# donahowe/TheaterGen

Hardware: AMD Instinct MI355X
Metric: 512px 50-step char images/sec (node), CMIGBench 4-turn story (higher is better)
Workload: dtype bf16; 1 GPU; SD-1.5 512x512, 4-turn story x 2 characters = 8 char images per step per GPU, 50 DDIM steps, CFG 7.5, IP-Adapter 77+4 tokens scale 0.4, bf16, random-init weights; plan=sd15, char_batch=8, cfg_batch=16, streams=1, ddim_steps=50, parallelism=dialogue-sharded x1 (RCCL broadcast + all_gather only)

## Files before the change

include/theatergen_hip.h:

```cpp
#ifndef THEATERGEN_HIP_H
#define THEATERGEN_HIP_H

#include <stdint.h>

#ifdef __cplusplus
extern "C" {
#endif

#define TG_BF16 0
#define TG_F16 1

#define TG_OK 0
#define TG_ERR_ARG (-1)
#define TG_ERR_LAUNCH (-2)
#define TG_ERR_UNSUPPORTED (-3)

#define TG_ACT_NONE 0
#define TG_ACT_SILU 1
#define TG_ACT_GELU 2
#define TG_ACT_QUICK_GELU 3

#define TG_ABI_VERSION 308
int tg_version(void);
const char* tg_last_error(void);

typedef struct {
  int32_t dtype;
  int32_t mode;
  const void* a0;
  const void* a1;
  int32_t c0, c1;
  int32_t batch, in_h, in_w, out_h, out_w;
  int32_t stride, upsample;
  const void* w;
  int64_t M, N, K;
  const void* bias;
  const void* bvec;
  int64_t ldbvec;
  int64_t rows_per_batch;
  const void* res;
  int64_t ldres;
  int32_t act;
  int32_t geglu;
  float out_scale;
  void* out;
  int64_t ldc;
  int64_t n_split;
  void* out_t;
  int64_t ldt;
  void* workspace;
  int64_t workspace_bytes;
  int32_t force_split_k;
  int32_t force_tile;
  int64_t a_rows_per_batch;
  int64_t a_batch_stride;
  int32_t pad_mode;
  int32_t a_silu;
  const void* a_coef;
  const float* ln_u;
  const float* ln_v;
  float ln_eps;
  const float* ln_rows;
  int64_t lda;
  int64_t ldw;
  float* out_gn_partials;
  int32_t out_gn_groups;
} tg_gemm_desc;

int tg_gemm(const tg_gemm_desc* d, void* stream);
int64_t tg_gemm_workspace_bytes(const tg_gemm_desc* d);
int tg_gemm_plan(const tg_gemm_desc* d, int32_t* tile_m, int32_t* tile_n, int32_t* splits, int32_t* kernel_kind);
int tg_gemm_gn_partial_blocks(const tg_gemm_desc* d);

int tg_conv_up2_eligible(const tg_gemm_desc* d);
int tg_conv_up2(const tg_gemm_desc* d, void* stream);

typedef struct {
  int32_t dtype;
  int32_t batch, heads, head_dim;
  int32_t n_q;
  const void* q; int64_t q_ld, q_bs;
  const void* k0; int64_t k0_ld, k0_bs;
  const void* vt0; int64_t vt0_ld, vt0_bs;
  int32_t len0;
  const void* k1; int64_t k1_ld, k1_bs;
  const void* vt1; int64_t vt1_ld, vt1_bs;
  int32_t len1;
  float scale;
  float w1;
  void* out; int64_t out_ld, out_bs;
  int32_t causal;
  const float* w1_dev;
  const float* mask;
  int64_t mask_bs, mask_hs, mask_qs;
} tg_attn_desc;

int tg_attention(const tg_attn_desc* d, void* stream);

typedef struct {
  int32_t dtype, batch, heads, head_dim, n;
  const void* q; const void* k; const void* v; const void* dout;
  int64_t ld, bs;
  const void* qt; const void* kt; const void* doutt;
  int64_t t_ld, t_bs;
  float* stats;
  void* dq; void* dk; void* dv;
  float scale;
} tg_attn_bwd_desc;
int tg_attention_bwd(const tg_attn_bwd_desc* d, void* stream);
typedef struct {
  int32_t dtype, batch, heads, head_dim, n_q, n_k;
  const void* q; const void* dout; int64_t q_ld, q_bs;
  const void* k; const void* v; int64_t k_ld, k_bs;
  const void* kt; int64_t t_ld, t_bs;
  const float* extra; int64_t extra_ld;
  float* stats;
  void* dq;
  float scale, ds_scale;
} tg_attn_bwd_cross_desc;
int tg_attention_bwd_cross(const tg_attn_bwd_cross_desc* d, void* stream);
int tg_attention_bwd_wide(const tg_attn_bwd_desc* d, void* stream);
int tg_attention_bwd_cross_wide(const tg_attn_bwd_cross_desc* d, void* stream);

int tg_attn_probs(int32_t dtype, int32_t batch, int32_t b0, int32_t heads, int32_t head_dim, int32_t n_q,
                  const void* q, int64_t q_ld, int64_t q_bs, const void* k, int64_t k_ld, int64_t k_bs,
                  int32_t len, float scale, const int32_t* tokens, int32_t n_tokens, float* probs, void* stream);

int64_t tg_groupnorm_scratch_bytes(int32_t batch, int64_t hw, int32_t groups);
int tg_groupnorm(int32_t dtype, const void* x0, const void* x1, int32_t c0, int32_t c1, int32_t batch, int64_t hw,
                 int32_t groups, float eps, const void* gamma, const void* beta, int32_t silu, void* out,
                 void* partials, void* stream);
int tg_layernorm(int32_t dtype, const void* x, int64_t rows, int32_t C, int64_t ldx, float eps, const void* gamma,
                 const void* beta, void* out, int64_t ldo, void* stream);
int tg_layernorm_stats(int32_t dtype, const void* x, int64_t rows, int32_t C, int64_t ldx, float eps, float* stats, void* stream);
int tg_groupnorm_coef(int32_t dtype, const void* x0, const void* x1, int32_t c0, int32_t c1, int32_t batch, int64_t hw,
                      int32_t groups, float eps, const void* gamma, const void* beta, float* coef, void* partials, void* stream);

int tg_groupnorm_from_partials(int32_t dtype, const void* x, int32_t C, int32_t batch, int64_t hw, int32_t groups, float eps, const void* gamma,
                               const void* beta, int32_t silu, void* out, float* coef, const float* partials, int32_t nblk, void* stream);

int tg_geglu(int32_t dtype, const void* x, int64_t rows, int64_t inner, void* out, void* stream);
int tg_act(int32_t dtype, const void* x, int64_t n, int32_t act, void* out, void* stream);
int tg_add(int32_t dtype, const void* a, const void* b, int64_t n, void* out, void* stream);

int tg_transpose(int32_t dtype, const void* src, int32_t batch, int32_t rows, int32_t cols, void* dst, void* stream);

int tg_conv1x1_nchw(const float* x, int32_t batch, int32_t cin, int32_t cout, int64_t hw, const float* weight,
                    const float* bias, float in_scale, float* out, void* stream);
int tg_softmax_rows(int32_t dtype, const void* x, int64_t rows, int32_t cols, int64_t ldx, float scale, void* out,
                    int64_t ldo, void* stream);

int tg_conv_in(int32_t dtype, const void* sample, int32_t src_dtype, int32_t batch, int32_t cin, int32_t h, int32_t w,
               const void* weight, const void* bias, int32_t cout, void* out, void* stream);
int tg_conv_out(int32_t dtype, const void* x, int32_t batch, int32_t cin, int32_t h, int32_t w, const void* weight,
                const void* bias, int32_t cout, void* out, int32_t out_f32, void* stream);
int tg_conv_out_gn(int32_t dtype, const void* x, const float* coef, int32_t a_silu, int32_t batch, int32_t cin, int32_t h, int32_t w,
                   const void* weight, const void* bias, int32_t cout, void* out, int32_t out_f32, void* stream);
int tg_conv_out_takes_coef(int32_t cin, int32_t h, int32_t w, int32_t cout);

int tg_timestep_embedding(int32_t dtype, const float* t, const int32_t* index, int32_t t_stride, int32_t rows, int32_t dim,
                          int32_t flip_sin_to_cos, float freq_shift, void* out, int64_t ldo, void* stream);

int tg_step_epilogue(const float* noise_pred, float* latents, int32_t n_img, int32_t chw, int32_t hw,
                     int32_t has_cfg, float guidance_scale, const float* coef, int32_t* step_idx, int32_t advance,
                     int32_t prediction_type, const float* frozen, const float* frozen_mask, int32_t mask_per_img,
                     int32_t frozen_steps, float* history, void* model_in, int32_t model_in_dtype, void* stream);

int tg_step_epilogue_sigma(const float* noise_pred, float* latents, int32_t n_img, int32_t chw, int32_t hw,
                           int32_t has_cfg, float guidance_scale, const float* coef, int32_t* step_idx, int32_t advance,
                           const void* noise, int32_t noise_dtype, const float* frozen, const float* frozen_mask,
                           int32_t mask_per_img, int32_t frozen_steps, float* history, void* model_in, int32_t model_in_dtype,
                           void* stream);

int tg_pixel_unshuffle(int32_t dtype, const void* in, int32_t batch, int32_t channels, int32_t h, int32_t w, int32_t factor,
                       void* out, void* stream);
int tg_relu(int32_t dtype, const void* x, int64_t n, void* out, void* stream);
int tg_avgpool2x2(int32_t dtype, const void* x, int32_t batch, int32_t h, int32_t w, int32_t channels, void* out, void* stream);
int tg_scale_repeat(int32_t dtype, const void* x, int64_t n, float scale, int32_t copies, void* out, void* stream);

int64_t tg_groupnorm_bwd_scratch_bytes(int32_t batch, int64_t hw, int32_t groups);
int tg_groupnorm_bwd(int32_t dtype, const void* x, const void* dy, int32_t batch, int64_t hw, int32_t channels, int32_t groups, float eps,
                     const void* gamma, const void* beta, int32_t silu, void* dx, void* partials, void* stream);
int tg_layernorm_bwd(int32_t dtype, const void* x, const void* dy, int64_t rows, int32_t channels, float eps, const void* gamma, void* dx,
                     void* stream);
int tg_geglu_bwd(int32_t dtype, const void* h, const void* dg, int64_t rows, int64_t inner, void* dh, void* stream);
int tg_softmax_bwd_rows(int32_t dtype, const void* probs, int32_t probs_fp32, int64_t ld_probs, const void* dprobs, int64_t ld_dprobs,
                        const float* extra, int64_t ld_extra, int64_t rows, int32_t length, float scale, void* dscores, void* probs_out,
                        int64_t ld_out, void* stream);
int tg_sumpool2x2(int32_t dtype, const void* du, int32_t batch, int32_t h, int32_t w, int32_t channels, void* out, void* stream);

int tg_blend_latents(const float* bg, const float* fg, const float* mask, int32_t planes, int32_t hw, float ratio,
                     float sigma, int32_t storage_dtype, float* out, void* stream);
int tg_shift(const float* src, int64_t planes, int32_t h, int32_t w, int32_t dx, int32_t dy, float* dst, void* stream);
int tg_gaussian_sample(const float* moments, const float* noise, int32_t batch, int32_t channels, int32_t hw, float scale,
                       float* out, void* stream);
int tg_add_noise(const float* x0, const float* noise, const float* ca, const float* cb, int32_t steps, int64_t n, float* out,
                 void* stream);
int tg_masked_compose(float* dst, const float* src, const float* mask, int64_t planes, int32_t hw, void* stream);

int tg_guidance_topk(const float* attn, int32_t heads, int32_t hw, int32_t n_tok, int32_t token, const float* mask,
                     int32_t k_fg, int32_t k_bg, float fg_w, float bg_w, float scale, float* out, float* grad,
                     void* stream);
int tg_guidance_ratio(const float* attn, int32_t heads, int32_t hw, int32_t n_tok, int32_t token, const float* mask,
                      float scale, float* out, float* grad, void* stream);
int tg_guidance_ref(const float* attn, int32_t heads, int32_t hw, int32_t n_tok, int32_t token, const float* ref,
                    const float* mask, float eps, float scale, float* out, float* grad, void* stream);
typedef struct {
  const float* attn;
  float* grad;
  const float* mask;
  const float* ref;
  int32_t heads, hw, n_tok, token;
  int32_t kind, k_fg, k_bg, reserved;
  float fg_w, bg_w, scale, eps;
} tg_guidance_item;
int tg_guidance_batch(const tg_guidance_item* items_device, int32_t n_items, int32_t max_hw_topk, int32_t max_heads,
                      float* partials, float* out, void* stream);

#define TG_GUIDANCE_MAX_SLOTS 64
typedef struct {
  int32_t attn_slot, grad_slot , mask_slot, ref_slot ;
  int32_t heads, hw, n_tok, token;
  int32_t kind, k_fg, k_bg, reserved;
  float fg_w, bg_w, scale, eps;
} tg_guidance_pitem;
int tg_guidance_plan_run(const tg_guidance_pitem* items_device, int32_t n_items, int32_t max_hw_topk, int32_t max_heads,
                         const void* const* slots_host, int32_t n_slots, float* head_terms, float* out, void* stream);

typedef struct {
  int32_t dtype;
  const void* x; int64_t ldx;
  const void* wpk;
  const void* res; int64_t ldres;
  void* out; int64_t ldc;
  int64_t M;
  int32_t N, K;
  int32_t ln;
  float ln_eps;
  int32_t variant;
  const float* v640;
  const float* u640;
} tg_rc_linear_desc;
int tg_rc_linear(const tg_rc_linear_desc* d, void* stream);

typedef struct {
  int32_t dtype;
  const void* h; int64_t ldh;
  const void* wq;
  const void* kv;
  const void* wo;
  void* out; int64_t ldc;
  int64_t M;
  int32_t rows_per_batch;
  int32_t text_len, ip_tokens;
  float ln_eps;
  const float* ip_scale;
} tg_rc_xattn_desc;
int tg_rc_xattn(const tg_rc_xattn_desc* d, void* stream);
int tg_rc_kv_pack(int32_t dtype, int32_t batch, const void* k, const void* vt, int64_t ldt, int32_t text_len, const void* kip,
                  const void* vtip, int64_t ldi, int32_t ip_tokens, void* out, void* stream);

typedef struct {
  int32_t dtype;
  const void* h; int64_t ldh;
  const void* w1;
  const void* w2;
  const float* b2;
  const void* wpo;
  const void* res0; int64_t ldres;
  void* out; int64_t ldc;
  int64_t M;
  int32_t inner;
  float ln_eps;
  int32_t dbg;
} tg_rc_ff_desc;
int tg_rc_ff(const tg_rc_ff_desc* d, void* stream);

typedef struct {
  int32_t dtype;
  const void* x; int64_t ldx;
  const float* coef;
  const void* win;
  const void* wqkv;
  void* y; int64_t ldy;
  void* qk; int64_t ldqk;
  void* vt; int64_t ldt;
  int64_t M;
  int32_t rows_per_batch;
  float ln_eps;
  int32_t dbg;
} tg_rc_front_desc;
int tg_rc_front(const tg_rc_front_desc* d, void* stream);

typedef struct {
  void* ptr;
  int64_t ld;
  int64_t batch_stride;
  int32_t n_end;
  int32_t transposed;
} tg_skinny_seg;
typedef struct {
  int32_t dtype;
  const void* x; int64_t ldx;
  const void* wpk;
  int64_t M;
  int32_t N, K;
  int32_t ln;
  float ln_eps;
  const float* ln_u;
  const float* ln_v;
  const void* bias;
  int32_t act;
  const void* res; int64_t ldres;
  int32_t nseg;
  int32_t rows_per_batch;
  tg_skinny_seg seg[3];
} tg_skinny_desc;
int tg_skinny_gemm(const tg_skinny_desc* d, void* stream);

typedef struct {
  int32_t dtype;
  const void* x; int64_t ldx;
  const void* wq;
  const float* ln_u;
  const float* ln_v;
  float ln_eps;
// ... 18 lines not shown
```

theatergen_amd/_lib.py:

```python
import ctypes as C
import os

HERE = os.path.dirname(os.path.abspath(__file__))
LIB_PATH = os.environ.get("THEATERGEN_HIP_LIB") or os.path.join(HERE, "lib", "libtheatergen_hip.so")

TG_BF16, TG_F16 = 0, 1
ABI_VERSION = 308
ACT_NONE, ACT_SILU, ACT_GELU, ACT_QUICK_GELU = 0, 1, 2, 3

i32, i64, f32, vp = C.c_int32, C.c_int64, C.c_float, C.c_void_p


class GemmDesc(C.Structure):
    _fields_ = [
        ("dtype", i32), ("mode", i32), ("a0", vp), ("a1", vp), ("c0", i32), ("c1", i32),
        ("batch", i32), ("in_h", i32), ("in_w", i32), ("out_h", i32), ("out_w", i32),
        ("stride", i32), ("upsample", i32), ("w", vp), ("M", i64), ("N", i64), ("K", i64),
        ("bias", vp), ("bvec", vp), ("ldbvec", i64), ("rows_per_batch", i64), ("res", vp), ("ldres", i64),
        ("act", i32), ("geglu", i32), ("out_scale", f32), ("out", vp), ("ldc", i64), ("n_split", i64),
        ("out_t", vp), ("ldt", i64), ("workspace", vp), ("workspace_bytes", i64),
        ("force_split_k", i32), ("force_tile", i32), ("a_rows_per_batch", i64), ("a_batch_stride", i64),
        ("pad_mode", i32), ("a_silu", i32), ("a_coef", vp), ("ln_u", vp), ("ln_v", vp), ("ln_eps", f32), ("ln_rows", vp),
        ("lda", i64), ("ldw", i64), ("out_gn_partials", vp), ("out_gn_groups", i32),
    ]
# ... 34 lines not shown
        ("dtype", i32), ("x", vp), ("ldx", i64), ("wpk", vp), ("res", vp), ("ldres", i64),
        ("out", vp), ("ldc", i64), ("M", i64), ("N", i32), ("K", i32), ("ln", i32), ("ln_eps", f32), ("variant", i32), ("v640", vp), ("u640", vp),
    ]


class RcXattnDesc(C.Structure):
    _fields_ = [
        ("dtype", i32), ("h", vp), ("ldh", i64), ("wq", vp), ("kv", vp), ("wo", vp), ("out", vp), ("ldc", i64), ("M", i64),
        ("rows_per_batch", i32), ("text_len", i32), ("ip_tokens", i32), ("ln_eps", f32), ("ip_scale", vp),
    ]


class XqAttnDesc(C.Structure):
    _fields_ = [
        ("dtype", i32), ("x", vp), ("ldx", i64), ("wq", vp), ("ln_u", vp), ("ln_v", vp), ("ln_eps", f32), ("kv", vp), ("ip_scale", vp),
        ("out", vp), ("ldc", i64), ("M", i64), ("C", i32), ("head_dim", i32), ("rows_per_batch", i32), ("text_len", i32), ("ip_tokens", i32),
    ]


class RcFfDesc(C.Structure):
    _fields_ = [
        ("dtype", i32), ("h", vp), ("ldh", i64), ("w1", vp), ("w2", vp), ("b2", vp), ("wpo", vp), ("res0", vp), ("ldres", i64),
        ("out", vp), ("ldc", i64), ("M", i64), ("inner", i32), ("ln_eps", f32), ("dbg", i32),
    ]


class SkinnySeg(C.Structure):
    _fields_ = [("ptr", vp), ("ld", i64), ("batch_stride", i64), ("n_end", i32), ("transposed", i32)]


class SkinnyDesc(C.Structure):
    _fields_ = [
        ("dtype", i32), ("x", vp), ("ldx", i64), ("wpk", vp), ("M", i64), ("N", i32), ("K", i32), ("ln", i32), ("ln_eps", f32), ("ln_u", vp), ("ln_v", vp),
        ("bias", vp), ("act", i32), ("res", vp), ("ldres", i64), ("nseg", i32), ("rows_per_batch", i32), ("seg", SkinnySeg * 3),
    ]


class RcFrontDesc(C.Structure):
    _fields_ = [
        ("dtype", i32), ("x", vp), ("ldx", i64), ("coef", vp), ("win", vp), ("wqkv", vp), ("y", vp), ("ldy", i64), ("qk", vp), ("ldqk", i64),
        ("vt", vp), ("ldt", i64), ("M", i64), ("rows_per_batch", i32), ("ln_eps", f32), ("dbg", i32),
    ]


class GuidanceItem(C.Structure):
    _fields_ = [
        ("attn", vp), ("grad", vp), ("mask", vp), ("ref", vp),
        ("heads", i32), ("hw", i32), ("n_tok", i32), ("token", i32),
        ("kind", i32), ("k_fg", i32), ("k_bg", i32), ("reserved", i32),
        ("fg_w", f32), ("bg_w", f32), ("scale", f32), ("eps", f32),
    ]


class GuidancePItem(C.Structure):
    _fields_ = [
        ("attn_slot", i32), ("grad_slot", i32), ("mask_slot", i32), ("ref_slot", i32),
        ("heads", i32), ("hw", i32), ("n_tok", i32), ("token", i32),
        ("kind", i32), ("k_fg", i32), ("k_bg", i32), ("reserved", i32),
        ("fg_w", f32), ("bg_w", f32), ("scale", f32), ("eps", f32),
    ]


GUIDANCE_MAX_SLOTS = 64

SIGNATURES = {
    "tg_version": (i32, []),
    "tg_last_error": (C.c_char_p, []),
    "tg_gemm": (i32, [C.POINTER(GemmDesc), vp]),
    "tg_gemm_workspace_bytes": (i64, [C.POINTER(GemmDesc)]),
    "tg_gemm_plan": (i32, [C.POINTER(GemmDesc), vp, vp, vp, vp]),
    "tg_attention": (i32, [C.POINTER(AttnDesc), vp]),
    "tg_attention_bwd": (i32, [C.POINTER(AttnBwdDesc), vp]),
    "tg_attention_bwd_cross": (i32, [C.POINTER(AttnBwdCrossDesc), vp]),
    "tg_attention_bwd_wide": (i32, [C.POINTER(AttnBwdDesc), vp]),
    "tg_attention_bwd_cross_wide": (i32, [C.POINTER(AttnBwdCrossDesc), vp]),
    "tg_attn_probs": (i32, [i32, i32, i32, i32, i32, i32, vp, i64, i64, vp, i64, i64, i32, f32, vp, i32, vp, vp]),
    "tg_groupnorm_scratch_bytes": (i64, [i32, i64, i32]),
    "tg_groupnorm": (i32, [i32, vp, vp, i32, i32, i32, i64, i32, f32, vp, vp, i32, vp, vp, vp]),
    "tg_layernorm": (i32, [i32, vp, i64, i32, i64, f32, vp, vp, vp, i64, vp]),
    "tg_layernorm_stats": (i32, [i32, vp, i64, i32, i64, f32, vp, vp]),
    "tg_groupnorm_coef": (i32, [i32, vp, vp, i32, i32, i32, i64, i32, f32, vp, vp, vp, vp, vp]),
    "tg_groupnorm_from_partials": (i32, [i32, vp, i32, i32, i64, i32, f32, vp, vp, i32, vp, vp, vp, i32, vp]),
    "tg_gemm_gn_partial_blocks": (i32, [C.POINTER(GemmDesc)]),
    "tg_conv_up2_eligible": (i32, [C.POINTER(GemmDesc)]),
    "tg_conv_up2": (i32, [C.POINTER(GemmDesc), vp]),
    "tg_geglu": (i32, [i32, vp, i64, i64, vp, vp]),
    "tg_act": (i32, [i32, vp, i64, i32, vp, vp]),
    "tg_add": (i32, [i32, vp, vp, i64, vp, vp]),
    "tg_transpose": (i32, [i32, vp, i32, i32, i32, vp, vp]),
    "tg_conv1x1_nchw": (i32, [vp, i32, i32, i32, i64, vp, vp, f32, vp, vp]),
    "tg_softmax_rows": (i32, [i32, vp, i64, i32, i64, f32, vp, i64, vp]),
    "tg_conv_in": (i32, [i32, vp, i32, i32, i32, i32, i32, vp, vp, i32, vp, vp]),
    "tg_conv_out": (i32, [i32, vp, i32, i32, i32, i32, vp, vp, i32, vp, i32, vp]),
    "tg_conv_out_gn": (i32, [i32, vp, vp, i32, i32, i32, i32, i32, vp, vp, i32, vp, i32, vp]),
    "tg_conv_out_takes_coef": (i32, [i32, i32, i32, i32]),
    "tg_timestep_embedding": (i32, [i32, vp, vp, i32, i32, i32, i32, f32, vp, i64, vp]),
    "tg_step_epilogue": (i32, [vp, vp, i32, i32, i32, i32, f32, vp, vp, i32, i32, vp, vp, i32, i32, vp, vp, i32, vp]),
    "tg_step_epilogue_sigma": (i32, [vp, vp, i32, i32, i32, i32, f32, vp, vp, i32, vp, i32, vp, vp, i32, i32, vp, vp, i32, vp]),
    "tg_pixel_unshuffle": (i32, [i32, vp, i32, i32, i32, i32, i32, vp, vp]),
    "tg_relu": (i32, [i32, vp, i64, vp, vp]),
    "tg_avgpool2x2": (i32, [i32, vp, i32, i32, i32, i32, vp, vp]),
    "tg_scale_repeat": (i32, [i32, vp, i64, f32, i32, vp, vp]),
    "tg_blend_latents": (i32, [vp, vp, vp, i32, i32, f32, f32, i32, vp, vp]),
    "tg_shift": (i32, [vp, i64, i32, i32, i32, i32, vp, vp]),
    "tg_masked_compose": (i32, [vp, vp, vp, i64, i32, vp]),
    "tg_gaussian_sample": (i32, [vp, vp, i32, i32, i32, f32, vp, vp]),
    "tg_add_noise": (i32, [vp, vp, vp, vp, i32, i64, vp, vp]),
    "tg_guidance_topk": (i32, [vp, i32, i32, i32, i32, vp, i32, i32, f32, f32, f32, vp, vp, vp]),
    "tg_guidance_ratio": (i32, [vp, i32, i32, i32, i32, vp, f32, vp, vp, vp]),
    "tg_guidance_ref": (i32, [vp, i32, i32, i32, i32, vp, vp, f32, f32, vp, vp, vp]),
    "tg_guidance_batch": (i32, [vp, i32, i32, i32, vp, vp, vp]),
    "tg_guidance_plan_run": (i32, [vp, i32, i32, i32, vp, i32, vp, vp, vp]),
    "tg_groupnorm_bwd_scratch_bytes": (i64, [i32, i64, i32]),
    "tg_groupnorm_bwd": (i32, [i32, vp, vp, i32, i64, i32, i32, f32, vp, vp, i32, vp, vp, vp]),
    "tg_layernorm_bwd": (i32, [i32, vp, vp, i64, i32, f32, vp, vp, vp]),
    "tg_geglu_bwd": (i32, [i32, vp, vp, i64, i64, vp, vp]),
    "tg_softmax_bwd_rows": (i32, [i32, vp, i32, i64, vp, i64, vp, i64, i64, i32, f32, vp, vp, i64, vp]),
    "tg_sumpool2x2": (i32, [i32, vp, i32, i32, i32, i32, vp, vp]),
    "tg_rc_linear": (i32, [C.POINTER(RcLinearDesc), vp]),
    "tg_rc_xattn": (i32, [C.POINTER(RcXattnDesc), vp]),
    "tg_rc_kv_pack": (i32, [i32, i32, vp, vp, i64, i32, vp, vp, i64, i32, vp, vp]),
    "tg_rc_ff": (i32, [C.POINTER(RcFfDesc), vp]),
    "tg_rc_front": (i32, [C.POINTER(RcFrontDesc), vp]),
    "tg_skinny_gemm": (i32, [C.POINTER(SkinnyDesc), vp]),
    "tg_xq_attn": (i32, [C.POINTER(XqAttnDesc), vp]),
    "tg_xq_kv_bytes": (i64, [i32, i32, i32]),
    "tg_xq_kv_pack": (i32, [i32, i32, i32, i32, vp, vp, i64, i32, vp, vp, i64, i32, vp, vp]),
    "tg_debug_mfma32": (i32, [i32, vp, vp, vp, vp]),
}

_lib = None


def lib():
    global _lib
    if _lib is None:
        if not os.path.exists(LIB_PATH):
            raise RuntimeError(
                f"theatergen_amd: HIP library not found at {LIB_PATH}; build it with "
                "`python -m theatergen_amd.build` (hipcc --offload-arch=gfx950). There is no CPU fallback.")
        import torch
        h = C.CDLL(LIB_PATH)
        h.tg_version.restype = i32
        got = h.tg_version()
        compat = os.environ.get("THEATERGEN_HIP_LIB") and os.environ.get("THEATERGEN_HIP_ABI_COMPAT") == str(got)
        for name, (res, args) in SIGNATURES.items():
            if compat and not hasattr(h, name):
                continue
            fn = getattr(h, name)
            fn.restype = res
            fn.argtypes = args
        if got != ABI_VERSION and not compat:
            raise RuntimeError(f"theatergen_amd: {LIB_PATH} has ABI version {got}, this binding needs {ABI_VERSION}: "
                               "rebuild with `python -m theatergen_amd.build` (a stale library would misread descriptors)")
        _lib = h
    return _lib


def check(rc):
    if rc != 0:
        msg = lib().tg_last_error()
        raise RuntimeError(f"theatergen_hip error {rc}: {msg.decode() if msg else ''}")
```

theatergen_amd/attention_processor.py:

```python
import os
import weakref

import torch
import torch.nn as nn

from . import ops, rowchain


def _round8(n):
    return (n + 7) // 8 * 8


def tensor_version(t):
    try:
        return t._version
    except RuntimeError:
        return None


_REPLAY_STREAMS = []


def register_replay_stream(stream, device=None):
    dev = torch.device(device) if device is not None else stream.device
# ... 178 lines not shown
            self.norm_cross = None
        elif cross_attention_norm == "layer_norm":
            self.norm_cross = nn.LayerNorm(cross_attention_dim)
        elif cross_attention_norm == "group_norm":
            self.norm_cross = nn.GroupNorm(num_channels=cross_attention_dim, num_groups=cross_attention_norm_num_groups, eps=1e-5, affine=True)
        else:
            raise ValueError(f"unknown cross_attention_norm: {cross_attention_norm}. Should be None, 'layer_norm' or 'group_norm'")
        self.to_q = nn.Linear(query_dim, inner_dim, bias=bias)
        self.to_k = nn.Linear(cross_attention_dim, inner_dim, bias=bias)
        self.to_v = nn.Linear(cross_attention_dim, inner_dim, bias=bias)
        self.to_out = nn.ModuleList([nn.Linear(inner_dim, query_dim, bias=out_bias), nn.Dropout(dropout)])
        self.set_processor(processor if processor is not None else AttnProcessor())

    def set_processor(self, processor):
        if hasattr(self, "processor") and isinstance(self.processor, nn.Module) and not isinstance(processor, nn.Module):
            self._modules.pop("processor")
        self.processor = processor

    def forward(self, hidden_states, encoder_hidden_states=None, attention_mask=None, **cross_attention_kwargs):
        return self.processor(self, hidden_states, encoder_hidden_states=encoder_hidden_states,
                              attention_mask=attention_mask, **cross_attention_kwargs)


def _check_common(attn, hidden_states, attn_process_fn):
    if attn_process_fn is not None:
        raise NotImplementedError("theatergen_amd: attn_process_fn would need materialised probabilities (unsupported)")
    if getattr(attn, "spatial_norm", None) is not None:
        raise NotImplementedError("theatergen_amd: attn.spatial_norm (MoVQ SpatialNorm) is not supported")
    if getattr(attn, "added_kv_proj_dim", None) is not None:
        raise NotImplementedError("theatergen_amd: added_kv_proj_dim belongs to the AttnAddedKV processors (unsupported)")
    _need_gpu(hidden_states)


def _need_gpu(t):
    if not t.is_cuda:
        raise RuntimeError("theatergen_amd: attention runs on the GPU only (no CPU fallback)")


def _group_norm_tokens(gn, x2d, B, N):
    return ops.groupnorm(x2d, B, N, gn.num_groups, gn.eps, gn.weight, gn.bias)


def _norm_encoder(attn, enc):
    nc = attn.norm_cross
    B, L, ctx = enc.shape
    e2 = enc.contiguous().reshape(B * L, ctx)
    if isinstance(nc, nn.LayerNorm):
        return ops.layernorm(e2, nc.weight, nc.bias, nc.eps).reshape(B, L, ctx)
    if isinstance(nc, nn.GroupNorm):
        return ops.groupnorm(e2, B, L, nc.num_groups, nc.eps, nc.weight, nc.bias).reshape(B, L, ctx)
    raise RuntimeError(f"theatergen_amd: unknown attn.norm_cross {type(nc).__name__}")


def _prepare_mask(attention_mask, L, B, heads, N):
    m = attention_mask
    if m.ndim != 3:
        raise RuntimeError(f"theatergen_amd: attention_mask must be 3-D [batch(*heads), 1 or queries, keys], got {tuple(m.shape)}")
    if m.shape[-1] != L:
        raise RuntimeError(f"theatergen_amd: attention_mask covers {m.shape[-1]} keys, the key sequence has {L} "
                           "(prepare_attention_mask would pad it to a length baddbmm rejects)")
    if m.shape[1] not in (1, N):
        raise RuntimeError(f"theatergen_amd: attention_mask has {m.shape[1]} query rows for {N} queries")
    m = m.to(torch.float32)
    if m.shape[0] == B * heads and heads > 1:
        m = m.reshape(B, heads, m.shape[1], L)
    elif m.shape[0] == B:
        m = m.reshape(B, 1, m.shape[1], L)
    elif m.shape[0] == 1:
        m = m.reshape(1, 1, m.shape[1], L)
    else:
        raise RuntimeError(f"theatergen_amd: attention_mask batch {m.shape[0]} matches neither batch {B} nor batch * heads {B * heads}")
    return m.contiguous()


def _to_tokens(hidden_states):
    if hidden_states.ndim == 4:
        b, c, h, w = hidden_states.shape
        x = ops.transpose(hidden_states.contiguous(), b, c, h * w)
        return x.reshape(b * h * w, c), b, h * w, c, (b, c, h, w)
    b, n, c = hidden_states.shape
    return hidden_states.contiguous().reshape(b * n, c), b, n, c, None


def _finish(attn, o2d, B, N, C, shape4, x_tokens, fused_residual):
    res = fused_residual
    if res is None and attn.residual_connection:
        res = x_tokens
    out = None
    if attn.rescale_output_factor == 1.0:
        out = rowchain.linear320(o2d, attn.to_out[0].weight, attn.to_out[0].bias, res, attn, "to_out", _cached)
    if out is None:
        out = ops.linear(o2d, attn.to_out[0].weight, attn.to_out[0].bias, res=res, out_scale=1.0 / attn.rescale_output_factor)
    if shape4 is not None:
        b, c, h, w = shape4
        return ops.transpose(out, b, h * w, c).reshape(b, c, h, w)
    return out.reshape(B, N, C)


def _enc_rows(enc):
    B, L, ctx = enc.shape
    if enc.stride(2) == 1 and enc.stride(1) == ctx and enc.stride(0) >= L * ctx and enc.stride(0) % 8 == 0:
        return enc, L, enc.stride(0)
    enc = enc.contiguous()
    return enc, L, L * ctx


def _save_probs(attn, q, q_ld, k, k_ld, B, N, L, save_attn_to_dict, save_keys, attn_key, return_cond_ca_only,
                return_token_ca_only, offload_cross_attn_to_cpu):
    b0 = 0
    if return_cond_ca_only:
        assert B % 2 == 0, f"Samples are not in pairs: {B} samples"
        b0 = B // 2
    tokens = None
    if return_token_ca_only is not None:
        if isinstance(return_token_ca_only, int):
            tokens = torch.tensor([return_token_ca_only], dtype=torch.int32, device=q.device)
        else:
            tokens = torch.as_tensor(return_token_ca_only).to(device=q.device, dtype=torch.int32).reshape(-1)
    _, heads, d = attn_dims(attn)
    probs = ops.attn_probs(q, q_ld, N * q_ld, k, k_ld, L * k_ld, B, b0, heads, d, N, L, attn.scale, tokens)
    if offload_cross_attn_to_cpu:
        probs = probs.cpu()
    if save_attn_to_dict is not None and (save_keys is None or (tuple(attn_key) in save_keys)):
        save_attn_to_dict[tuple(attn_key)] = probs
    return probs


def front_eligible(attn, kwargs):
    if type(attn.processor) is not AttnProcessor or kwargs.get("attention_mask") is not None or kwargs.get("attn_process_fn") is not None:
        return False
    if getattr(attn, "group_norm", None) is not None or getattr(attn, "spatial_norm", None) is not None:
        return False
    if attn.rescale_output_factor != 1.0 or attn.residual_connection or kwargs.get("return_attntion_probs"):
        return False
    inner, heads, d = attn_dims(attn)
    return inner == 320 and attn.to_q.weight.shape[1] == 320


def self_attention_from_qkv(attn, qk, vt, ldt, B, N, residual):
    inner, heads, d = attn_dims(attn)
    o = torch.empty((B * N, inner), dtype=qk.dtype, device=qk.device)
    ops.attention(qk, 2 * inner, N * 2 * inner, qk[:, inner:], 2 * inner, N * 2 * inner, vt, ldt, inner * ldt, N,
                  B, heads, d, N, attn.scale, o, inner, N * inner)
    return _finish(attn, o, B, N, inner, None, None, residual).reshape(B * N, -1)


def fused_cross_block(attn, norm, x2d, B, N, enc, kwargs):
    proc = attn.processor
    if type(proc) not in (AttnProcessor, IPAttnProcessor) or enc is None or enc.ndim != 3:
        rowchain.trace("xattn no: processor / enc", type(proc).__name__, None if enc is None else tuple(enc.shape))
        return None
    for k in ("save_attn_to_dict", "attention_mask", "attn_process_fn"):
        if kwargs.get(k) is not None:
            return None
    if kwargs.get("return_attntion_probs") or attn.rescale_output_factor != 1.0 or attn.residual_connection:
        return None
    if getattr(attn, "group_norm", None) is not None or getattr(attn, "norm_cross", None) or getattr(attn, "spatial_norm", None) is not None:
        return None
    is_ip = type(proc) is IPAttnProcessor
    T = int(proc.num_tokens) if is_ip else 0
    L = enc.shape[1] - T
    C = x2d.shape[1]
    if enc.shape[0] != B or not rowchain.xattn_eligible(attn, C, B, N, L, T, x2d.dtype) or x2d.stride(0) != C:
        rowchain.trace("xattn no", tuple(enc.shape), B, N, C, L, T)
        return None
    rowchain.trace("xattn yes", B, N, T)
    inner = 320
    if is_ip:
        enc_c = enc.contiguous()
        kvpk = proc.project_kv_frags(attn, enc_c)
        scale_dev = proc.scale_device(x2d.device)
    else:
        e, Lr, enc_bs = _enc_rows(enc)
        ldt = _round8(L)
        k = torch.empty((B * L, inner), dtype=x2d.dtype, device=x2d.device)
# ... 262 lines not shown
```

theatergen_amd/csrc/tg_elementwise.hip:

```cpp
#include "tg_common.h"

namespace {

template <typename T>
__global__ __launch_bounds__(256) void geglu_kernel(const T* x, long rows, long inner, T* out) {
  typedef typename Vec<T>::v8 V8;
  const long c8 = inner / 8;
  const long total = rows * c8;
  for (long i = (long)blockIdx.x * blockDim.x + threadIdx.x; i < total; i += (long)gridDim.x * blockDim.x) {
    const long r = i / c8, c = (i - r * c8) * 8;
    V8 a = *reinterpret_cast<const V8*>(x + r * 2 * inner + c);
    V8 g = *reinterpret_cast<const V8*>(x + r * 2 * inner + inner + c);
    V8 o;
#pragma unroll
    for (int j = 0; j < 8; ++j) o[j] = from_f32<T>(to_f32<T>(a[j]) * gelu_erf_f(to_f32<T>(g[j])));
    *reinterpret_cast<V8*>(out + r * inner + c) = o;
  }
}

template <typename T>
__global__ __launch_bounds__(256) void act_kernel(const T* x, long n, int act, T* out) {
  for (long i = (long)blockIdx.x * blockDim.x + threadIdx.x; i < n; i += (long)gridDim.x * blockDim.x) {
    float f = to_f32<T>(x[i]);
    f = apply_act(f, act);
// ... 275 lines not shown
    *reinterpret_cast<V8*>(d + (c0 + c) * rows + r0 + rg * 32 + q * 8) = o;
  }
}

inline int grid_for(long n, int per_thread = 1) {
  long b = (n / per_thread + 255) / 256;
  if (b < 1) b = 1;
  if (b > 2048) b = 2048;
  return (int)b;
}

template <typename T>
__global__ __launch_bounds__(256) void conv_in_fast_kernel(const void* sample, int src_dtype, int batch, int cin, int h, int w,
                                                           const T* weight, const T* bias, int cout, T* out, int groups) {
  typedef typename Vec<T>::v8 V8;
  extern __shared__ float cin_smem[];
  const int K = 9 * cin;
  float* sw = cin_smem;
  float* patch = sw + K * cout;
  const int tid = threadIdx.x, G = cout >> 3;
  for (int i = tid; i < K * cout; i += blockDim.x) {
    const int n = i / K, k = i - n * K;
    sw[k * cout + n] = to_f32<T>(weight[i]);
  }
  const long npix = (long)batch * h * w;
  const int ppb = groups * 2;
  const int g = tid / G, cg = tid - g * G;
  float bias8[8];
#pragma unroll
  for (int e = 0; e < 8; ++e) bias8[e] = (bias != nullptr && g < groups) ? to_f32<T>(bias[cg * 8 + e]) : 0.f;
  for (long base = (long)blockIdx.x * ppb; base < npix; base += (long)gridDim.x * ppb) {
    __syncthreads();
    for (int i = tid; i < ppb * K; i += blockDim.x) {
      const int lp = i / K, k = i - lp * K;
      const long pix = base + lp;
      float v = 0.f;
      if (pix < npix) {
        const int tap = k / cin, c = k - tap * cin;
        const int ky = tap / 3, kx = tap - ky * 3;
        const int b = (int)(pix / (h * w));
        const int r = (int)(pix - (long)b * h * w);
        const int y = r / w + ky - 1, x = r % w + kx - 1;
        if (y >= 0 && y < h && x >= 0 && x < w) v = load_src(sample, src_dtype, (((long)b * cin + c) * h + y) * w + x);
      }
      patch[i] = v;
    }
    __syncthreads();
    if (g >= groups) continue;
    float a0[8], a1[8];
#pragma unroll
    for (int e = 0; e < 8; ++e) { a0[e] = bias8[e]; a1[e] = bias8[e]; }
    const float* p0 = patch + (2 * g) * K;
    const float* p1 = p0 + K;
    const float* wp = sw + cg * 8;
    for (int k = 0; k < K; ++k) {
      const f32x4 wlo = *reinterpret_cast<const f32x4*>(wp + k * cout);
      const f32x4 whi = *reinterpret_cast<const f32x4*>(wp + k * cout + 4);
      const float x0 = p0[k], x1 = p1[k];
#pragma unroll
      for (int e = 0; e < 4; ++e) {
        a0[e] = __builtin_fmaf(x0, wlo[e], a0[e]);
        a0[4 + e] = __builtin_fmaf(x0, whi[e], a0[4 + e]);
        a1[e] = __builtin_fmaf(x1, wlo[e], a1[e]);
        a1[4 + e] = __builtin_fmaf(x1, whi[e], a1[4 + e]);
      }
    }
    const long pix0 = base + 2 * g;
    V8 o;
    if (pix0 < npix) {
#pragma unroll
      for (int e = 0; e < 8; ++e) o[e] = from_f32<T>(a0[e]);
      *reinterpret_cast<V8*>(out + pix0 * cout + cg * 8) = o;
    }
    if (pix0 + 1 < npix) {
#pragma unroll
      for (int e = 0; e < 8; ++e) o[e] = from_f32<T>(a1[e]);
      *reinterpret_cast<V8*>(out + (pix0 + 1) * cout + cg * 8) = o;
    }
  }
}

template <typename T>
__global__ __launch_bounds__(256) void conv_in_mfma_kernel(const void* sample, int src_dtype, int batch, int h, int w, const T* weight, const T* bias,
                                                           int cout, T* out) {
  typedef typename Vec<T>::v8 V8;
  typedef typename Vec<T>::v4 V4;
  constexpr int CIN = 4, K = 36, KP = 48, WP = 56, OP = 168;
  extern __shared__ __attribute__((aligned(16))) char cim_smem[];
  T* sw = reinterpret_cast<T*>(cim_smem);
  const int tid = threadIdx.x, lane = tid & 63, wave = tid >> 6, l31 = lane & 31, hi = lane >> 5;
  T* so = sw + (size_t)cout * WP + (size_t)wave * 32 * OP;
  for (int i = tid; i < cout * (KP / 4); i += 256) {
    const int n = i / (KP / 4), c = i - n * (KP / 4);
    V4 v;
#pragma unroll
    for (int e = 0; e < 4; ++e) v[e] = from_f32<T>(0.f);
    if (c < K / 4) v = *reinterpret_cast<const V4*>(weight + n * K + 4 * c);
    *reinterpret_cast<V4*>(sw + n * WP + 4 * c) = v;
  }
  __syncthreads();
  const long npix = (long)batch * h * w;
  for (long base = ((long)blockIdx.x * 4 + wave) * 32; base < npix; base += (long)gridDim.x * 128) {
    const long pix = base + l31;
    const bool ok = pix < npix;
    const long pp = ok ? pix : 0;
    const int b = (int)(pp / ((long)h * w));
    const int r = (int)(pp - (long)b * h * w);
    const int y = r / w, x = r - y * w;
    V8 bh[3], bl[3];
#pragma unroll
    for (int ks = 0; ks < 3; ++ks)
#pragma unroll
      for (int e = 0; e < 8; ++e) {
        const int k = 16 * ks + 8 * hi + e, tap = k >> 2, c = k & 3;
        const int ky = tap / 3, kx = tap - 3 * ky;
        const int yy = y + ky - 1, xx = x + kx - 1;
        float v = 0.f;
        if (ok && tap < 9 && yy >= 0 && yy < h && xx >= 0 && xx < w) v = load_src(sample, src_dtype, (((long)b * CIN + c) * h + yy) * w + xx);
        const T vh = from_f32<T>(v);
        bh[ks][e] = vh;
        bl[ks][e] = from_f32<T>(v - to_f32<T>(vh));
      }
    for (int half = 0; half < cout / 160; ++half) {
      f32x16 acc[5];
#pragma unroll
      for (int j = 0; j < 5; ++j) {
#pragma unroll
        for (int q = 0; q < 16; ++q) acc[j][q] = 0.f;
#pragma unroll
        for (int ks = 0; ks < 3; ++ks) {
          const V8 a = *reinterpret_cast<const V8*>(sw + (size_t)(half * 160 + 32 * j + l31) * WP + 16 * ks + 8 * hi);
          acc[j] = mfma32(a, bl[ks], acc[j]);
          acc[j] = mfma32(a, bh[ks], acc[j]);
        }
      }
#pragma unroll
      for (int j = 0; j < 5; ++j)
#pragma unroll
        for (int g = 0; g < 4; ++g) {
          const int ch = 32 * j + 8 * g + 4 * hi;
          V4 o;
#pragma unroll
          for (int e = 0; e < 4; ++e) o[e] = from_f32<T>(acc[j][4 * g + e] + (bias != nullptr ? to_f32<T>(bias[half * 160 + ch + e]) : 0.f));
          *reinterpret_cast<V4*>(so + l31 * OP + ch) = o;
        }
      __builtin_amdgcn_wave_barrier();
      asm volatile("s_waitcnt lgkmcnt(0)" ::: "memory");
#pragma unroll
      for (int it = 0; it < 10; ++it) {
        const int q = it * 64 + lane, px = q / 20, cn = q - px * 20;
        const V8 v = *reinterpret_cast<const V8*>(so + px * OP + cn * 8);
        if (base + px < npix) *reinterpret_cast<V8*>(out + (base + px) * cout + half * 160 + cn * 8) = v;
      }
      __builtin_amdgcn_wave_barrier();
      asm volatile("s_waitcnt lgkmcnt(0)" ::: "memory");
    }
  }
}

__device__ __forceinline__ float dot8_acc(bf16x8 a, bf16x8 b, float acc) {
  typedef __attribute__((ext_vector_type(2))) __bf16 bf16x2;
#pragma unroll
  for (int i = 0; i < 4; ++i) {
    bf16x2 x = {a[2 * i], a[2 * i + 1]}, y = {b[2 * i], b[2 * i + 1]};
    acc = __builtin_amdgcn_fdot2_f32_bf16(x, y, acc, false);
  }
  return acc;
}
__device__ __forceinline__ float dot8_acc(f16x8 a, f16x8 b, float acc) {
  typedef __attribute__((ext_vector_type(2))) _Float16 f16x2;
#pragma unroll
  for (int i = 0; i < 4; ++i) {
    f16x2 x = {a[2 * i], a[2 * i + 1]}, y = {b[2 * i], b[2 * i + 1]};
    acc = __builtin_amdgcn_fdot2(x, y, acc, false);
  }
  return acc;
}

template <typename T, int COUT>
__global__ __launch_bounds__(256) void conv_out_fast_kernel(const T* x, int batch, int cin, int h, int w, const T* weight,
                                                            const T* bias, int cout, void* out, int out_f32) {
  typedef typename Vec<T>::v8 V8;
  extern __shared__ __attribute__((aligned(16))) char cout_smem[];
  T* sw = reinterpret_cast<T*>(cout_smem);
  const int K = 9 * cin, c8 = cin >> 3;
  for (int i = threadIdx.x; i < cout * K / 8; i += blockDim.x)
    reinterpret_cast<V8*>(sw)[i] = reinterpret_cast<const V8*>(weight)[i];
  __syncthreads();
  const int lane = threadIdx.x & 63;
  const long npix = (long)batch * h * w, npair = (npix + 1) >> 1;
  const long nw = (long)gridDim.x * 4;
  V8 zero8;
#pragma unroll
  for (int e = 0; e < 8; ++e) zero8[e] = from_f32<T>(0.f);
  for (long pp = (long)blockIdx.x * 4 + (threadIdx.x >> 6); pp < npair; pp += nw) {
    const long pix0 = 2 * pp, pix1 = pix0 + 1;
    const bool v1 = pix1 < npix;
    const int b0 = (int)(pix0 / (h * w)), r0 = (int)(pix0 - (long)b0 * h * w);
    const int y0 = r0 / w, x0 = r0 - y0 * w;
    const long q1 = v1 ? pix1 : pix0;
    const int b1 = (int)(q1 / (h * w)), r1 = (int)(q1 - (long)b1 * h * w);
    const int y1 = r1 / w, x1 = r1 - y1 * w;
    float acc0[COUT], acc1[COUT];
#pragma unroll
    for (int n = 0; n < COUT; ++n) { acc0[n] = 0.f; acc1[n] = 0.f; }
    for (int i = lane; i < 9 * c8; i += 64) {
      const int tap = i / c8, c = (i - tap * c8) << 3;
      const int dy = tap / 3 - 1, dx = tap - (tap / 3) * 3 - 1;
      const int ya = y0 + dy, xa = x0 + dx, yb = y1 + dy, xb = x1 + dx;
      V8 va = zero8, vb = zero8;
      if (ya >= 0 && ya < h && xa >= 0 && xa < w) va = *reinterpret_cast<const V8*>(x + (((long)b0 * h + ya) * w + xa) * cin + c);
      if (v1 && yb >= 0 && yb < h && xb >= 0 && xb < w) vb = *reinterpret_cast<const V8*>(x + (((long)b1 * h + yb) * w + xb) * cin + c);
#pragma unroll
      for (int n = 0; n < COUT; ++n) {
        if (n < cout) {
          const V8 wv = *reinterpret_cast<const V8*>(sw + n * K + tap * cin + c);
          acc0[n] = dot8_acc(va, wv, acc0[n]);
          acc1[n] = dot8_acc(vb, wv, acc1[n]);
        }
      }
    }
#pragma unroll
    for (int n = 0; n < COUT; ++n) {
      if (n >= cout) continue;
      const float s0 = wave_sum(acc0[n]), s1 = wave_sum(acc1[n]);
      if (lane == 0) {
        const float bn = bias ? to_f32<T>(bias[n]) : 0.f;
        const long o0 = (((long)b0 * cout + n) * h + y0) * w + x0;
        const long o1 = (((long)b1 * cout + n) * h + y1) * w + x1;
        if (out_f32) {
          reinterpret_cast<float*>(out)[o0] = s0 + bn;
          if (v1) reinterpret_cast<float*>(out)[o1] = s1 + bn;
        } else {
          reinterpret_cast<T*>(out)[o0] = from_f32<T>(s0 + bn);
          if (v1) reinterpret_cast<T*>(out)[o1] = from_f32<T>(s1 + bn);
// ... 102 lines not shown
  if (idx >= (long)batch * hw) return;
  const long b = idx / hw, p = idx - b * hw;
  float v[8];
  for (int c = 0; c < cin; ++c) v[c] = x[(b * cin + c) * hw + p] * in_scale;
  for (int o = 0; o < cout; ++o) {
    float a = bias ? bias[o] : 0.f;
    for (int c = 0; c < cin; ++c) a += w[o * cin + c] * v[c];
    out[(b * cout + o) * hw + p] = a;
  }
}

template <typename T>
__global__ __launch_bounds__(256) void softmax_rows_kernel(const T* x, long rows, int cols, long ldx, float scale, T* out, long ldo) {
  typedef typename Vec<T>::v8 V8;
  const int lane = threadIdx.x & 63;
  const long row = (long)blockIdx.x * 4 + (threadIdx.x >> 6);
  if (row >= rows) return;
  const T* xr = x + row * ldx;
  T* orow = out + row * ldo;
  const int c8 = cols / 8;
  float mx = -INFINITY;
  for (int i = lane; i < c8; i += 64) {
    V8 v = *reinterpret_cast<const V8*>(xr + i * 8);
#pragma unroll
    for (int j = 0; j < 8; ++j) mx = fmaxf(mx, to_f32<T>(v[j]));
  }
  mx = wave_max(mx) * scale;
  const float c = scale * 1.4426950408889634f, mc = mx * 1.4426950408889634f;
  float sum = 0.f;
  for (int i = lane; i < c8; i += 64) {
    V8 v = *reinterpret_cast<const V8*>(xr + i * 8);
#pragma unroll
    for (int j = 0; j < 8; ++j) sum += __builtin_amdgcn_exp2f(__builtin_fmaf(to_f32<T>(v[j]), c, -mc));
  }
  const float inv = 1.f / wave_sum(sum);
  for (int i = lane; i < c8; i += 64) {
    V8 v = *reinterpret_cast<const V8*>(xr + i * 8);
    V8 o;
#pragma unroll
    for (int j = 0; j < 8; ++j) o[j] = from_f32<T>(__builtin_amdgcn_exp2f(__builtin_fmaf(to_f32<T>(v[j]), c, -mc)) * inv);
    *reinterpret_cast<V8*>(orow + i * 8) = o;
  }
}

}

#define DISPATCH(dtype, NAME, GRID, BLOCK, LDS, ...)                                            \
  do {                                                                                          \
    if ((dtype) == TG_BF16) hipLaunchKernelGGL(NAME<bf16_t>, GRID, BLOCK, LDS, st, __VA_ARGS__); \
    else hipLaunchKernelGGL(NAME<f16_t>, GRID, BLOCK, LDS, st, __VA_ARGS__);                     \
  } while (0)

extern "C" int tg_geglu(int32_t dtype, const void* x, int64_t rows, int64_t inner, void* out, void* stream) {
  TG_CHECK((dtype == TG_BF16 || dtype == TG_F16) && x && out && rows > 0 && inner > 0 && inner % 8 == 0, TG_ERR_ARG,
           "tg_geglu: bad args");
  hipStream_t st = reinterpret_cast<hipStream_t>(stream);
  const int grid = grid_for(rows * inner / 8);
  if (dtype == TG_BF16) hipLaunchKernelGGL(geglu_kernel<bf16_t>, dim3(grid), dim3(256), 0, st, (const bf16_t*)x, rows, inner, (bf16_t*)out);
  else hipLaunchKernelGGL(geglu_kernel<f16_t>, dim3(grid), dim3(256), 0, st, (const f16_t*)x, rows, inner, (f16_t*)out);
  TG_LAUNCH_CHECK();
  return TG_OK;
}

extern "C" int tg_act(int32_t dtype, const void* x, int64_t n, int32_t act, void* out, void* stream) {
  TG_CHECK((dtype == TG_BF16 || dtype == TG_F16) && x && out && n > 0, TG_ERR_ARG, "tg_act: bad args");
  hipStream_t st = reinterpret_cast<hipStream_t>(stream);
  const int grid = grid_for(n);
  if (dtype == TG_BF16) hipLaunchKernelGGL(act_kernel<bf16_t>, dim3(grid), dim3(256), 0, st, (const bf16_t*)x, n, act, (bf16_t*)out);
  else hipLaunchKernelGGL(act_kernel<f16_t>, dim3(grid), dim3(256), 0, st, (const f16_t*)x, n, act, (f16_t*)out);
  TG_LAUNCH_CHECK();
  return TG_OK;
}

extern "C" int tg_add(int32_t dtype, const void* a, const void* b, int64_t n, void* out, void* stream) {
  TG_CHECK((dtype == TG_BF16 || dtype == TG_F16) && a && b && out && n > 0, TG_ERR_ARG, "tg_add: bad args");
  hipStream_t st = reinterpret_cast<hipStream_t>(stream);
  const int grid = grid_for(n, 8);
  if (dtype == TG_BF16) hipLaunchKernelGGL(add_kernel<bf16_t>, dim3(grid), dim3(256), 0, st, (const bf16_t*)a, (const bf16_t*)b, n, (bf16_t*)out);
  else hipLaunchKernelGGL(add_kernel<f16_t>, dim3(grid), dim3(256), 0, st, (const f16_t*)a, (const f16_t*)b, n, (f16_t*)out);
  TG_LAUNCH_CHECK();
  return TG_OK;
}

extern "C" int tg_conv_in(int32_t dtype, const void* sample, int32_t src_dtype, int32_t batch, int32_t cin, int32_t h,
                          int32_t w, const void* weight, const void* bias, int32_t cout, void* out, void* stream) {
  TG_CHECK((dtype == TG_BF16 || dtype == TG_F16) && sample && weight && out, TG_ERR_ARG, "tg_conv_in: bad args");
  TG_CHECK(src_dtype >= 0 && src_dtype <= 2 && batch > 0 && cin > 0 && cin <= 16 && cout > 0, TG_ERR_ARG, "tg_conv_in: bad shape");
  hipStream_t st = reinterpret_cast<hipStream_t>(stream);
  const long npix = (long)batch * h * w;
  {
    static const bool mfma_on = [] { const char* e = getenv("TG_CONV_IN_MFMA"); return !(e && e[0] == '0'); }();
    if (mfma_on && cin == 4 && cout % 160 == 0 && cout <= 640 && (reinterpret_cast<uintptr_t>(out) & 15) == 0 && (reinterpret_cast<uintptr_t>(weight) & 7) == 0) {
      const size_t lds = ((size_t)cout * 56 + 4 * 32 * 168) * 2;
      long nb = (npix + 127) / 128;
      if (nb > 1024) nb = 1024;
      if (dtype == TG_BF16) {
        auto k = conv_in_mfma_kernel<bf16_t>;
        static const hipError_t attr = hipFuncSetAttribute(reinterpret_cast<const void*>(k), hipFuncAttributeMaxDynamicSharedMemorySize, 160 * 1024);
        (void)attr;
        hipLaunchKernelGGL(k, dim3((unsigned)nb), dim3(256), lds, st, sample, src_dtype, batch, h, w, (const bf16_t*)weight, (const bf16_t*)bias, cout, (bf16_t*)out);
      } else {
        auto k = conv_in_mfma_kernel<f16_t>;
        static const hipError_t attr = hipFuncSetAttribute(reinterpret_cast<const void*>(k), hipFuncAttributeMaxDynamicSharedMemorySize, 160 * 1024);
        (void)attr;
        hipLaunchKernelGGL(k, dim3((unsigned)nb), dim3(256), lds, st, sample, src_dtype, batch, h, w, (const f16_t*)weight, (const f16_t*)bias, cout, (f16_t*)out);
      }
      TG_LAUNCH_CHECK();
      return TG_OK;
    }
  }
  {
    const int K = 9 * cin, G = cout / 8;
    const int groups = G > 0 ? 256 / G : 0;
    if (cout % 8 == 0 && groups >= 1 && (reinterpret_cast<uintptr_t>(out) & 15) == 0) {
      const size_t lds = ((size_t)K * cout + (size_t)groups * 2 * K) * sizeof(float);
      if (lds <= 64 * 1024) {
        long nb = (npix + groups * 2 - 1) / (groups * 2);
        if (nb > 512) nb = 512;
        if (dtype == TG_BF16)
          hipLaunchKernelGGL(conv_in_fast_kernel<bf16_t>, dim3((unsigned)nb), dim3(256), lds, st, sample, src_dtype, batch, cin, h, w, (const bf16_t*)weight, (const bf16_t*)bias, cout, (bf16_t*)out, groups);
        else
          hipLaunchKernelGGL(conv_in_fast_kernel<f16_t>, dim3((unsigned)nb), dim3(256), lds, st, sample, src_dtype, batch, cin, h, w, (const f16_t*)weight, (const f16_t*)bias, cout, (f16_t*)out, groups);
        TG_LAUNCH_CHECK();
        return TG_OK;
      }
    }
  }
  const int ppb = 4;
  const size_t lds = (size_t)ppb * 9 * cin * sizeof(float);
  dim3 grid((unsigned)((npix + ppb - 1) / ppb));
  if (dtype == TG_BF16)
    hipLaunchKernelGGL(conv_in_kernel<bf16_t>, grid, dim3(256), lds, st, sample, src_dtype, batch, cin, h, w, (const bf16_t*)weight, (const bf16_t*)bias, cout, (bf16_t*)out);
  else
    hipLaunchKernelGGL(conv_in_kernel<f16_t>, grid, dim3(256), lds, st, sample, src_dtype, batch, cin, h, w, (const f16_t*)weight, (const f16_t*)bias, cout, (f16_t*)out);
  TG_LAUNCH_CHECK();
  return TG_OK;
}

namespace {
bool conv_out_mfma_ok(int cin, int h, int w, int cout) {
  static const bool on = [] { const char* e = getenv("TG_CONV_OUT_MFMA"); return !(e && e[0] == '0'); }();
  return on && cin % 64 == 0 && cin <= 320 && cout > 0 && cout <= 8 && h % 8 == 0 && w % 16 == 0;
}
}

extern "C" int tg_conv_out_takes_coef(int32_t cin, int32_t h, int32_t w, int32_t cout) { return conv_out_mfma_ok(cin, h, w, cout) ? 1 : 0; }

static int conv_out_impl(int32_t dtype, const void* x, const float* coef, int32_t a_silu, int32_t batch, int32_t cin, int32_t h, int32_t w,
                         const void* weight, const void* bias, int32_t cout, void* out, int32_t out_f32, void* stream) {
  TG_CHECK((dtype == TG_BF16 || dtype == TG_F16) && x && weight && out, TG_ERR_ARG, "tg_conv_out: bad args");
  TG_CHECK(batch > 0 && cin % 8 == 0 && cout > 0 && cout <= 8, TG_ERR_ARG, "tg_conv_out: bad shape cin=%d cout=%d", cin, cout);
  hipStream_t st = reinterpret_cast<hipStream_t>(stream);
  const long npix = (long)batch * h * w;
  if (conv_out_mfma_ok(cin, h, w, cout) && (reinterpret_cast<uintptr_t>(x) & 15) == 0 && (reinterpret_cast<uintptr_t>(weight) & 15) == 0) {
    const size_t lds = ((size_t)180 * cin + (size_t)cout * 9 * cin) * 2 + (size_t)2 * cin * 4;
    const dim3 g((unsigned)(batch * (h / 8) * (w / 16)));
    if (dtype == TG_BF16) {
      auto k = conv_out_mfma_kernel<bf16_t>;
      static const hipError_t attr = hipFuncSetAttribute(reinterpret_cast<const void*>(k), hipFuncAttributeMaxDynamicSharedMemorySize, 160 * 1024);
      (void)attr;
      hipLaunchKernelGGL(k, g, dim3(512), lds, st, (const bf16_t*)x, coef, a_silu, batch, cin, h, w, (const bf16_t*)weight, (const bf16_t*)bias, cout, out, out_f32);
    } else {
      auto k = conv_out_mfma_kernel<f16_t>;
      static const hipError_t attr = hipFuncSetAttribute(reinterpret_cast<const void*>(k), hipFuncAttributeMaxDynamicSharedMemorySize, 160 * 1024);
      (void)attr;
      hipLaunchKernelGGL(k, g, dim3(512), lds, st, (const f16_t*)x, coef, a_silu, batch, cin, h, w, (const f16_t*)weight, (const f16_t*)bias, cout, out, out_f32);
    }
    TG_LAUNCH_CHECK();
    return TG_OK;
  }
  TG_CHECK(coef == nullptr, TG_ERR_UNSUPPORTED, "tg_conv_out_gn: the GroupNorm prologue needs a problem the matrix-core kernel takes (tg_conv_out_takes_coef)");
  {
    const size_t lds = (size_t)cout * 9 * cin * 2;
    if (lds <= 64 * 1024 && (reinterpret_cast<uintptr_t>(x) & 15) == 0 && (reinterpret_cast<uintptr_t>(weight) & 15) == 0) {
      long nb = ((npix + 1) / 2 + 3) / 4;
      if (nb > 1024) nb = 1024;
      const dim3 g((unsigned)nb);
      if (dtype == TG_BF16) {
        if (cout <= 4) hipLaunchKernelGGL((conv_out_fast_kernel<bf16_t, 4>), g, dim3(256), lds, st, (const bf16_t*)x, batch, cin, h, w, (const bf16_t*)weight, (const bf16_t*)bias, cout, out, out_f32);
        else hipLaunchKernelGGL((conv_out_fast_kernel<bf16_t, 8>), g, dim3(256), lds, st, (const bf16_t*)x, batch, cin, h, w, (const bf16_t*)weight, (const bf16_t*)bias, cout, out, out_f32);
      } else {
        if (cout <= 4) hipLaunchKernelGGL((conv_out_fast_kernel<f16_t, 4>), g, dim3(256), lds, st, (const f16_t*)x, batch, cin, h, w, (const f16_t*)weight, (const f16_t*)bias, cout, out, out_f32);
        else hipLaunchKernelGGL((conv_out_fast_kernel<f16_t, 8>), g, dim3(256), lds, st, (const f16_t*)x, batch, cin, h, w, (const f16_t*)weight, (const f16_t*)bias, cout, out, out_f32);
      }
      TG_LAUNCH_CHECK();
      return TG_OK;
    }
  }
// ... 146 lines not shown
```

theatergen_amd/csrc/tg_rowchain.hip:

```cpp
#include "tg_common.h"

#include <type_traits>
#include <utility>

#ifdef TG_RC_DEV_BUILD
#define RC_DBG(bit) ((p.dbg & (bit)) != 0)
#define RC_DBG_ARG() (p.dbg >> 8)
#else
#define RC_DBG(bit) (false)
#define RC_DBG_ARG() (0)
#endif
#define RC_DBG_RT(bit) ((p.dbg & (bit)) != 0)

namespace {

struct RcLinearParams {
  const void* x;
  long ldx;
  const void* wpk;
  const void* res;
  long ldres;
  void* out;
  long ldc;
  long M;
  int N, K;
  float ln_eps;
  int dbg;
};

template <typename V>
__device__ __forceinline__ V gld(const void* ptr) { return *(const __attribute__((address_space(1))) V*)ptr; }
template <typename V>
__device__ __forceinline__ void gst(void* ptr, V v) { *(__attribute__((address_space(1))) V*)ptr = v; }

__device__ __forceinline__ int rc_block_id(int bid, int nblocks) {
  const int q = nblocks >> 3, r = nblocks & 7;
  const int xcd = bid & 7;
  const int start = xcd < r ? xcd * (q + 1) : r * (q + 1) + (xcd - r) * q;
  return start + (bid >> 3);
}

template <typename T> __device__ __forceinline__ typename Vec<T>::v8 pack8(const float* f) {
  typename Vec<T>::v8 o;
#pragma unroll
  for (int e = 0; e < 8; ++e) o[e] = from_f32<T>(f[e]);
  return o;
}

#define TG_SEL4_DPP(QP, MASK, D, X, Y)                                                                          \
  asm volatile("s_mov_b32 vcc_lo, " MASK "\n\ts_mov_b32 vcc_hi, " MASK "\n\t"                                    \
               "v_cndmask_b32_dpp %0, %4, %8, vcc quad_perm:" QP " row_mask:0xf bank_mask:0xf\n\t"               \
               "v_cndmask_b32_dpp %1, %5, %9, vcc quad_perm:" QP " row_mask:0xf bank_mask:0xf\n\t"               \
               "v_cndmask_b32_dpp %2, %6, %10, vcc quad_perm:" QP " row_mask:0xf bank_mask:0xf\n\t"              \
               "v_cndmask_b32_dpp %3, %7, %11, vcc quad_perm:" QP " row_mask:0xf bank_mask:0xf"                   \
               : "=&v"(D[0]), "=&v"(D[1]), "=&v"(D[2]), "=&v"(D[3])                                             \
               : "v"(X[0]), "v"(X[1]), "v"(X[2]), "v"(X[3]), "v"(Y[0]), "v"(Y[1]), "v"(Y[2]), "v"(Y[3])         \
               : "vcc")
template <typename V8> __device__ __forceinline__ void quad_transpose(V8& p0, V8& p1, V8& p2, V8& p3) {
  unsigned x[4][4], y[4][4];
  {
    const u32x4 t0 = __builtin_bit_cast(u32x4, p0), t1 = __builtin_bit_cast(u32x4, p1), t2 = __builtin_bit_cast(u32x4, p2), t3 = __builtin_bit_cast(u32x4, p3);
#pragma unroll
    for (int d = 0; d < 4; ++d) { x[0][d] = t0[d]; x[1][d] = t1[d]; x[2][d] = t2[d]; x[3][d] = t3[d]; }
  }
  TG_SEL4_DPP("[1,0,3,2]", "0x55555555", y[0], x[1], x[0]);
  TG_SEL4_DPP("[1,0,3,2]", "0x55555555", y[2], x[3], x[2]);
  TG_SEL4_DPP("[1,0,3,2]", "0xaaaaaaaa", y[1], x[0], x[1]);
  TG_SEL4_DPP("[1,0,3,2]", "0xaaaaaaaa", y[3], x[2], x[3]);
  TG_SEL4_DPP("[2,3,0,1]", "0x33333333", x[0], y[2], y[0]);
  TG_SEL4_DPP("[2,3,0,1]", "0x33333333", x[1], y[3], y[1]);
  TG_SEL4_DPP("[2,3,0,1]", "0xcccccccc", x[2], y[0], y[2]);
  TG_SEL4_DPP("[2,3,0,1]", "0xcccccccc", x[3], y[1], y[3]);
  u32x4 o0, o1, o2, o3;
#pragma unroll
  for (int d = 0; d < 4; ++d) { o0[d] = x[0][d]; o1[d] = x[1][d]; o2[d] = x[2][d]; o3[d] = x[3][d]; }
  p0 = __builtin_bit_cast(V8, o0); p1 = __builtin_bit_cast(V8, o1); p2 = __builtin_bit_cast(V8, o2); p3 = __builtin_bit_cast(V8, o3);
}

template <typename T, int KS, int NW, int NBUF, bool LN, int PD>
__global__ __launch_bounds__(NW * 64) void rc_linear_kernel(RcLinearParams p) {
  typedef typename Vec<T>::v8 V8;
  constexpr int NP = 2 * KS + 1;
  constexpr int CB = NP * 1024;
  constexpr int PPW = (NP + NW - 1) / NW;
  extern __shared__ __attribute__((aligned(16))) char smem[];

  const int tid = threadIdx.x;
  const int lane = tid & 63;
  const int wave = __builtin_amdgcn_readfirstlane(tid >> 6);
  const int l31 = lane & 31, hi = lane >> 5;
  const int lbid = rc_block_id((int)blockIdx.x, (int)gridDim.x);
  const long tok0 = ((long)lbid * NW + wave) * 32;
  const int qb = lane & 3;
  long mrow[4];
  bool mok[4];
#pragma unroll
  for (int i = 0; i < 4; ++i) {
    const long r = tok0 + (l31 & ~3) + i;
    mok[i] = r < p.M;
    mrow[i] = mok[i] ? r : p.M - 1;
  }
  const int NC = p.N >> 6;
  const char* wpk = reinterpret_cast<const char*>(p.wpk);

  auto issue_chunk = [&](int c, int buf) {
    const char* src = wpk + (long)c * CB + lane * 16;
    char* dst = smem + buf * CB;
#pragma unroll
    for (int j = 0; j < PPW; ++j) {
      const int i = j * NW + wave;
      if (i < NP)
        __builtin_amdgcn_global_load_lds((const __attribute__((address_space(1))) void*)(src + i * 1024),
                                         (__attribute__((address_space(3))) void*)(dst + i * 1024), 16, 0, 0);
    }
  };
#pragma unroll
  for (int b = 0; b < NBUF - 1; ++b)
    if (b < NC) issue_chunk(b, b);

  V8 B[KS];
  {
    const T* xp = reinterpret_cast<const T*>(p.x) + 32 * hi + 8 * qb;
#pragma unroll
    for (int s = 0; s < KS; ++s) B[s] = *reinterpret_cast<const V8*>(xp + mrow[s & 3] * p.ldx + 64 * (s >> 2));
#pragma unroll
    for (int q = 0; q < KS / 4; ++q) quad_transpose(B[4 * q], B[4 * q + 1], B[4 * q + 2], B[4 * q + 3]);
  }
  float ln_rstd = 1.f, ln_std = 1.f, ln_nmean = 0.f;
  if constexpr (LN) {
    float sum = 0.f;
#pragma unroll
    for (int s = 0; s < KS; ++s)
#pragma unroll
      for (int e = 0; e < 8; ++e) sum += to_f32<T>(B[s][e]);
    sum += __shfl_xor(sum, 32, 64);
    const float inv_k = 1.0f / (float)p.K;
    const float mean = sum * inv_k;
    float c2 = 0.f;
#pragma unroll
    for (int s = 0; s < KS; ++s) {
      asm volatile("" : "+v"(B[s]));
#pragma unroll
      for (int e = 0; e < 8; ++e) { const float d = to_f32<T>(B[s][e]) - mean; c2 = __builtin_fmaf(d, d, c2); }
    }
    c2 += __shfl_xor(c2, 32, 64);
    const float var = c2 * inv_k + p.ln_eps;
    ln_rstd = __builtin_amdgcn_rsqf(var);
    ln_std = var * ln_rstd;
    ln_nmean = -mean;
  } else {
#pragma unroll
    for (int s = 0; s < KS; ++s) asm volatile("" : "+v"(B[s]));
  }

  const T* resp = reinterpret_cast<const T*>(p.res);
  T* outp = reinterpret_cast<T*>(p.out);
  V8 pend[4];
  long pend_ch = -1;
  for (int c = 0; c < NC; ++c) {
    const int buf = c % NBUF;
    asm volatile("s_waitcnt vmcnt(0)" ::: "memory");
    if (!RC_DBG(4)) __builtin_amdgcn_s_barrier();
    if (c + NBUF - 1 < NC && !RC_DBG(2)) issue_chunk(c + NBUF - 1, (c + NBUF - 1) % NBUF);
    if (pend_ch >= 0 && !RC_DBG(1)) {
#pragma unroll
      for (int i = 0; i < 4; ++i)
        if (mok[i]) *reinterpret_cast<V8*>(outp + mrow[i] * p.ldc + pend_ch + 8 * qb) = pend[i];
    }
    const long ch0 = 64 * (long)c + 32 * hi;
    V8 r8[4];
    if (resp != nullptr) {
#pragma unroll
      for (int i = 0; i < 4; ++i) r8[i] = *reinterpret_cast<const V8*>(resp + mrow[i] * p.ldres + ch0 + 8 * qb);
    }
    const char* cbase = smem + buf * CB;
    f32x16 acc[2];
    {
      const float* vec = reinterpret_cast<const float*>(cbase + 2 * KS * 1024) + 32 * hi;
#pragma unroll
      for (int uu = 0; uu < 2; ++uu)
#pragma unroll
        for (int g = 0; g < 4; ++g) {
          const f32x4 v4 = *reinterpret_cast<const f32x4*>(vec + 16 * uu + 4 * g);
          if constexpr (LN) {
            const f32x4 u4 = *reinterpret_cast<const f32x4*>(vec + 64 + 16 * uu + 4 * g);
#pragma unroll
            for (int e = 0; e < 4; ++e) acc[uu][4 * g + e] = __builtin_fmaf(ln_nmean, u4[e], ln_std * v4[e]);
          } else {
#pragma unroll
            for (int e = 0; e < 4; ++e) acc[uu][4 * g + e] = v4[e];
          }
        }
    }
    const char* cb = cbase + lane * 16;
    if RC_DBG(8) {
    } else if constexpr (PD == 0) {
#pragma unroll
      for (int s = 0; s < KS; ++s) {
        const V8 a0 = *reinterpret_cast<const V8*>(cb + s * 1024);
        const V8 a1 = *reinterpret_cast<const V8*>(cb + (KS + s) * 1024);
        acc[0] = mfma32(a0, B[s], acc[0]);
        acc[1] = mfma32(a1, B[s], acc[1]);
      }
    } else {
      V8 a0[KS], a1[KS];
#pragma unroll
      for (int s = 0; s < PD; ++s) {
        a0[s] = *reinterpret_cast<const V8*>(cb + s * 1024);
        a1[s] = *reinterpret_cast<const V8*>(cb + (KS + s) * 1024);
      }
#pragma unroll
      for (int s = 0; s < KS; ++s) {
        if (s + PD < KS) {
          a0[s + PD] = *reinterpret_cast<const V8*>(cb + (s + PD) * 1024);
          a1[s + PD] = *reinterpret_cast<const V8*>(cb + (KS + s + PD) * 1024);
        }
        __builtin_amdgcn_sched_barrier(0);
        acc[0] = mfma32(a0[s], B[s], acc[0]);
        acc[1] = mfma32(a1[s], B[s], acc[1]);
        __builtin_amdgcn_sched_barrier(0);
      }
    }
    float o[32];
#pragma unroll
    for (int uu = 0; uu < 2; ++uu)
#pragma unroll
      for (int r = 0; r < 16; ++r) o[16 * uu + r] = LN ? acc[uu][r] * ln_rstd : acc[uu][r];
    if (resp != nullptr) {
      quad_transpose(r8[0], r8[1], r8[2], r8[3]);
#pragma unroll
      for (int i = 0; i < 4; ++i)
#pragma unroll
        for (int e = 0; e < 8; ++e) o[8 * i + e] += to_f32<T>(r8[i][e]);
    }
#pragma unroll
    for (int i = 0; i < 4; ++i) pend[i] = pack8<T>(o + 8 * i);
    quad_transpose(pend[0], pend[1], pend[2], pend[3]);
    pend_ch = ch0;
  }
  if (pend_ch >= 0) {
#pragma unroll
    for (int i = 0; i < 4; ++i)
      if (mok[i]) *reinterpret_cast<V8*>(outp + mrow[i] * p.ldc + pend_ch + 8 * qb) = pend[i];
  }
}


struct RcXattnParams {
  const void* h;
  long ldh;
  const void* wq;
  const void* kv;
  const void* wo;
  void* out;
  long ldc;
  long M;
  int rows_per_batch;
  float ln_eps;
  const float* ip_scale;
  int dbg;
};

template <typename T> __device__ __forceinline__ typename Vec<T>::v8 pack8r(const f32x16& a, int r0) {
  typename Vec<T>::v8 o;
#pragma unroll
  for (int e = 0; e < 8; ++e) o[e] = from_f32<T>(a[r0 + e]);
  return o;
}

template <typename T, int NW, int TEXT, int IPT>
__global__ __launch_bounds__(NW * 64) __attribute__((amdgpu_waves_per_eu(2, 2))) void rc_xattn_kernel(RcXattnParams p) {
  typedef typename Vec<T>::v8 V8;
  constexpr int KS = 20;
  constexpr int TBW = (KS + 1) * 1024;
  constexpr int KVH = 24 * 1024;
  constexpr int SLOT = 24 * 1024;
  static_assert(TEXT > 64 && TEXT <= 80, "text keys: three 32-key tiles, five 16-key PV steps");
  static_assert(IPT == 0 || IPT == 4 || IPT == 16, "image tokens");
  extern __shared__ __attribute__((aligned(16))) char smem[];

  const int tid = threadIdx.x;
  const int lane = tid & 63;
  const int wave = __builtin_amdgcn_readfirstlane(tid >> 6);
  const int l31 = lane & 31, hi = lane >> 5;
  const int lbid = rc_block_id((int)blockIdx.x, (int)gridDim.x);
  const long tok0 = ((long)lbid * NW + wave) * 32;
  const int qb = lane & 3;
  long mrow[4];
  bool mok[4];
#pragma unroll
  for (int i = 0; i < 4; ++i) {
    const long r = tok0 + (l31 & ~3) + i;
    mok[i] = r < p.M;
    mrow[i] = mok[i] ? r : p.M - 1;
  }
  const long bi = ((long)lbid * NW * 32) / p.rows_per_batch;
  const char* kvb = reinterpret_cast<const char*>(p.kv) + bi * (8 * KVH);

  static_assert(NW == 4, "six 1-KiB pieces per wave and stage");
  auto issue = [&](const char* src, int slot) {
    const char* s0 = src + lane * 16 + wave * 1024;
    char* dst = smem + slot * SLOT + wave * 1024;
#pragma unroll
    for (int j = 0; j < 6; ++j)
      __builtin_amdgcn_global_load_lds((const __attribute__((address_space(1))) void*)(s0 + j * NW * 1024),
                                       (__attribute__((address_space(3))) void*)(dst + j * NW * 1024), 16, 0, 0);
  };
  auto issue_stage = [&](int st) {
    if (st < 10) issue(reinterpret_cast<const char*>(p.wq) + (long)st * TBW, st % 3);
    else if (st < 18) issue(kvb + (long)(st - 10) * KVH, st % 3);
    else if (st < 28) issue(reinterpret_cast<const char*>(p.wo) + (long)(st - 18) * TBW, st % 3);
  };
  if ((RC_DBG_RT(32) && (blockIdx.x & 1)) || (RC_DBG_RT(64) && blockIdx.x >= gridDim.x / 2)) {
    for (int i = 0; i < (p.dbg >> 8); ++i) __builtin_amdgcn_s_sleep(127);
  }
  issue_stage(0);
  issue_stage(1);

  V8 H[KS];
  {
    const T* xp = reinterpret_cast<const T*>(p.h) + 32 * hi + 8 * qb;
#pragma unroll
    for (int s = 0; s < KS; ++s) H[s] = *reinterpret_cast<const V8*>(xp + mrow[s & 3] * p.ldh + 64 * (s >> 2));
#pragma unroll
    for (int q = 0; q < KS / 4; ++q) quad_transpose(H[4 * q], H[4 * q + 1], H[4 * q + 2], H[4 * q + 3]);
  }
// ... 910 lines not shown
        for (int x = 0; x < KS; ++x) {
          if (x + PD < KS) a[x + PD] = *reinterpret_cast<const V8*>(cb + (x + PD) * 1024);
          __builtin_amdgcn_sched_barrier(0);
          acc = mfma32(a[x], HB[x], acc);
          __builtin_amdgcn_sched_barrier(0);
        }
        if (uu == 0) quad_transpose(r8[0], r8[1], r8[2], r8[3]);
        float o[16];
#pragma unroll
        for (int r = 0; r < 16; ++r) o[r] = acc[r] + to_f32<T>(r8[2 * uu + (r >> 3)][r & 7]);
        pend[2 * uu] = pack8<T>(o);
        pend[2 * uu + 1] = pack8<T>(o + 8);
        if (uu == 1) quad_transpose(pend[0], pend[1], pend[2], pend[3]);
      }
    }
    {
      const long ch0 = 64 * 4 + 32 * hi;
#pragma unroll
      for (int i = 0; i < 4; ++i)
        if (mok[i]) *reinterpret_cast<V8*>(outp + mrow[i] * p.ldc + ch0 + 8 * qb) = pend[i];
    }
  }
}

template <typename T>
int launch_rc_ff(const tg_rc_ff_desc* d, const RcFfParams& p, hipStream_t st) {
  const size_t lds = 2 * 44 * 1024 + 2 * 20 * 1024;
  const long grid = (d->M + 127) / 128;
  if (d->wpo != nullptr) {
    auto k = rc_ff_kernel<T, true>;
    static const hipError_t attr = hipFuncSetAttribute(reinterpret_cast<const void*>(k), hipFuncAttributeMaxDynamicSharedMemorySize, (int)lds);
    (void)attr;
    hipLaunchKernelGGL(k, dim3((unsigned)grid), dim3(256), lds, st, p);
  } else {
    auto k = rc_ff_kernel<T, false>;
    static const hipError_t attr = hipFuncSetAttribute(reinterpret_cast<const void*>(k), hipFuncAttributeMaxDynamicSharedMemorySize, (int)lds);
    (void)attr;
    hipLaunchKernelGGL(k, dim3((unsigned)grid), dim3(256), lds, st, p);
  }
  TG_LAUNCH_CHECK();
  return TG_OK;
}

template <typename T, int KS, int NW, int NBUF, int PD>
int launch_rc_linear(const tg_rc_linear_desc* d, const RcLinearParams& p, hipStream_t st) {
  const size_t lds = (size_t)NBUF * (2 * KS + 1) * 1024;
  const long grid = (d->M + NW * 32 - 1) / (NW * 32);
  if (d->ln) {
    auto k = rc_linear_kernel<T, KS, NW, NBUF, true, PD>;
    static const hipError_t attr = hipFuncSetAttribute(reinterpret_cast<const void*>(k), hipFuncAttributeMaxDynamicSharedMemorySize, (int)lds);
    (void)attr;
    hipLaunchKernelGGL(k, dim3((unsigned)grid), dim3(NW * 64), lds, st, p);
  } else {
    auto k = rc_linear_kernel<T, KS, NW, NBUF, false, PD>;
    static const hipError_t attr = hipFuncSetAttribute(reinterpret_cast<const void*>(k), hipFuncAttributeMaxDynamicSharedMemorySize, (int)lds);
    (void)attr;
    hipLaunchKernelGGL(k, dim3((unsigned)grid), dim3(NW * 64), lds, st, p);
  }
  TG_LAUNCH_CHECK();
  return TG_OK;
}

template <typename T>
int dispatch_rc_linear(const tg_rc_linear_desc* d, const RcLinearParams& p, hipStream_t st) {
  switch (d->variant & 255) {
    case 1: return launch_rc_linear<T, 20, 8, 2, 4>(d, p, st);
    case 2: return launch_rc_linear<T, 20, 8, 3, 0>(d, p, st);
    case 3: return launch_rc_linear<T, 20, 8, 3, 4>(d, p, st);
    default: return launch_rc_linear<T, 20, 8, 2, 0>(d, p, st);
  }
}

inline bool rc_dev_enabled() {
#ifdef TG_RC_DEV_BUILD
  static const bool on = []() { const char* e = getenv("TG_RC_DEV"); return e != nullptr && e[0] == '1'; }();
  return on;
#else
  return false;
#endif
}

}

extern "C" int tg_rc_linear(const tg_rc_linear_desc* d, void* stream) {
  TG_CHECK(d != nullptr, TG_ERR_ARG, "tg_rc_linear: null descriptor");
  TG_CHECK(d->dtype == TG_BF16 || d->dtype == TG_F16, TG_ERR_ARG, "tg_rc_linear: dtype %d", d->dtype);
  TG_CHECK(d->K == 320, TG_ERR_ARG, "tg_rc_linear: K = %d (320: the token row lives in registers; the K = 640 variant of round 4 was removed)", d->K);
  TG_CHECK(d->N > 0 && d->N % 64 == 0, TG_ERR_ARG, "tg_rc_linear: N = %d must be a positive multiple of 64", d->N);
  TG_CHECK(d->variant >= 0 && ((d->variant >> 8) == 0 || rc_dev_enabled()), TG_ERR_ARG, "tg_rc_linear: variant %d carries dev bits (TG_RC_DEV=1 enables them)", d->variant);
  TG_CHECK(d->M > 0 && d->x && d->wpk && d->out, TG_ERR_ARG, "tg_rc_linear: null operand or M <= 0");
  TG_CHECK(d->ldx >= d->K && d->ldx % 8 == 0 && d->ldc >= d->N && d->ldc % 8 == 0, TG_ERR_ARG, "tg_rc_linear: row pitches must be multiples of 8 elements");
  TG_CHECK(!d->res || (d->ldres >= d->N && d->ldres % 8 == 0), TG_ERR_ARG, "tg_rc_linear: residual pitch");
    RcLinearParams p;
  p.x = d->x; p.ldx = d->ldx; p.wpk = d->wpk; p.res = d->res; p.ldres = d->ldres;
  p.out = d->out; p.ldc = d->ldc; p.M = d->M; p.N = d->N; p.K = d->K; p.ln_eps = d->ln_eps; p.dbg = d->variant >> 8;
  hipStream_t st = reinterpret_cast<hipStream_t>(stream);
  if (d->dtype == TG_BF16) return dispatch_rc_linear<bf16_t>(d, p, st);
  return dispatch_rc_linear<f16_t>(d, p, st);
}

extern "C" int tg_rc_xattn(const tg_rc_xattn_desc* d, void* stream) {
  TG_CHECK(d != nullptr, TG_ERR_ARG, "tg_rc_xattn: null descriptor");
  TG_CHECK(d->dtype == TG_BF16 || d->dtype == TG_F16, TG_ERR_ARG, "tg_rc_xattn: dtype %d", d->dtype);
  TG_CHECK(d->h && d->wq && d->kv && d->wo && d->out && d->M > 0, TG_ERR_ARG, "tg_rc_xattn: null operand or M <= 0");
  TG_CHECK(d->text_len == 77 || (rc_dev_enabled() && d->text_len > 0 && (d->text_len & 255) == 77), TG_ERR_ARG,
           "tg_rc_xattn: %d text keys (built for CLIP's 77; the high bits are dev switches, TG_RC_DEV=1)", d->text_len);
  TG_CHECK(d->ip_tokens == 0 || d->ip_tokens == 4 || d->ip_tokens == 16, TG_ERR_ARG, "tg_rc_xattn: %d image tokens (0, 4 or 16)", d->ip_tokens);
  TG_CHECK(d->rows_per_batch > 0 && d->rows_per_batch % 128 == 0 && d->M % d->rows_per_batch == 0, TG_ERR_ARG,
           "tg_rc_xattn: rows_per_batch = %d must be a multiple of 128 that divides M (a workgroup's 128 tokens share one key set)", d->rows_per_batch);
  TG_CHECK(d->ldh >= 320 && d->ldh % 8 == 0 && d->ldc >= 320 && d->ldc % 8 == 0, TG_ERR_ARG, "tg_rc_xattn: row pitches");
  RcXattnParams p;
  p.h = d->h; p.ldh = d->ldh; p.wq = d->wq; p.kv = d->kv; p.wo = d->wo; p.out = d->out; p.ldc = d->ldc; p.M = d->M;
  p.rows_per_batch = d->rows_per_batch; p.ln_eps = d->ln_eps; p.ip_scale = d->ip_scale; p.dbg = d->text_len >> 8;
  hipStream_t st = reinterpret_cast<hipStream_t>(stream);
  if (d->dtype == TG_BF16) return dispatch_rc_xattn<bf16_t>(d, p, st);
  return dispatch_rc_xattn<f16_t>(d, p, st);
}

extern "C" int tg_rc_kv_pack(int32_t dtype, int32_t batch, const void* k, const void* vt, int64_t ldt, int32_t text_len, const void* kip,
                             const void* vtip, int64_t ldi, int32_t ip_tokens, void* out, void* stream) {
  TG_CHECK(dtype == TG_BF16 || dtype == TG_F16, TG_ERR_ARG, "tg_rc_kv_pack: dtype %d", dtype);
  TG_CHECK(batch > 0 && k && vt && out, TG_ERR_ARG, "tg_rc_kv_pack: null operand");
  TG_CHECK(text_len > 0 && text_len <= 80 && ip_tokens >= 0 && ip_tokens <= 16 && (ip_tokens == 0 || (kip && vtip)), TG_ERR_ARG,
           "tg_rc_kv_pack: %d text keys (<= 80), %d image keys (<= 16)", text_len, ip_tokens);
  hipStream_t st = reinterpret_cast<hipStream_t>(stream);
  const unsigned grid = (unsigned)batch * 8 * 24;
  if (dtype == TG_BF16)
    hipLaunchKernelGGL(rc_kv_pack_kernel<bf16_t>, dim3(grid), dim3(64), 0, st, (const bf16_t*)k, (const bf16_t*)vt, (long)ldt,
                       (const bf16_t*)kip, (const bf16_t*)vtip, (long)ldi, text_len, ip_tokens, (bf16_t*)out);
  else
    hipLaunchKernelGGL(rc_kv_pack_kernel<f16_t>, dim3(grid), dim3(64), 0, st, (const f16_t*)k, (const f16_t*)vt, (long)ldt,
                       (const f16_t*)kip, (const f16_t*)vtip, (long)ldi, text_len, ip_tokens, (f16_t*)out);
  TG_LAUNCH_CHECK();
  return TG_OK;
}

extern "C" int tg_rc_ff(const tg_rc_ff_desc* d, void* stream) {
  TG_CHECK(d != nullptr, TG_ERR_ARG, "tg_rc_ff: null descriptor");
  TG_CHECK(d->dtype == TG_BF16 || d->dtype == TG_F16, TG_ERR_ARG, "tg_rc_ff: dtype %d", d->dtype);
  TG_CHECK(d->h && d->w1 && d->w2 && d->b2 && d->out && d->M > 0, TG_ERR_ARG, "tg_rc_ff: null operand or M <= 0");
  TG_CHECK(d->inner >= 64 && d->inner % 64 == 0, TG_ERR_ARG, "tg_rc_ff: inner = %d must be a multiple of 64", d->inner);
  TG_CHECK(d->ldh >= 320 && d->ldh % 8 == 0 && d->ldc >= 320 && d->ldc % 8 == 0, TG_ERR_ARG, "tg_rc_ff: row pitches");
  TG_CHECK(!d->wpo || (d->res0 && d->ldres >= 320 && d->ldres % 8 == 0), TG_ERR_ARG, "tg_rc_ff: proj_out needs its residual");
  TG_CHECK(d->dbg == 0 || rc_dev_enabled(), TG_ERR_ARG, "tg_rc_ff: dbg = %d (dev switches need TG_RC_DEV=1)", d->dbg);
  RcFfParams p;
  p.h = d->h; p.ldh = d->ldh; p.w1 = d->w1; p.w2 = d->w2; p.b2 = d->b2; p.wpo = d->wpo; p.res0 = d->res0; p.ldres = d->ldres;
  p.out = d->out; p.ldc = d->ldc; p.M = d->M; p.n_slices = d->inner / 32; p.ln_eps = d->ln_eps; p.dbg = d->dbg;
  hipStream_t st = reinterpret_cast<hipStream_t>(stream);
  if (d->dtype == TG_BF16) return launch_rc_ff<bf16_t>(d, p, st);
  return launch_rc_ff<f16_t>(d, p, st);
}

extern "C" int tg_rc_front(const tg_rc_front_desc* d, void* stream) {
  TG_CHECK(d != nullptr, TG_ERR_ARG, "tg_rc_front: null descriptor");
  TG_CHECK(d->dtype == TG_BF16 || d->dtype == TG_F16, TG_ERR_ARG, "tg_rc_front: dtype %d", d->dtype);
  TG_CHECK(d->x && d->coef && d->win && d->wqkv && d->y && d->qk && d->vt && d->M > 0, TG_ERR_ARG, "tg_rc_front: null operand or M <= 0");
  TG_CHECK(d->rows_per_batch > 0 && d->rows_per_batch % 128 == 0 && d->M % d->rows_per_batch == 0, TG_ERR_ARG,
           "tg_rc_front: rows_per_batch = %d must be a multiple of 128 that divides M", d->rows_per_batch);
  TG_CHECK(d->ldx >= 320 && d->ldx % 8 == 0 && d->ldy >= 320 && d->ldy % 8 == 0 && d->ldqk >= 640 && d->ldqk % 8 == 0 && d->ldt >= d->rows_per_batch,
           TG_ERR_ARG, "tg_rc_front: row pitches");
  TG_CHECK(d->dbg == 0 || rc_dev_enabled(), TG_ERR_ARG, "tg_rc_front: dbg = %d (dev switches need TG_RC_DEV=1)", d->dbg);
  RcFrontParams p;
  p.x = d->x; p.ldx = d->ldx; p.coef = d->coef; p.win = d->win; p.wqkv = d->wqkv; p.y = d->y; p.ldy = d->ldy; p.qk = d->qk; p.ldqk = d->ldqk;
  p.vt = d->vt; p.ldt = d->ldt; p.M = d->M; p.rows_per_batch = d->rows_per_batch; p.ln_eps = d->ln_eps; p.dbg = d->dbg;
  hipStream_t st = reinterpret_cast<hipStream_t>(stream);
  if (d->dtype == TG_BF16) return launch_rc_front<bf16_t>(d, p, st);
  return launch_rc_front<f16_t>(d, p, st);
}
```

theatergen_amd/ops.py:

```python
import ctypes as C
import os

import torch

from . import _lib
from ._lib import ACT_GELU, ACT_NONE, ACT_QUICK_GELU, ACT_SILU, AttnDesc, GemmDesc

_workspaces = {}


def _dt(t):
    if t.dtype == torch.bfloat16:
        return _lib.TG_BF16
    if t.dtype == torch.float16:
        return _lib.TG_F16
    raise RuntimeError(f"theatergen_amd: unsupported activation dtype {t.dtype} (bf16 / fp16 only)")


def _stream():
    return torch.cuda.current_stream().cuda_stream


def _ptr(t):
    return None if t is None else t.data_ptr()


def _need_cuda(t):
    if not t.is_cuda:
        raise RuntimeError("theatergen_amd: tensors must live on the GPU (no CPU fallback)")


_ws_slot = 0


class workspace_slot:

    def __init__(self, slot):
        self.slot = int(slot)

    def __enter__(self):
        global _ws_slot
        self._prev, _ws_slot = _ws_slot, self.slot

    def __exit__(self, *exc):
        global _ws_slot
        _ws_slot = self._prev
        return False


def workspace(nbytes, device):
    key = (device.index, "ws", _ws_slot)
    buf = _workspaces.get(key)
    if buf is None or buf.numel() * 4 < nbytes:
        buf = torch.empty(max(int(nbytes) // 4 + 1, 1 << 20), dtype=torch.float32, device=device)
        _workspaces[key] = buf
    return buf


def gemm(a0, w, M, N, K, *, mode=0, a1=None, c0=None, c1=0, conv=None, bias=None, bvec=None, rows_per_batch=0,
         res=None, act=ACT_NONE, out_scale=1.0, out=None, n_split=0, out_t=None, ldt=0, force_split_k=0, force_tile=0,
         a_rows_per_batch=0, a_batch_stride=0, geglu=False, pad_mode=0, a_coef=None, a_silu=False, plan_only=False, ln=None, lda=0, ldw=0,
         gn_out=None):
    _need_cuda(a0)
    L = _lib.lib()
    d = GemmDesc()
    d.dtype = _dt(a0)
    d.mode = mode
    d.a0, d.a1 = _ptr(a0), _ptr(a1)
    d.c0 = int(c0 if c0 is not None else (K if mode == 0 else K // 9))
    d.c1 = int(c1)
    if conv is not None:
        d.batch, d.in_h, d.in_w, d.out_h, d.out_w, d.stride, d.upsample = [int(v) for v in conv]
    d.w = _ptr(w)
    d.M, d.N, d.K = int(M), int(N), int(K)
    d.bias = _ptr(bias)
    d.bvec = _ptr(bvec)
    d.ldbvec = int(bvec.stride(0)) if bvec is not None else 0
    d.rows_per_batch = int(rows_per_batch)
    d.res = _ptr(res)
    d.ldres = int(res.stride(0)) if res is not None else 0
    d.act = act
    d.geglu = 1 if geglu else 0
    d.out_scale = float(out_scale)
    n_main = n_split if n_split > 0 else (N // 2 if geglu else N)
    if out is None:
        out = torch.empty((M, n_main), dtype=a0.dtype, device=a0.device)
    d.out = _ptr(out)
    d.ldc = int(out.stride(0))
    d.n_split = int(n_split)
    d.out_t = _ptr(out_t)
    d.ldt = int(ldt)
    d.force_split_k = force_split_k
    d.force_tile = force_tile
    d.a_rows_per_batch, d.a_batch_stride = int(a_rows_per_batch), int(a_batch_stride)
    d.pad_mode = int(pad_mode)
    d.a_coef = _ptr(a_coef)
    d.a_silu = 1 if a_silu else 0
    d.lda, d.ldw = int(lda), int(ldw)
    if ln is not None:
        d.ln_u, d.ln_v, d.ln_eps = _ptr(ln[0]), _ptr(ln[1]), float(ln[2])
        if len(ln) > 3 and ln[3] is not None:
            if ln[3].dtype != torch.float32 or ln[3].numel() != 2 * M or not ln[3].is_contiguous():
                raise RuntimeError("gemm: ln rows must be the contiguous fp32 [M, 2] tensor of layernorm_stats")
            d.ln_rows = _ptr(ln[3])
    if gn_out is not None and not plan_only:
        d.out_gn_groups = int(gn_out["groups"])
        nb = L.tg_gemm_gn_partial_blocks(C.byref(d))
        if nb > 0:
            gn_out["partials"] = torch.empty((int(conv[0]), nb, d.out_gn_groups, 2), dtype=torch.float32, device=a0.device)
            gn_out["nblk"] = nb
            d.out_gn_partials = gn_out["partials"].data_ptr()
        else:
            d.out_gn_groups = 0
    if plan_only:
        tm, tn, sp, kk = C.c_int32(), C.c_int32(), C.c_int32(), C.c_int32()
        _lib.check(L.tg_gemm_plan(C.byref(d), C.byref(tm), C.byref(tn), C.byref(sp), C.byref(kk)))
        return tm.value, tn.value, sp.value, kk.value
    need = L.tg_gemm_workspace_bytes(C.byref(d))
    if need < 0:
        _lib.check(-1)
    if need > 0:
        ws = workspace(need, a0.device)
        d.workspace = ws.data_ptr()
        d.workspace_bytes = ws.numel() * 4
    if _gemm_profile is None:
        _lib.check(L.tg_gemm(C.byref(d), _stream()))
        return out
    tm, tn, sp, kk = C.c_int32(), C.c_int32(), C.c_int32(), C.c_int32()
    _lib.check(L.tg_gemm_plan(C.byref(d), C.byref(tm), C.byref(tn), C.byref(sp), C.byref(kk)))
    e0, e1 = torch.cuda.Event(enable_timing=True), torch.cuda.Event(enable_timing=True)
    e0.record()
    _lib.check(L.tg_gemm(C.byref(d), _stream()))
    e1.record()
    if kk.value == 2:
        kname = "conv_halo_kernel<128x128>"
    elif kk.value == 4:
        spp = os.environ.get("TG_SLAB_PP", "3")
        ow = int(conv[4]) if conv is not None else 0
        pw = ow if ow in (16, 32, 64) else (64 if ow % 64 == 0 else 32 if ow % 32 == 0 else 16 if ow % 16 == 0 else 8)
        two_wave = ((pw == 64 and spp != "0") or (pw in (16, 32) and spp not in ("0", "1"))) and (pw == ow or spp not in ("0", "1", "2"))
        kname = ("conv_slab_pp_kernel" if two_wave and int(conv[2]) == ow else "conv_slab_kernel") + f"<{tm.value}x{tn.value}>" + ("+gn" if a_coef is not None else "")
    elif kk.value == 3:
        kname = f"bt_gemm_kernel<{tm.value}x{tn.value}>"
    elif kk.value == 6:
        kname = f"gemm_glds_kernel<plain+ln,{tm.value}x{tn.value}>"
    elif kk.value == 7:
        kname = ("pp160_gemm_kernel" if tn.value == 160 else "pp_gemm_kernel") + f"<{tm.value}x{tn.value}" + (",geglu" if geglu else "") + (",ln" if ln is not None else "") + ">"
    else:
        kname = f"gemm_glds_kernel<{'conv' if mode == 1 else 'plain'},{tm.value}x{tn.value}>"
    _gemm_profile.append(dict(kernel=kname, splits=sp.value,
                              M=int(M), N=int(N), K=int(K), flops=2.0 * M * N * K, events=(e0, e1),
                              has_res=res is not None, n_out=int(n_main if n_split <= 0 else N)))
    return out


_gemm_profile = None


def _profiled(launch, kernel, M, N, K, flops, has_res=False, alg_bytes=None):
    if _gemm_profile is None:
        launch()
        return
    e0, e1 = torch.cuda.Event(enable_timing=True), torch.cuda.Event(enable_timing=True)
    e0.record()
    launch()
    e1.record()
    _gemm_profile.append(dict(kernel=kernel, splits=1, M=int(M), N=int(N), K=int(K), flops=float(flops), events=(e0, e1),
                              has_res=bool(has_res), n_out=int(N), **({"alg_bytes": float(alg_bytes)} if alg_bytes is not None else {})))


def gemm_profile_start():
    global _gemm_profile
    _gemm_profile = []


def gemm_profile_stop():
    global _gemm_profile
    recs, _gemm_profile = _gemm_profile, None
    for r in recs or []:
        e0, e1 = r.pop("events")
        r["ms"] = e0.elapsed_time(e1)
    return recs or []


def linear(x, w, bias=None, **kw):
    M, K = x.shape
    N = w.shape[0]
    if x.stride(0) != K or w.shape[1] != K or w.stride(0) != K:
        assert x.stride(1) == 1 and w.stride(1) == 1 and w.shape[1] == K and x.stride(0) >= K and w.stride(0) >= K
        return gemm(x, w, M, N, K, bias=bias, lda=x.stride(0), ldw=w.stride(0), **kw)
    return gemm(x, w, M, N, K, bias=bias, **kw)


def rc_linear(x, wpk, N, *, res=None, ln_eps=None, out=None, variant=0):
    from ._lib import RcLinearDesc
    _need_cuda(x)
    M, K = x.shape
    assert x.stride(1) == 1 and wpk.dtype == torch.uint8
    if K != 320:
        raise RuntimeError(f"rc_linear: K = {K} (the row-chain projection keeps a 320-channel token row in registers)")
    assert wpk.numel() == (N // 64) * (128 * K + 1024), (wpk.numel(), N, K)
    if out is None:
        out = torch.empty(M, N, dtype=x.dtype, device=x.device)
    d = RcLinearDesc()
    d.dtype = _dt(x)
    d.x, d.ldx, d.wpk = _ptr(x), int(x.stride(0)), _ptr(wpk)
    d.res, d.ldres = (_ptr(res), int(res.stride(0))) if res is not None else (None, 0)
    d.out, d.ldc = _ptr(out), int(out.stride(0))
    d.M, d.N, d.K = int(M), int(N), int(K)
    d.ln, d.ln_eps = (1, float(ln_eps)) if ln_eps is not None else (0, 0.0)
    d.variant = int(variant)
    _profiled(lambda: _lib.check(_lib.lib().tg_rc_linear(C.byref(d), _stream())), "rc_linear_kernel<320>" + ("+ln" if ln_eps is not None else ""),
              M, N, K, 2.0 * M * N * K, res is not None)
    return out


def rc_kv_pack(k, vt, ldt, L, kip, vtip, ldi, T, batch, out=None):
    _need_cuda(k)
    if out is None:
        out = torch.empty((batch, 8, 24 * 512), dtype=k.dtype, device=k.device)
    _lib.check(_lib.lib().tg_rc_kv_pack(_dt(k), int(batch), _ptr(k), _ptr(vt), int(ldt), int(L), _ptr(kip), _ptr(vtip), int(ldi), int(T),
                                       _ptr(out), _stream()))
    return out


def xq_kv_pack(k, vt, ldt, L, kip, vtip, ldi, T, batch, C_, head_dim, out=None):
    _need_cuda(k)
    need = _lib.lib().tg_xq_kv_bytes(int(batch), int(C_), int(head_dim))
    if need < 0:
        raise RuntimeError(f"xq_kv_pack: C = {C_}, head_dim = {head_dim} not supported")
    if out is None:
        out = torch.empty(need, dtype=torch.uint8, device=k.device)
    assert out.numel() == need and out.dtype == torch.uint8
    _lib.check(_lib.lib().tg_xq_kv_pack(_dt(k), int(batch), int(C_), int(head_dim), _ptr(k), _ptr(vt), int(ldt), int(L), _ptr(kip), _ptr(vtip),
                                       int(ldi), int(T), _ptr(out), _stream()))
    return out


def xq_attn(x, wq, ln_u, ln_v, ln_eps, kv, head_dim, rows_per_batch, text_len, ip_tokens, ip_scale=None, out=None):
    from ._lib import XqAttnDesc
    _need_cuda(x)
    M, Cc = x.shape
    assert x.stride(1) == 1 and x.stride(0) == Cc and wq.shape == (Cc, Cc)
    if out is None:
        out = torch.empty(M, Cc, dtype=x.dtype, device=x.device)
    d = XqAttnDesc()
    d.dtype = _dt(x)
    d.x, d.ldx, d.wq = _ptr(x), int(x.stride(0)), _ptr(wq)
    d.ln_u, d.ln_v, d.ln_eps = _ptr(ln_u), _ptr(ln_v), float(ln_eps)
    d.kv, d.ip_scale = _ptr(kv), _ptr(ip_scale)
    d.out, d.ldc = _ptr(out), int(out.stride(0))
    d.M, d.C, d.head_dim, d.rows_per_batch, d.text_len, d.ip_tokens = int(M), int(Cc), int(head_dim), int(rows_per_batch), int(text_len), int(ip_tokens)
    L_ = text_len + ip_tokens
    flops = 2.0 * M * Cc * Cc + 4.0 * M * L_ * Cc
    tile = "128x128" if int(head_dim) == 64 else "128x160"
    _profiled(lambda: _lib.check(_lib.lib().tg_xq_attn(C.byref(d), _stream())), f"gemm_glds_kernel<plain+ln+xattn d{head_dim},{tile}>", M, Cc, Cc, flops,
              alg_bytes=2.0 * (2 * M * Cc + Cc * Cc) + 2.0 * (M // rows_per_batch) * 2 * L_ * Cc)
    return out


def rc_xattn(h, wq, kv, wo, rows_per_batch, ln_eps, ip_tokens, ip_scale=None, out=None, text_len=77):
    from ._lib import RcXattnDesc
    _need_cuda(h)
    M, Cc = h.shape
    assert Cc == 320 and h.stride(1) == 1
    if out is None:
        out = torch.empty(M, 320, dtype=h.dtype, device=h.device)
    d = RcXattnDesc()
    d.dtype = _dt(h)
    d.h, d.ldh = _ptr(h), int(h.stride(0))
    d.wq, d.kv, d.wo = _ptr(wq), _ptr(kv), _ptr(wo)
    d.out, d.ldc = _ptr(out), int(out.stride(0))
    d.M, d.rows_per_batch = int(M), int(rows_per_batch)
    d.text_len, d.ip_tokens = int(text_len), int(ip_tokens)
    d.ln_eps = float(ln_eps)
    d.ip_scale = _ptr(ip_scale)
    _profiled(lambda: _lib.check(_lib.lib().tg_rc_xattn(C.byref(d), _stream())), f"rc_xattn_kernel<77+{int(ip_tokens)}>",
              M, 320, 320, 4.0 * M * 320 * 320 + 4.0 * M * 320 * (int(text_len) + int(ip_tokens)), True,
              alg_bytes=2.0 * (3 * M * 320 + 2 * 320 * 320) + 2.0 * kv.numel())
    return out


def rc_ff(h, w1, w2, b2, inner, ln_eps, wpo=None, res0=None, out=None, dbg=0):
    from ._lib import RcFfDesc
    _need_cuda(h)
    M, Cc = h.shape
    assert Cc == 320 and h.stride(1) == 1
    if out is None:
        out = torch.empty(M, 320, dtype=h.dtype, device=h.device)
    d = RcFfDesc()
    d.dtype = _dt(h)
    d.h, d.ldh = _ptr(h), int(h.stride(0))
    d.w1, d.w2, d.b2, d.wpo = _ptr(w1), _ptr(w2), _ptr(b2), _ptr(wpo)
    d.res0, d.ldres = (_ptr(res0), int(res0.stride(0))) if res0 is not None else (None, 0)
    d.out, d.ldc = _ptr(out), int(out.stride(0))
# ... 287 lines not shown
    qt, kt, dot = transpose(q, batch, n, inner), transpose(k, batch, n, inner), transpose(dout, batch, n, inner)
    stats = torch.empty((batch, heads, n, 2), dtype=torch.float32, device=q.device)
    dq, dk, dv = torch.empty_like(q), torch.empty_like(q), torch.empty_like(q)
    d = _lib.AttnBwdDesc()
    d.dtype, d.batch, d.heads, d.head_dim, d.n = _dt(q), batch, heads, head_dim, n
    d.q, d.k, d.v, d.dout = _ptr(q), _ptr(k), _ptr(v), _ptr(dout)
    d.ld, d.bs = inner, n * inner
    d.qt, d.kt, d.doutt = _ptr(qt), _ptr(kt), _ptr(dot)
    d.t_ld, d.t_bs = n, inner * n
    d.stats = _ptr(stats)
    d.dq, d.dk, d.dv = _ptr(dq), _ptr(dk), _ptr(dv)
    d.scale = float(scale)
    _lib.check(getattr(L, entry)(C.byref(d), _stream()))
    return dq, dk, dv


def attention_bwd_cross(q, dout, k, v, batch, n_q, n_k, heads, head_dim, scale, ds_scale, extra=None):
    return _attention_bwd_cross("tg_attention_bwd_cross", q, dout, k, v, batch, n_q, n_k, heads, head_dim, scale, ds_scale, extra)


def _attention_bwd_cross(entry, q, dout, k, v, batch, n_q, n_k, heads, head_dim, scale, ds_scale, extra):
    _need_cuda(q)
    inner = heads * head_dim
    lp = (n_k + 7) // 8 * 8
    kt = torch.zeros((batch, inner, lp), dtype=q.dtype, device=q.device)
    kt[:, :, :n_k] = k.reshape(batch, n_k, inner).transpose(1, 2)
    stats = torch.empty((batch, heads, n_q, 2), dtype=torch.float32, device=q.device)
    dq = torch.empty_like(q)
    d = _lib.AttnBwdCrossDesc()
    d.dtype, d.batch, d.heads, d.head_dim, d.n_q, d.n_k = _dt(q), batch, heads, head_dim, n_q, n_k
    d.q, d.dout, d.q_ld, d.q_bs = _ptr(q), _ptr(dout), inner, n_q * inner
    d.k, d.v, d.k_ld, d.k_bs = _ptr(k), _ptr(v), inner, n_k * inner
    d.kt, d.t_ld, d.t_bs = _ptr(kt), lp, inner * lp
    if extra is not None:
        if extra.dtype != torch.float32 or extra.shape != (batch, heads, n_q, n_k) or not extra.is_contiguous():
            raise RuntimeError(entry[3:] + ": extra must be a contiguous fp32 [batch, heads, n_q, n_k] tensor")
        d.extra, d.extra_ld = _ptr(extra), n_k
    d.stats, d.dq = _ptr(stats), _ptr(dq)
    d.scale, d.ds_scale = float(scale), float(ds_scale)
    _lib.check(getattr(_lib.lib(), entry)(C.byref(d), _stream()))
    return dq


def attention_bwd_wide_supported(head_dim, n):
    return head_dim % 8 == 0 and 64 < head_dim <= 160 and n % 8 == 0


def attention_bwd_wide(q, k, v, dout, batch, n, heads, head_dim, scale):
    return _attention_bwd("tg_attention_bwd_wide", q, k, v, dout, batch, n, heads, head_dim, scale)


def attention_bwd_cross_wide(q, dout, k, v, batch, n_q, n_k, heads, head_dim, scale, ds_scale, extra=None):
    return _attention_bwd_cross("tg_attention_bwd_cross_wide", q, dout, k, v, batch, n_q, n_k, heads, head_dim, scale, ds_scale, extra)


def transpose(src, batch, rows, cols, out=None):
    if out is None:
        out = torch.empty((batch, cols, rows), dtype=src.dtype, device=src.device)
    _lib.check(_lib.lib().tg_transpose(_dt(src), _ptr(src), batch, rows, cols, _ptr(out), _stream()))
    return out


def conv1x1_nchw(x, weight, bias, in_scale=1.0):
    _need_cuda(x)
    B, cin, h, w = x.shape
    cout = weight.shape[0]
    out = torch.empty((B, cout, h, w), dtype=torch.float32, device=x.device)
    _lib.check(_lib.lib().tg_conv1x1_nchw(_ptr(x), B, cin, cout, h * w, _ptr(weight), _ptr(bias), float(in_scale), _ptr(out), _stream()))
    return out


def softmax_rows(x, scale=1.0, out=None):
    _need_cuda(x)
    rows, cols = x.shape
    if out is None:
        out = torch.empty_like(x)
    _lib.check(_lib.lib().tg_softmax_rows(_dt(x), _ptr(x), rows, cols, x.stride(0), float(scale), _ptr(out), out.stride(0), _stream()))
    return out


_SRC = {torch.bfloat16: 0, torch.float16: 1, torch.float32: 2}


def conv_in(sample, weight_packed, bias, cout, dtype):
    _need_cuda(sample)
    B, cin, h, w = sample.shape
    out = torch.empty((B * h * w, cout), dtype=dtype, device=sample.device)
    _lib.check(_lib.lib().tg_conv_in(_dt(out), _ptr(sample), _SRC[sample.dtype], B, cin, h, w, _ptr(weight_packed), _ptr(bias),
                                     cout, _ptr(out), _stream()))
    return out


def conv_out_takes_gn(cin, h, w, cout):
    return bool(_lib.lib().tg_conv_out_takes_coef(int(cin), int(h), int(w), int(cout)))


def conv_out(x, weight_packed, bias, batch, h, w, cout, out_dtype, coef=None, silu=True):
    cin = x.shape[-1]
    out = torch.empty((batch, cout, h, w), dtype=out_dtype, device=x.device)
    if coef is not None:
        _lib.check(_lib.lib().tg_conv_out_gn(_dt(x), _ptr(x), _ptr(coef), 1 if silu else 0, batch, cin, h, w, _ptr(weight_packed), _ptr(bias), cout,
                                             _ptr(out), 1 if out_dtype == torch.float32 else 0, _stream()))
        return out
    _lib.check(_lib.lib().tg_conv_out(_dt(x), _ptr(x), batch, cin, h, w, _ptr(weight_packed), _ptr(bias), cout, _ptr(out),
                                      1 if out_dtype == torch.float32 else 0, _stream()))
    return out


def timestep_embedding(t_dev, rows, dim, flip_sin_to_cos, freq_shift, dtype, t_stride=0, index=None):
    out = torch.empty((rows, dim), dtype=dtype, device=t_dev.device)
    _lib.check(_lib.lib().tg_timestep_embedding(_dt(out), _ptr(t_dev), _ptr(index), t_stride, rows, dim, 1 if flip_sin_to_cos else 0,
                                                float(freq_shift), _ptr(out), dim, _stream()))
    return out


def step_epilogue(noise_pred, latents, guidance_scale, coef, step_idx, *, has_cfg=True, advance=True, prediction_type=0, frozen=None,
                  frozen_mask=None, frozen_steps=0, history=None, model_in=None):
    n_img = latents.shape[0]
    chw = latents[0].numel()
    hw = latents.shape[-1] * latents.shape[-2]
    mask_per_img = 1 if (frozen_mask is not None and frozen_mask.numel() == n_img * hw and n_img > 1) else 0
    mi_dt = -1 if model_in is None else _SRC[model_in.dtype]
    _lib.check(_lib.lib().tg_step_epilogue(_ptr(noise_pred), _ptr(latents), n_img, chw, hw, 1 if has_cfg else 0, float(guidance_scale), _ptr(coef),
                                           _ptr(step_idx), 1 if advance else 0, prediction_type, _ptr(frozen), _ptr(frozen_mask),
                                           mask_per_img, int(frozen_steps), _ptr(history), _ptr(model_in), mi_dt, _stream()))


def step_epilogue_sigma(noise_pred, latents, guidance_scale, coef, step_idx, *, has_cfg=True, advance=True, noise=None, frozen=None,
                        frozen_mask=None, frozen_steps=0, history=None, model_in=None):
    n_img = latents.shape[0]
    chw = latents[0].numel()
    hw = latents.shape[-1] * latents.shape[-2]
    mask_per_img = 1 if (frozen_mask is not None and frozen_mask.numel() == n_img * hw and n_img > 1) else 0
    mi_dt = -1 if model_in is None else _SRC[model_in.dtype]
    nz_dt = -1 if noise is None else _SRC[noise.dtype]
    _lib.check(_lib.lib().tg_step_epilogue_sigma(_ptr(noise_pred), _ptr(latents), n_img, chw, hw, 1 if has_cfg else 0, float(guidance_scale),
                                                 _ptr(coef), _ptr(step_idx), 1 if advance else 0, _ptr(noise), nz_dt, _ptr(frozen),
                                                 _ptr(frozen_mask), mask_per_img, int(frozen_steps), _ptr(history), _ptr(model_in), mi_dt,
                                                 _stream()))


def pixel_unshuffle(x, factor):
    _need_cuda(x)
    B, ch, h, w = x.shape
    x = x.contiguous()
    out = torch.empty((B * (h // factor) * (w // factor), ch * factor * factor), dtype=x.dtype, device=x.device)
    _lib.check(_lib.lib().tg_pixel_unshuffle(_dt(x), _ptr(x), B, ch, h, w, int(factor), _ptr(out), _stream()))
    return out


def relu(x, out=None):
    if out is None:
        out = torch.empty_like(x)
    _lib.check(_lib.lib().tg_relu(_dt(x), _ptr(x), x.numel(), _ptr(out), _stream()))
    return out


def avgpool2x2(x, batch, h, w):
    ch = x.shape[-1]
    out = torch.empty((batch * ((h + 1) // 2) * ((w + 1) // 2), ch), dtype=x.dtype, device=x.device)
    _lib.check(_lib.lib().tg_avgpool2x2(_dt(x), _ptr(x), batch, h, w, ch, _ptr(out), _stream()))
    return out


def scale_repeat(x, scale, copies, out=None):
    if out is None:
        out = torch.empty((copies * x.shape[0], *x.shape[1:]), dtype=x.dtype, device=x.device)
    _lib.check(_lib.lib().tg_scale_repeat(_dt(x), _ptr(x), x.numel(), float(scale), int(copies), _ptr(out), _stream()))
    return out

# ... 202 lines not shown
```

theatergen_amd/pipelines.py:

```python
import os
import weakref

import torch

from . import ops
from .attention_processor import register_replay_stream, tensor_version, unregister_replay_stream
from .scheduler import DDIMScheduler, EulerAncestralDiscreteScheduler, EulerDiscreteScheduler
from .unet import DeviceSchedule


DEFAULT_GUIDANCE_ATTN_KEYS = [("mid", 0, 0, 0), ("up", 1, 0, 0), ("up", 1, 1, 0), ("up", 1, 2, 0)]


class SDPipe:

    def __init__(self, unet, scheduler=None, controlnet=None):
        self.unet = unet
        self.scheduler = scheduler if scheduler is not None else DDIMScheduler(prediction_type=unet.config.prediction_type)
        self.controlnet = controlnet
        self.vae_scale_factor = 8

    def to(self, device, dtype=None):
        self.unet.to(device=device, dtype=dtype) if dtype is not None else self.unet.to(device)
        return self
# ... 89 lines not shown
                self.adapter_feats, self.graph = None, None
            return
        acts = []
        for f in features:
            if not isinstance(f, _Act):
                b, c, h, w = f.shape
                t = ops.transpose(f.to(self.dt).contiguous(), b, c, h * w).reshape(b * h * w, c)
                f = _Act(t, b, h, w, c)
            if f.b != self.n_img or f.t.dtype != self.dt:
                raise ValueError(f"set_adapter: features must have batch {self.n_img} and dtype {self.dt}")
            acts.append(f)
        geo = [(f.h, f.w, f.c) for f in acts]
        if self.adapter_feats is None or [(f.h, f.w, f.c) for f in self.adapter_feats] != geo:
            self.adapter_feats = [_Act(torch.empty((2 * f.b * f.hw, f.c), dtype=self.dt, device=self.dev), 2 * f.b, f.h, f.w, f.c) for f in acts]
            self.graph = None
        for dst, f in zip(self.adapter_feats, acts):
            ops.scale_repeat(f.t.contiguous(), conditioning_scale, 2, out=dst.t)

    def set_step_noise(self, table):
        if self.kind != "euler_a":
            raise RuntimeError("set_step_noise: only an Euler-ancestral engine draws noise in its step")
        self.step_noise.copy_(table.reshape(self.step_noise.shape))
        self._noise_set = True

    def _refresh_kv(self):
        self.unet.register_conditioning(self.enc)

    def set_frozen(self, frozen_latents, frozen_mask, frozen_steps):
        if self.graph is not None and (self.frozen is None) != (frozen_latents is None):
            self.graph = None
        if frozen_latents is None:
            self.frozen = self.frozen_mask = None
            self.frozen_steps = 0
            return
        if self.frozen is None:
            self.frozen = torch.empty_like(self.history)
            self.frozen_mask = torch.empty((self.n_img, self.h, self.w), dtype=torch.float32, device=self.dev)
        self.frozen.copy_(frozen_latents)
        self.frozen_mask.copy_(frozen_mask.to(torch.float32).expand(self.n_img, self.h, self.w))
        if self.graph is not None and frozen_steps != self.frozen_steps:
            self.graph = None
        self.frozen_steps = int(frozen_steps)

    def _ensure_time_proj(self):
        unet = self.unet
        if unet.config.addition_embed_type is not None or os.environ.get("TG_TPROJ_TABLE", "1") == "0":
            if self._tproj_table is not None:
                self._tproj_table, self._tproj_key, self.graph = None, None, None
            return
        te = unet.time_embedding
        ps = [te.linear_1.weight, te.linear_1.bias, te.linear_2.weight, te.linear_2.bias]
        for r in unet._resnets:
            ps += [r.time_emb_proj.weight, r.time_emb_proj.bias]
        key = tuple((p.data_ptr(), tensor_version(p)) for p in ps) + (self.t_table.data_ptr(), tensor_version(self.t_table), unet.dtype)
        if key == self._tproj_key:
            return
        B = 2 * self.n_img
        idx = torch.zeros(1, dtype=torch.int32, device=self.dev)
        rows = []
        with torch.no_grad(), ops.workspace_slot(self.ws_slot):
            for s in range(self.steps):
                idx.fill_(s)
                rows.append(unet.time_embed(DeviceSchedule(self.t_table, idx), B, None)[1].clone())
        self._tproj_table = torch.stack(rows).contiguous()
        self._tproj_key = key
        self.graph = None

    def _step(self):
        with ops.workspace_slot(self.ws_slot):
            self._step_body()

    def _step_body(self):
        down = mid = None
        if self.controlnet is not None:
            down, mid = self.controlnet(self.model_in, self.sched, self.cn_enc, self.cn_cond, conditioning_scale=self.cn_scale,
                                        return_dict=False, token_major=True)
        tp = None
        if self._tproj_table is not None:
            tp = torch.index_select(self._tproj_table, 0, self.step_idx)[0]
        if self.adapter_feats is not None:
            down = self.adapter_feats
        noise_pred = self.unet(self.model_in, self.sched, self.enc, added_cond_kwargs=self.added, return_dict=False,
                               out_dtype=torch.float32, down_block_additional_residuals=down,
                               mid_block_additional_residual=mid, time_proj=tp)[0]
        if self.kind != "ddim":
            ops.step_epilogue_sigma(noise_pred, self.latents, self.g, self.coef, self.step_idx, advance=True, noise=self.step_noise,
                                    frozen=self.frozen, frozen_mask=self.frozen_mask, frozen_steps=self.frozen_steps, history=self.history,
                                    model_in=self.model_in)
            return
        ops.step_epilogue(noise_pred, self.latents, self.g, self.coef, self.step_idx, advance=True,
                          prediction_type=self.pred_type, frozen=self.frozen,
                          frozen_mask=self.frozen_mask, frozen_steps=self.frozen_steps, history=self.history,
                          model_in=self.model_in)

    def _signature(self):
        return self.frozen is not None, self.frozen_steps, self.g

    def _reset(self, latents):
        self.latents.copy_(latents.to(device=self.dev, dtype=torch.float32))
        self.history[0].copy_(self.latents)
        if self.kind != "ddim":
            x0 = self.latents / self.in_div0
            self.model_in[:self.n_img].copy_(x0)
            self.model_in[self.n_img:].copy_(x0)
            self.step_idx.zero_()
            return
        self.model_in[:self.n_img].copy_(self.latents)
        self.model_in[self.n_img:].copy_(self.latents)
        self.step_idx.zero_()

    def _capture(self):
        s = torch.cuda.Stream(device=self.dev)
        s.wait_stream(torch.cuda.current_stream(self.dev))
        with torch.cuda.stream(s):
            self._step()
        torch.cuda.current_stream(self.dev).wait_stream(s)
        torch.cuda.synchronize(self.dev)
        g = torch.cuda.CUDAGraph()
        with torch.cuda.graph(g):
            self._step()
        self.graph = g

    def _ensure_graph(self, latents):
        self._ensure_time_proj()
        sig = self._signature()
        if self.use_graph and (self.graph is None or sig != self._graph_sig):
            self._reset(latents)
            self._capture()
            self._graph_sig = sig

    @staticmethod
    def run_concurrent(engines, latents_list, before_step=None):
        dev = engines[0].dev
        with torch.no_grad():
            for e, lat in zip(engines, latents_list):
                if not e.use_graph:
                    raise RuntimeError("run_concurrent needs graph engines")
                e._ensure_graph(lat)
            cur = torch.cuda.current_stream(dev)
            streams = [e._stream() for e in engines]
            for e, lat, st in zip(engines, latents_list, streams):
                st.wait_stream(cur)
                with torch.cuda.stream(st):
                    e._reset(lat)
            for i in range(engines[0].steps):
                if before_step is not None:
                    before_step(i)
                for e, st in zip(engines, streams):
                    with torch.cuda.stream(st):
                        e.graph.replay()
            for st in streams:
                cur.wait_stream(st)
        return [e.history for e in engines]

    def _stream(self):
        if getattr(self, "_own_stream", None) is None:
            self._own_stream = register_replay_stream(torch.cuda.Stream(device=self.dev), self.dev)
            weakref.finalize(self, unregister_replay_stream, self._own_stream)
        return self._own_stream

    def run(self, latents, before_step=None):
        if self.kind == "euler_a" and not self._noise_set:
            raise RuntimeError("DenoiseEngine (Euler ancestral): set_step_noise(...) before run(): the step noise is drawn on the host in the reference's order")
        with torch.no_grad():
            self._ensure_graph(latents)
            self._reset(latents)
            for i in range(self.steps):
# ... 323 lines not shown
```

theatergen_amd/rowchain.py:

```python
import math
import os

import torch

from . import ops
from .weights_pack import rc_pack, rc_pack_tiles

ENABLED = os.environ.get("TG_RC", "1") != "0"
MODE = int(os.environ.get("TG_RC_MODE", "15"))
MIN_ROWS = int(os.environ.get("TG_RC_MIN_ROWS", "8192"))
MIN_ROWS_CHAIN = int(os.environ.get("TG_RC_MIN_ROWS_CHAIN", "32768"))
TRACE = os.environ.get("TG_RC_TRACE") == "1"


def trace(*a):
    if TRACE:
        print("[tg_rc]", *a, flush=True)

HEADS, DH, C = 8, 40, 320


def _q_slot_channels():
    out = torch.empty(C, dtype=torch.long)
    for n in range(C):
        c, hi, i, j = n // 64, (n // 32) & 1, (n // 8) & 3, n & 7
        s = 4 * c + i
        m, w5 = s // 5, s % 5
        if w5 == 0:
            head, d = 2 * m, 8 * hi + j
        elif w5 == 1:
            head, d = 2 * m, 16 + 8 * hi + j
        elif w5 == 2:
            head, d = (2 * m, 32 + j) if hi == 0 else (2 * m + 1, j)
        elif w5 == 3:
            head, d = 2 * m + 1, 8 + 8 * hi + j
        else:
            head, d = 2 * m + 1, 24 + 8 * hi + j
        out[n] = head * DH + d
    assert sorted(out.tolist()) == list(range(C))
    return out


def _o_slot_channels():
    out = torch.empty(C, dtype=torch.long)
    for n in range(C):
        c, hi, i, j = n // 64, (n // 32) & 1, (n // 8) & 3, n & 7
        t = 4 * c + i
        m, t5 = t // 5, t % 5
        if t5 in (0, 1):
            head, d = 2 * m, 16 * t5 + 8 * (j >> 2) + 4 * hi + (j & 3)
        elif t5 == 2:
            head, d = (2 * m, 32 + 4 * hi + j) if j < 4 else (2 * m + 1, 32 + 4 * hi + j - 4)
        else:
            head, d = 2 * m + 1, 16 * (t5 - 3) + 8 * (j >> 2) + 4 * hi + (j & 3)
        out[n] = head * DH + d
    assert sorted(out.tolist()) == list(range(C))
    return out


_QS, _OS = None, None



def pack_xattn_q(wq, bq, gamma, beta, scale):
    global _QS
    if _QS is None:
        _QS = _q_slot_channels()
    s = float(scale) * math.log2(math.e)
    w32 = wq.detach().float()
    wp = (w32 * gamma.detach().float()[None, :] * s).to(wq.dtype)
    u = wp.float().sum(dim=1)
    v = w32 @ beta.detach().float()
    if bq is not None:
        v = v + bq.detach().float()
    v = v * s
    perm = _QS.to(wq.device)
    return rc_pack_tiles(wp[perm].contiguous(), v[perm], u[perm])


def pack_xattn_out(wo, bo):
    global _OS
    if _OS is None:
        _OS = _o_slot_channels()
    perm = _OS.to(wo.device)
    w2 = wo.detach()[:, perm].contiguous()
    return rc_pack_tiles(w2, bo.detach().float() if bo is not None else None)


def linear320(x2d, lin_weight, bias, res, owner, name, cached):
    M, K = x2d.shape
    N = lin_weight.shape[0]
    if not ENABLED or x2d.stride(1) != 1 or lin_weight.shape[1] != K:
        return None
    ts = [lin_weight] + ([bias] if bias is not None else [])
    if K == 320 and (MODE & 1) and N % 64 == 0 and M >= MIN_ROWS_CHAIN:
        trace("linear320 yes", name, M, N)
        wpk = cached(owner, "rc_" + name, ts, lambda: rc_pack(lin_weight.detach(), bias.detach().float() if bias is not None else None))
        return ops.rc_linear(x2d, wpk, N, res=res)
    trace("linear_rc no", name, M, K, N)
    return None


def xattn_eligible(attn, C, B, N, L, T, dtype):
    inner = attn.to_q.weight.shape[0]
    return (ENABLED and (MODE & 2) and C == 320 and inner == 320 and int(attn.heads) == 8 and L == 77 and T in (0, 4, 16) and N % 128 == 0
            and B * N >= MIN_ROWS and dtype in (torch.bfloat16, torch.float16) and attn.to_out[0].weight.shape[0] == 320)


def _ff_row_of():
    r = torch.arange(32)
    rho = (r & 3) + 4 * (r >> 3)
    hi = (r >> 2) & 1
    return 16 * hi + rho


def pack_ff(w1, b1, gamma, beta, w2, b2):
    from .weights_pack import _rc_maps
    inner = w2.shape[1]
    assert w1.shape == (2 * inner, C) and w2.shape == (C, inner) and inner % 32 == 0
    dev, dt = w1.device, w1.dtype
    g32, be32 = gamma.detach().float(), beta.detach().float()
    w1f = w1.detach().float()
    w1g = (w1f * g32[None, :]).to(dt)
    v1 = w1f @ be32 + (b1.detach().float() if b1 is not None else 0.0)
    pi, kap = _rc_maps(C)
    kap = kap.to(dev)
    rowoff = _ff_row_of().to(dev)
    ns = inner // 32
    hid = 32 * torch.arange(ns, device=dev)[:, None] + rowoff[None, :]
    rows_a, rows_g = hid, inner + hid
    rows = torch.stack([rows_a, rows_g], dim=1)
    frag = w1g[rows[:, :, None, None, :, None], kap[None, None, :, :, None, :]].contiguous()
    fb = frag.reshape(ns, -1).view(torch.uint8)
    page = torch.zeros(ns, 256, dtype=torch.float32, device=dev)
    acc_ch = (16 * torch.arange(2, device=dev)[:, None] + torch.arange(16, device=dev)[None, :]).reshape(-1)
    page[:, :32] = v1[(32 * torch.arange(ns, device=dev)[:, None] + acc_ch[None, :])]
    page[:, 32:64] = v1[inner + (32 * torch.arange(ns, device=dev)[:, None] + acc_ch[None, :])]
    s1 = torch.cat([fb, page.view(torch.uint8)], dim=1).reshape(-1)
    s1 = torch.cat([s1, torch.zeros(3 * 1024, dtype=torch.uint8, device=dev)])
    out_rows = (64 * torch.arange(C // 64)[:, None, None] + pi[None]).reshape(-1, 32).to(dev)
    kcol = (32 * torch.arange(ns, device=dev)[:, None, None, None] + 16 * torch.arange(2, device=dev)[None, None, :, None]
            + 8 * torch.arange(2, device=dev)[None, :, None, None] + torch.arange(8, device=dev)[None, None, None, :])
    w2d = w2.detach()
    f2 = w2d[out_rows[None, :, None, None, :, None], kcol[:, None, :, :, None, :]].contiguous()
    s2 = f2.reshape(-1).view(torch.uint8)
    bb2 = (b2.detach().float() if b2 is not None else torch.zeros(C, device=dev)).contiguous()
    return s1.contiguous(), s2.contiguous(), bb2
```

theatergen_amd/unet.py:

```python
from types import SimpleNamespace

import os

import torch
import torch.nn as nn

from . import ops
from . import rowchain
from .attention_processor import (tensor_version, Attention, AttnProcessor, CNAttnProcessor, IPAttnProcessor, _cached, front_eligible, fused_cross_block,
                                  ln_weight, self_attention_from_qkv)
from .config import UNetConfig
from .weights_pack import pack_conv1x1, pack_conv3x3, pack_conv3x3_up2, pack_geglu, pack_ln_linear, rc_pack_tiles


class DeviceSchedule:

    def __init__(self, table, index):
        self.table, self.index = table, index


class _Act:
    __slots__ = ("t", "b", "h", "w", "c", "gn")

    def __init__(self, t, b, h, w, c, gn=None):
        self.t, self.b, self.h, self.w, self.c = t, b, h, w, c
        self.gn = gn

    @property
    def hw(self):
        return self.h * self.w


class _Packed:

    def __init__(self):
        self._c = {}

    def get(self, name, tensors, build):
        key = tuple((t.data_ptr(), tensor_version(t), t.dtype, t.device) for t in tensors)
        hit = self._c.get(name)
        if hit is None or hit[0] != key:
            with torch.no_grad():
                hit = (key, build())
            self._c[name] = hit
        return hit[1]


_FUSE_GN = not os.environ.get("TG_NO_GN_FUSE")
_GN_EPI = os.environ.get("TG_GN_EPI", "1") != "0"


def _gn_of(gn, groups):
    return gn if gn is not None and "partials" in gn and gn["groups"] == groups else None
_LN_MODE = 0 if os.environ.get("TG_NO_LN_FUSE") else int(os.environ.get("TG_LN_MODE", "1"))
_LN_FF_MAX_ROWS = int(os.environ.get("TG_LN_FF_MAX_ROWS", "0"))
_CONV_OUT_GN = os.environ.get("TG_CONV_OUT_GN", "1") != "0"
_FF_PAD = os.environ.get("TG_FF_PAD", "1") != "0"
_PP_MODE = int(os.environ.get("TG_PP", "15"))


def _pp_takes_ln(M, N, K):
    if not (_PP_MODE & 4) or M % 256 or K % 64:
        return False
    if N % 256 == 0 and K >= 640:
        tiles = (M // 256) * (N // 256)
        if tiles >= 192 and tiles / (((tiles + 255) // 256) * 256) >= 0.6:
            return True
    if N % 160 == 0 and K >= 640 and (_PP_MODE & 8):
        tiles = (M // 256) * (N // 160)
        return tiles >= 192 and tiles / (((tiles + 255) // 256) * 256) >= 0.74 and (2 * N // 3) % 80 == 0
    return False


_FUSE_LN_MIN_ROWS = int(os.environ.get("TG_LN_FUSE_MIN_ROWS", "2048"))


class ResnetBlock2D(nn.Module):

    def __init__(self, in_channels, out_channels, temb_channels, groups=32, eps=1e-5, output_scale_factor=1.0):
        super().__init__()
        self.in_channels, self.out_channels = in_channels, out_channels
        self.groups, self.eps, self.output_scale_factor = groups, eps, output_scale_factor
        self.norm1 = nn.GroupNorm(groups, in_channels, eps=eps)
        self.conv1 = nn.Conv2d(in_channels, out_channels, 3, padding=1)
        self.time_emb_proj = nn.Linear(temb_channels, out_channels) if temb_channels is not None else None
        self.norm2 = nn.GroupNorm(groups, out_channels, eps=eps)
        self.conv2 = nn.Conv2d(out_channels, out_channels, 3, padding=1)
        self.conv_shortcut = nn.Conv2d(in_channels, out_channels, 1) if in_channels != out_channels else None
        self._p = _Packed()
        self.temb_slot = None

    def run(self, x: _Act, skip: _Act, tproj):
        c1 = skip.c if skip is not None else 0
        assert x.c + c1 == self.in_channels
        w1 = self._p.get("c1", [self.conv1.weight], lambda: pack_conv3x3(self.conv1.weight.detach()))
        w2 = self._p.get("c2", [self.conv2.weight], lambda: pack_conv3x3(self.conv2.weight.detach()))
        x1 = skip.t if skip is not None else None
        kw1 = dict(bias=self.conv1.bias)
        if tproj is not None:
            off, width = self.temb_slot
            kw1.update(bvec=tproj[:, off:off + width], rows_per_batch=x.hw)
        fuse2 = _FUSE_GN and ops.conv3x3_takes_gn(x.t.dtype, x.b, x.h, x.w, self.out_channels, 0, self.out_channels)
        gn1 = {"groups": self.groups} if _GN_EPI and fuse2 else None
        if gn1 is not None:
            kw1.update(gn_out=gn1)
        if _FUSE_GN and ops.conv3x3_takes_gn(x.t.dtype, x.b, x.h, x.w, x.c, c1, self.out_channels):
            g0 = _gn_of(x.gn, self.groups) if skip is None else None
            coef = (ops.groupnorm_from_partials(g0, x.b, x.hw, x.c, self.eps, self.norm1.weight, self.norm1.bias) if g0 is not None else
                    ops.groupnorm_coef(x.t, x.b, x.hw, self.groups, self.eps, self.norm1.weight, self.norm1.bias, x1=x1))
            h = ops.conv3x3(x.t, w1, x.b, x.h, x.w, x.c, x1=x1, c1=c1, a_coef=coef, a_silu=True, **kw1)
        else:
            h = ops.groupnorm(x.t, x.b, x.hw, self.groups, self.eps, self.norm1.weight, self.norm1.bias, silu=True, x1=x1)
            h = ops.conv3x3(h, w1, x.b, x.h, x.w, self.in_channels, **kw1)
        if self.conv_shortcut is not None:
            ws = self._p.get("sc", [self.conv_shortcut.weight], lambda: pack_conv1x1(self.conv_shortcut.weight.detach()))
            res = ops.gemm(x.t, ws, x.b * x.hw, self.out_channels, self.in_channels, a1=skip.t if skip is not None else None,
                           c0=x.c, c1=c1, bias=self.conv_shortcut.bias)
        else:
            res = x.t
        kw2 = dict(bias=self.conv2.bias, res=res, out_scale=1.0 / self.output_scale_factor)
        gn2 = {"groups": self.groups} if _GN_EPI else None
        if gn2 is not None:
            kw2.update(gn_out=gn2)
        if fuse2:
            g1 = _gn_of(gn1, self.groups)
            coef = (ops.groupnorm_from_partials(g1, x.b, x.hw, self.out_channels, self.eps, self.norm2.weight, self.norm2.bias) if g1 is not None else
                    ops.groupnorm_coef(h, x.b, x.hw, self.groups, self.eps, self.norm2.weight, self.norm2.bias))
            out = ops.conv3x3(h, w2, x.b, x.h, x.w, self.out_channels, a_coef=coef, a_silu=True, **kw2)
        else:
            h = ops.groupnorm(h, x.b, x.hw, self.groups, self.eps, self.norm2.weight, self.norm2.bias, silu=True)
            out = ops.conv3x3(h, w2, x.b, x.h, x.w, self.out_channels, **kw2)
        return _Act(out, x.b, x.h, x.w, self.out_channels, gn=_gn_of(gn2, self.groups))


class Downsample2D(nn.Module):

    def __init__(self, channels):
        super().__init__()
        self.conv = nn.Conv2d(channels, channels, 3, stride=2, padding=1)
        self._p = _Packed()

    def run(self, x: _Act, res=None):
        w = self._p.get("w", [self.conv.weight], lambda: pack_conv3x3(self.conv.weight.detach()))
        kw = {} if res is None else dict(res=res)
        out = ops.conv3x3(x.t, w, x.b, x.h, x.w, x.c, stride=2, bias=self.conv.bias, **kw)
        return _Act(out, x.b, (x.h - 1) // 2 + 1, (x.w - 1) // 2 + 1, x.c)


_UP_FOLD = os.environ.get("TG_UP_FOLD", "1") != "0"


class Upsample2D(nn.Module):

    def __init__(self, channels):
        super().__init__()
        self.conv = nn.Conv2d(channels, channels, 3, padding=1)
        self._p = _Packed()

    def run(self, x: _Act):
        if _UP_FOLD and ops.conv_up2_eligible(x.t.dtype, x.b, x.h, x.w, x.c, self.conv.out_channels):
            wf = self._p.get("w_up2", [self.conv.weight], lambda: pack_conv3x3_up2(self.conv.weight.detach()))
            out = ops.conv_up2(x.t, wf, x.b, x.h, x.w, x.c, bias=self.conv.bias)
            return _Act(out, x.b, 2 * x.h, 2 * x.w, x.c)
        w = self._p.get("w", [self.conv.weight], lambda: pack_conv3x3(self.conv.weight.detach()))
        out = ops.conv3x3(x.t, w, x.b, x.h, x.w, x.c, upsample=True, bias=self.conv.bias)
        return _Act(out, x.b, 2 * x.h, 2 * x.w, x.c)


class GEGLU(nn.Module):
    def __init__(self, dim_in, dim_out):
        super().__init__()
        self.proj = nn.Linear(dim_in, dim_out * 2)


class FeedForward(nn.Module):

    def __init__(self, dim, mult=4):
        super().__init__()
        inner = dim * mult
        self.net = nn.ModuleList([GEGLU(dim, inner), nn.Dropout(0.0), nn.Linear(inner, dim)])
        self._p = _Packed()

    def run_fused(self, x2d, norm, tail=None):
        proj, lin2 = self.net[0].proj, self.net[2]
        M, K = x2d.shape
        inner = lin2.weight.shape[1]
        if (not rowchain.ENABLED or not (rowchain.MODE & 4) or K != 320 or lin2.weight.shape[0] != 320 or inner % 64 or M < rowchain.MIN_ROWS_CHAIN
                or x2d.stride(0) != K or proj.weight.shape[0] != 2 * inner):
            return None
        ts = [proj.weight, proj.bias, norm.weight, norm.bias, lin2.weight] + ([lin2.bias] if lin2.bias is not None else [])
        s1, s2, b2 = self._p.get("rc_ff", ts, lambda: rowchain.pack_ff(proj.weight, proj.bias, norm.weight, norm.bias, lin2.weight, lin2.bias))
        wpo = res0 = None
        if tail is not None:
            w_out, b_out, res0 = tail
            wpo = self._p.get("rc_po", [w_out] + ([b_out] if b_out is not None else []),
                              lambda: rc_pack_tiles(w_out.detach(), b_out.detach().float() if b_out is not None else None))
        return ops.rc_ff(x2d, s1, s2, b2, inner, norm.eps, wpo=wpo, res0=res0)

    def _hidden(self, M, inner, like):
        if _FF_PAD and inner % 512 == 0:
            return torch.empty((M, inner + 64), dtype=like.dtype, device=like.device)[:, :inner]
        return torch.empty((M, inner), dtype=like.dtype, device=like.device)

    def _w2(self):
        w2 = self.net[2].weight
        inner = w2.shape[1]
        if not (_FF_PAD and inner % 512 == 0):
            return w2

        def build():
            wp = torch.zeros((w2.shape[0], inner + 64), dtype=w2.dtype, device=w2.device)
            wp[:, :inner] = w2.detach()
            return wp
        return self._p.get("w2pad", [w2], build)[:, :inner]

    def run(self, x2d, residual, ln=None):
        proj = self.net[0].proj
        M, K = x2d.shape
        inner = proj.weight.shape[0] // 2
        if ln is not None:
            norm, rows = ln

            def build():
                wp, bp = pack_geglu(proj.weight.detach(), proj.bias.detach())
                return pack_ln_linear(wp, bp, norm.weight, norm.bias)
            wl, ul, vl = self._p.get("geglu_ln", [proj.weight, proj.bias, norm.weight, norm.bias], build)
            g = ops.gemm(x2d, wl, M, wl.shape[0], K, geglu=True, ln=(ul, vl, norm.eps, rows), out=self._hidden(M, inner, x2d))
        elif M > 64 and inner % 32 == 0:
            wp, bp = self._p.get("geglu", [proj.weight, proj.bias], lambda: pack_geglu(proj.weight.detach(), proj.bias.detach()))
            g = ops.gemm(x2d, wp, M, wp.shape[0], K, bias=bp, geglu=True, out=self._hidden(M, inner, x2d))
        else:
            g = ops.geglu(ops.linear(x2d, proj.weight, proj.bias))
            return ops.linear(g, self.net[2].weight, self.net[2].bias, res=residual)
        return ops.linear(g, self._w2(), self.net[2].bias, res=residual)


class BasicTransformerBlock(nn.Module):

    def __init__(self, dim, heads, dim_head, cross_attention_dim):
        super().__init__()
        self.norm1 = nn.LayerNorm(dim)
        self.attn1 = Attention(query_dim=dim, heads=heads, dim_head=dim_head)
        self.norm2 = nn.LayerNorm(dim)
        self.attn2 = Attention(query_dim=dim, cross_attention_dim=cross_attention_dim, heads=heads, dim_head=dim_head)
        self.norm3 = nn.LayerNorm(dim)
        self.ff = FeedForward(dim)

    @staticmethod
    def _call(attn, x2d, b, n, enc, residual, kwargs, ln=None):
        proc = attn.processor
        ours = isinstance(proc, (AttnProcessor, IPAttnProcessor, CNAttnProcessor))
        if ln is not None and not ours:
            x2d, ln = ops.layernorm(x2d, ln[0].weight, ln[0].bias, ln[0].eps), None
        x3 = x2d.reshape(b, n, -1)
        if isinstance(proc, (AttnProcessor, IPAttnProcessor)) and attn.rescale_output_factor == 1.0 \
                and not attn.residual_connection and not kwargs.get("return_attntion_probs"):
            return proc(attn, x3, encoder_hidden_states=enc, _fused_residual=residual, _fused_ln=ln, **kwargs).reshape(b * n, -1)
        if isinstance(proc, CNAttnProcessor):
            return proc(attn, x3, encoder_hidden_states=enc, _fused_residual=residual, _fused_ln=ln).reshape(b * n, -1)
        if ln is not None:
            x3 = ops.layernorm(x2d, ln[0].weight, ln[0].bias, ln[0].eps).reshape(b, n, -1)
        out = attn(x3, encoder_hidden_states=enc, **kwargs)
        if isinstance(out, tuple):
            out = out[0]
        return ops.add(out.reshape(b * n, -1).contiguous(), residual)

    def run(self, x2d, b, n, enc, ca_kwargs, tail=None, pre_qkv=None):
        M, C = x2d.shape
        if _LN_MODE and M >= _FUSE_LN_MIN_ROWS and C % 64 == 0 and x2d.stride(0) == C:
            def folded(norm, t, n_out=0):
                return (norm, ops.layernorm_stats(t, norm.eps) if (_LN_MODE & 4 or _pp_takes_ln(t.shape[0], n_out, t.shape[1])) else None)
            if _LN_MODE & 1:
                if pre_qkv is not None:
                    x2d = self_attention_from_qkv(self.attn1, pre_qkv[0], pre_qkv[1], pre_qkv[2], b, n, x2d)
                else:
                    x2d = self._call(self.attn1, x2d, b, n, None, x2d, ca_kwargs, ln=folded(self.norm1, x2d, 3 * self.attn1.to_q.weight.shape[0]))
                h2 = fused_cross_block(self.attn2, self.norm2, x2d, b, n, enc, ca_kwargs)
                x2d = h2 if h2 is not None else self._call(self.attn2, x2d, b, n, enc, x2d, ca_kwargs, ln=folded(self.norm2, x2d))
            else:
                h = ops.layernorm(x2d, self.norm1.weight, self.norm1.bias, self.norm1.eps)
                x2d = self._call(self.attn1, h, b, n, None, x2d, ca_kwargs)
                h = ops.layernorm(x2d, self.norm2.weight, self.norm2.bias, self.norm2.eps)
                x2d = self._call(self.attn2, h, b, n, enc, x2d, ca_kwargs)
            fused = self.ff.run_fused(x2d, self.norm3, tail)
            if fused is not None:
                return (fused, True) if tail is not None else fused
            if _LN_MODE & 2 or M <= _LN_FF_MAX_ROWS:
                return self.ff.run(x2d, x2d, ln=folded(self.norm3, x2d))
            h = ops.layernorm(x2d, self.norm3.weight, self.norm3.bias, self.norm3.eps)
            return self.ff.run(h, x2d)
        h = ops.layernorm(x2d, self.norm1.weight, self.norm1.bias, self.norm1.eps)
        x2d = self._call(self.attn1, h, b, n, None, x2d, ca_kwargs)
        h = ops.layernorm(x2d, self.norm2.weight, self.norm2.bias, self.norm2.eps)
        x2d = self._call(self.attn2, h, b, n, enc, x2d, ca_kwargs)
        h = ops.layernorm(x2d, self.norm3.weight, self.norm3.bias, self.norm3.eps)
        return self.ff.run(h, x2d)


class Transformer2DModel(nn.Module):

    def __init__(self, heads, dim_head, in_channels, num_layers, cross_attention_dim, groups, use_linear_projection):
        super().__init__()
        inner = heads * dim_head
        assert inner == in_channels
        self.groups = groups
        self.use_linear_projection = use_linear_projection
        self.norm = nn.GroupNorm(groups, in_channels, eps=1e-6)
        if use_linear_projection:
            self.proj_in = nn.Linear(in_channels, inner)
            self.proj_out = nn.Linear(inner, in_channels)
        else:
            self.proj_in = nn.Conv2d(in_channels, inner, 1)
            self.proj_out = nn.Conv2d(inner, in_channels, 1)
        self.transformer_blocks = nn.ModuleList(
            [BasicTransformerBlock(inner, heads, dim_head, cross_attention_dim) for _ in range(num_layers)])
        self._p = _Packed()

    def _w(self, name, mod):
        if self.use_linear_projection:
            return mod.weight
        return self._p.get(name, [mod.weight], lambda: pack_conv1x1(mod.weight.detach()))

    def _front(self, x, w_in, ca_kwargs):
        blk = self.transformer_blocks[0]
        M, C = x.t.shape
        if (not rowchain.ENABLED or not (rowchain.MODE & 8) or not _LN_MODE & 1 or C != 320 or w_in.shape != (320, 320) or M < rowchain.MIN_ROWS_CHAIN
                or x.hw % 128 or x.t.stride(0) != C or x.c != 320 or not front_eligible(blk.attn1, ca_kwargs)):
            return None
        g = _gn_of(x.gn, self.groups)
        coef = (ops.groupnorm_from_partials(g, x.b, x.hw, x.c, 1e-6, self.norm.weight, self.norm.bias) if g is not None else
                ops.groupnorm_coef(x.t, x.b, x.hw, self.groups, 1e-6, self.norm.weight, self.norm.bias))
        bin_ = self.proj_in.bias
        win = self._p.get("rc_front_in", [w_in] + ([bin_] if bin_ is not None else []),
                          lambda: rc_pack_tiles(w_in.detach(), bin_.detach().float() if bin_ is not None else None))
        wl, ul, vl = ln_weight(blk.attn1, "qkv", blk.norm1)
        wqkv = self._p.get("rc_front_qkv", [wl, ul, vl], lambda: rc_pack_tiles(wl, vl, ul))
        return ops.rc_front(x.t, coef, win, wqkv, x.hw, blk.norm1.eps)

    def run(self, x: _Act, enc, ca_kwargs):
        w_in = self._w("in", self.proj_in)
        pre = self._front(x, w_in, ca_kwargs)
        if pre is not None:
            y, pre = pre[0], pre[1:]
        else:
            g = _gn_of(x.gn, self.groups)
            y = (ops.groupnorm_from_partials(g, x.b, x.hw, x.c, 1e-6, self.norm.weight, self.norm.bias, x=x.t) if g is not None else
                 ops.groupnorm(x.t, x.b, x.hw, self.groups, 1e-6, self.norm.weight, self.norm.bias, silu=False))
            y_in = rowchain.linear320(y, w_in, self.proj_in.bias, None, self, "proj_in", _cached)
            y = y_in if y_in is not None else ops.linear(y, w_in, self.proj_in.bias)
        base_key = list(ca_kwargs.get("attn_key", [])) if "attn_key" in ca_kwargs else None
        w_out = self._w("out", self.proj_out)
        last = len(self.transformer_blocks) - 1
        for i, blk in enumerate(self.transformer_blocks):
            if base_key is not None:
                ca_kwargs["attn_key"] = base_key + [i]
            y = blk.run(y, x.b, x.hw, enc, ca_kwargs, tail=(w_out, self.proj_out.bias, x.t) if i == last else None,
                        pre_qkv=pre if i == 0 else None)
            if isinstance(y, tuple):
                return _Act(y[0], x.b, x.h, x.w, x.c)
        out = rowchain.linear320(y, w_out, self.proj_out.bias, x.t, self, "proj_out", _cached)
        if out is None:
            out = ops.linear(y, w_out, self.proj_out.bias, res=x.t)
        return _Act(out, x.b, x.h, x.w, x.c)


class _Block(nn.Module):
    def __init__(self):
        super().__init__()
        self.resnets = nn.ModuleList()
        self.has_cross_attention = False


class TimestepEmbedding(nn.Module):
    def __init__(self, in_dim, dim):
        super().__init__()
        self.linear_1 = nn.Linear(in_dim, dim)
        self.linear_2 = nn.Linear(dim, dim)

    def run(self, x2d):
        h = ops.linear(x2d, self.linear_1.weight, self.linear_1.bias, act=ops.ACT_SILU)
        return ops.linear(h, self.linear_2.weight, self.linear_2.bias)


class UNet2DConditionOutput(SimpleNamespace):
    pass


class UNet2DConditionModel(nn.Module):
    def __init__(self, config: UNetConfig = None, **kw):
        super().__init__()
        cfg = config if config is not None else UNetConfig(**kw)
        self.config = cfg
        boc = tuple(cfg.block_out_channels)
        nb = len(boc)
        ted = cfg.time_embed_dim
        heads_t = cfg.per_block(cfg.attention_head_dim)
        tl_t = cfg.per_block(cfg.transformer_layers_per_block)
        lpb = cfg.per_block(cfg.layers_per_block)
        g, eps, ctx, lin = cfg.norm_num_groups, cfg.norm_eps, cfg.cross_attention_dim, cfg.use_linear_projection

        self.conv_in = nn.Conv2d(cfg.in_channels, boc[0], 3, padding=1)
        self.time_embedding = TimestepEmbedding(boc[0], ted)
        if cfg.addition_embed_type == "text_time":
            self.add_embedding = TimestepEmbedding(cfg.projection_class_embeddings_input_dim, ted)
        elif cfg.addition_embed_type is not None:
            raise ValueError(f"addition_embed_type {cfg.addition_embed_type} unsupported")

        def tfm(c, heads, layers):
            return Transformer2DModel(heads, c // heads, c, layers, ctx, g, lin)

        self.down_blocks = nn.ModuleList()
        self.up_blocks = nn.ModuleList()
        out_c = boc[0]
        for i, bt in enumerate(cfg.down_block_types):
            in_c, out_c = out_c, boc[i]
            blk = _Block()
            if bt == "CrossAttnDownBlock2D":
                blk.has_cross_attention = True
                blk.attentions = nn.ModuleList()
            elif bt != "DownBlock2D":
                raise ValueError(f"unknown down block {bt}")
            for j in range(lpb[i]):
                blk.resnets.append(ResnetBlock2D(in_c if j == 0 else out_c, out_c, ted, g, eps))
                if blk.has_cross_attention:
                    blk.attentions.append(tfm(out_c, heads_t[i], tl_t[i]))
            blk.downsamplers = nn.ModuleList([Downsample2D(out_c)]) if i != nb - 1 else None
            self.down_blocks.append(blk)

        mid = _Block()
        mid.has_cross_attention = True
        mid.resnets.append(ResnetBlock2D(boc[-1], boc[-1], ted, g, eps))
        mid.attentions = nn.ModuleList([tfm(boc[-1], heads_t[-1], tl_t[-1])])
        mid.resnets.append(ResnetBlock2D(boc[-1], boc[-1], ted, g, eps))
        self.mid_block = mid

        rboc, rheads, rtl, rlpb = tuple(reversed(boc)), tuple(reversed(heads_t)), tuple(reversed(tl_t)), tuple(reversed(lpb))
        out_c = rboc[0]
        for i, bt in enumerate(cfg.up_block_types):
            prev_out, out_c = out_c, rboc[i]
            in_c = rboc[min(i + 1, nb - 1)]
            blk = _Block()
            if bt == "CrossAttnUpBlock2D":
                blk.has_cross_attention = True
                blk.attentions = nn.ModuleList()
            elif bt != "UpBlock2D":
                raise ValueError(f"unknown up block {bt}")
# ... 27 lines not shown

    @property
    def device(self):
        return self.conv_in.weight.device

    @property
    def attn_processors(self):
        procs = {}
        for name, m in self.named_modules():
            if isinstance(m, Attention):
                procs[f"{name}.processor"] = m.processor
        return procs

    def set_attn_processor(self, processor):
        attns = {f"{n}.processor": m for n, m in self.named_modules() if isinstance(m, Attention)}
        if isinstance(processor, dict):
            if len(processor) != len(attns):
                raise ValueError(f"A dict of processors was passed, but the number of processors {len(processor)} does not match "
                                 f"the number of attention layers: {len(attns)}. Please make sure to pass {len(attns)} processor classes.")
            for k, m in attns.items():
                m.set_processor(processor[k])
        else:
            for m in attns.values():
                m.set_processor(processor)

    def set_default_attn_processor(self):
        self.set_attn_processor(AttnProcessor())

    def register_conditioning(self, encoder_hidden_states):
        enc = encoder_hidden_states
        if enc.dtype != self.dtype or not enc.is_contiguous():
            enc = enc.to(self.dtype).contiguous()
        for m in self.modules():
            if isinstance(m, Attention) and isinstance(m.processor, IPAttnProcessor):
                m.processor.register_static(m, enc)
        return enc

    def _timestep_dev(self, timestep, B):
        dev = self.device
        if isinstance(timestep, DeviceSchedule):
            return timestep.table, 0
        if torch.is_tensor(timestep):
            t = timestep
            if t.device != dev or t.dtype != torch.float32:
                t = t.to(device=dev, dtype=torch.float32)
            t = t.reshape(-1)
            return t, (1 if t.numel() == B and B > 1 else 0)
        key = float(timestep)
        if key not in self._t_cache:
            self._t_cache[key] = torch.tensor([key], dtype=torch.float32, device=dev)
        return self._t_cache[key], 0

    def _tproj_weight(self):
        ws = [r.time_emb_proj.weight for r in self._resnets]
        bs = [r.time_emb_proj.bias for r in self._resnets]
        return self._p.get("tproj", ws + bs, lambda: (torch.cat([w.detach() for w in ws], 0).contiguous(),
                                                       torch.cat([b.detach() for b in bs], 0).contiguous()))

    def time_embed(self, timestep, B, added_cond_kwargs=None):
        cfg = self.config
        dt = self.dtype
        t, stride = self._timestep_dev(timestep, B)
        index = timestep.index if isinstance(timestep, DeviceSchedule) else None
        t_emb = ops.timestep_embedding(t, B, cfg.block_out_channels[0], cfg.flip_sin_to_cos, cfg.freq_shift, dt, t_stride=stride,
                                       index=index)
        emb = self.time_embedding.run(t_emb)
        if cfg.addition_embed_type == "text_time":
            if added_cond_kwargs is None or "text_embeds" not in added_cond_kwargs or "time_ids" not in added_cond_kwargs:
                raise ValueError("addition_embed_type 'text_time' requires `text_embeds` and `time_ids` in `added_cond_kwargs`")
            text_embeds = added_cond_kwargs["text_embeds"].to(dt)
            time_ids = added_cond_kwargs["time_ids"].to(device=self.device, dtype=torch.float32).contiguous()
            n_ids = time_ids.shape[1]
            d_add = cfg.addition_time_embed_dim
            add_in = torch.empty((B, text_embeds.shape[1] + n_ids * d_add), dtype=dt, device=self.device)
            add_in[:, :text_embeds.shape[1]].copy_(text_embeds)
            te = ops.timestep_embedding(time_ids.reshape(-1), B * n_ids, d_add, True, 0.0, dt, t_stride=1)
            add_in[:, text_embeds.shape[1]:].copy_(te.reshape(B, n_ids * d_add))
            aug = ops.linear(add_in, self.add_embedding.linear_1.weight, self.add_embedding.linear_1.bias, act=ops.ACT_SILU)
            emb = ops.linear(aug, self.add_embedding.linear_2.weight, self.add_embedding.linear_2.bias, res=emb)
        w, b = self._tproj_weight()
        tproj = ops.linear(ops.act(emb, ops.ACT_SILU), w, b)
        return emb, tproj

    def _residual(self, act: _Act, extra):
        if isinstance(extra, _Act):
            if (extra.b, extra.h, extra.w, extra.c) != (act.b, act.h, act.w, act.c):
                raise ValueError("ControlNet residual geometry mismatch")
            return _Act(ops.add(act.t, extra.t), act.b, act.h, act.w, act.c)
        e = extra.to(act.t.dtype).contiguous()
        e_tok = ops.transpose(e, act.b, act.c, act.hw).reshape(act.b * act.hw, act.c)
        return _Act(ops.add(act.t, e_tok), act.b, act.h, act.w, act.c)

    @staticmethod
    def _same_geometry(act: _Act, extra):
        if isinstance(extra, _Act):
            return (extra.b, extra.h, extra.w, extra.c) == (act.b, act.h, act.w, act.c)
        return tuple(extra.shape) == (act.b, act.c, act.h, act.w)

    def _token_major(self, act: _Act, extra):
        if not self._same_geometry(act, extra):
            got = (extra.b, extra.c, extra.h, extra.w) if isinstance(extra, _Act) else tuple(extra.shape)
            raise ValueError(f"T2I-Adapter feature shape {got} does not match the UNet activation {(act.b, act.c, act.h, act.w)}")
        if isinstance(extra, _Act):
            return extra.t
        e = extra.to(act.t.dtype).contiguous()
        return ops.transpose(e, act.b, act.c, act.hw).reshape(act.b * act.hw, act.c)

    def _adapter_add(self, act: _Act, extra):
        return _Act(ops.add(act.t, self._token_major(act, extra)), act.b, act.h, act.w, act.c)

    def forward(self, sample, timestep, encoder_hidden_states, class_labels=None, timestep_cond=None, attention_mask=None,
                cross_attention_kwargs=None, added_cond_kwargs=None, down_block_additional_residuals=None,
                mid_block_additional_residual=None, encoder_attention_mask=None, return_dict=True, out_dtype=None, time_proj=None):
        cfg = self.config
        if attention_mask is not None or encoder_attention_mask is not None or class_labels is not None or timestep_cond is not None:
            raise NotImplementedError("attention masks / class labels / timestep_cond are not on the TheaterGen hot path")
        if not sample.is_cuda:
            raise RuntimeError("theatergen_amd UNet runs on the GPU only (no CPU fallback)")
        dt = self.dtype
        B, _, H, W = sample.shape
        enc = encoder_hidden_states
        if enc.dtype != dt:
            enc = enc.to(dt)
        enc = enc.contiguous()
        ca_kwargs = {} if cross_attention_kwargs is None else cross_attention_kwargs
        track_keys = cross_attention_kwargs is not None

        if time_proj is not None:
            if tuple(time_proj.shape) != (B, self._tproj_width) or time_proj.dtype != dt or time_proj.stride(1) != 1:
                raise ValueError(f"time_proj must be a [{B}, {self._tproj_width}] {dt} tensor of time_embed(...)[1]")
            tproj = time_proj
        else:
            _, tproj = self.time_embed(timestep, B, added_cond_kwargs)

        w_in = self._p.get("conv_in", [self.conv_in.weight], lambda: pack_conv3x3(self.conv_in.weight.detach()))
        x = _Act(ops.conv_in(sample.contiguous(), w_in, self.conv_in.bias, cfg.block_out_channels[0], dt), B, H, W,
                 cfg.block_out_channels[0])

        is_controlnet = mid_block_additional_residual is not None and down_block_additional_residuals is not None
        is_adapter = mid_block_additional_residual is None and down_block_additional_residuals is not None
        feats = list(down_block_additional_residuals) if is_adapter else []
        res = [x]
        for i, blk in enumerate(self.down_blocks):
            cross_feat = feats.pop(0) if blk.has_cross_attention and feats else None
            last = len(blk.resnets) - 1
            for j, resnet in enumerate(blk.resnets):
                x = resnet.run(x, None, tproj)
                if blk.has_cross_attention:
                    if track_keys:
                        ca_kwargs["attn_key"] = ["down", i, j]
                    x = blk.attentions[j].run(x, enc, ca_kwargs)
                    if j == last and cross_feat is not None:
                        x = self._adapter_add(x, cross_feat)
                res.append(x)
            plain_feat = feats.pop(0) if not blk.has_cross_attention and feats else None
            if blk.downsamplers is not None:
                ds = blk.downsamplers[0]
                if plain_feat is not None:
                    out_geom = _Act(x.t, x.b, (x.h - 1) // 2 + 1, (x.w - 1) // 2 + 1, x.c)
                    x = ds.run(x, res=self._token_major(out_geom, plain_feat))
                else:
                    x = ds.run(x)
                res.append(x)
            elif plain_feat is not None:
                x = self._adapter_add(x, plain_feat)
                res[-1] = x

        if is_controlnet:
            if len(down_block_additional_residuals) != len(res):
                raise ValueError("down_block_additional_residuals length mismatch")
            res = [self._residual(r, e) for r, e in zip(res, down_block_additional_residuals)]

        x = self.mid_block.resnets[0].run(x, None, tproj)
        if track_keys:
            ca_kwargs["attn_key"] = ["mid", 0, 0]
        x = self.mid_block.attentions[0].run(x, enc, ca_kwargs)
        x = self.mid_block.resnets[1].run(x, None, tproj)
        if feats and self._same_geometry(x, feats[0]):
            x = self._adapter_add(x, feats.pop(0))
        if mid_block_additional_residual is not None:
            x = self._residual(x, mid_block_additional_residual)

        for i, blk in enumerate(self.up_blocks):
            for j, resnet in enumerate(blk.resnets):
                skip = res.pop()
                x = resnet.run(x, skip, tproj)
                if blk.has_cross_attention:
                    if track_keys:
                        ca_kwargs["attn_key"] = ["up", i, j]
                    x = blk.attentions[j].run(x, enc, ca_kwargs)
            if blk.upsamplers is not None:
                x = blk.upsamplers[0].run(x)

        w_out = self._p.get("conv_out", [self.conv_out.weight], lambda: pack_conv3x3(self.conv_out.weight.detach()))
        odt = out_dtype if out_dtype is not None else dt
        if _CONV_OUT_GN and ops.conv_out_takes_gn(x.t.shape[-1], x.h, x.w, cfg.out_channels):
            coef = ops.groupnorm_coef(x.t, x.b, x.hw, cfg.norm_num_groups, cfg.norm_eps, self.conv_norm_out.weight, self.conv_norm_out.bias)
            out = ops.conv_out(x.t, w_out, self.conv_out.bias, B, x.h, x.w, cfg.out_channels, odt, coef=coef, silu=True)
        else:
            y = ops.groupnorm(x.t, x.b, x.hw, cfg.norm_num_groups, cfg.norm_eps, self.conv_norm_out.weight, self.conv_norm_out.bias,
                              silu=True)
            out = ops.conv_out(y, w_out, self.conv_out.bias, B, x.h, x.w, cfg.out_channels, odt)
        if not return_dict:
            return (out,)
        return UNet2DConditionOutput(sample=out)

    __call__ = forward

    @classmethod
    def from_state_dict(cls, config, state_dict, device="cuda", dtype=torch.bfloat16, ip_adapter=True, num_tokens=4, ip_scale=1.0):
        return _load_on_meta(lambda: _with_ip(cls(config), ip_adapter, num_tokens, ip_scale), state_dict, device, dtype)


def _with_ip(m, ip_adapter, num_tokens, ip_scale):
    if ip_adapter:
        install_ip_processors(m, num_tokens=num_tokens, scale=ip_scale)
    return m


def _load_on_meta(build, state_dict, device, dtype):
    with torch.device("meta"):
        m = build()
    missing, unexpected = m.load_state_dict(state_dict, strict=False, assign=True)
    if unexpected or missing:
        raise RuntimeError(f"state dict mismatch: missing {missing[:5]}... unexpected {unexpected[:5]}...")
    left = [n for n, t in list(m.named_parameters()) + list(m.named_buffers()) if t.is_meta]
    if left:
        raise RuntimeError(f"state dict does not cover {left[:5]}... (constructed on the meta device)")
    m = m.to(device=device, dtype=dtype)
    src = {t.data_ptr() for t in state_dict.values() if torch.is_tensor(t)}
    with torch.no_grad():
        for t in list(m.parameters()) + list(m.buffers()):
            if t.data_ptr() in src:
                t.data = t.data.clone()
# ... 22 lines not shown
```

Measured before the change: 9.668 char_images/s.

## Share CFG-identical prefix computation across the two batch halves in the first down block

Adds a shared_pair mode in which the UNet computes the first resnet and the first transformer block's self-attention only once for half the batch, then writes the result to both halves. This covers the conditional and unconditional CFG halves, which share the latent and the timestep. conv_in, rc_linear and gemm gain dup-offset or pair_out paths that store the duplicate rows directly, and a new dup_rows kernel handles the other cases. The goal is to skip redundant work at the highest-resolution stage before cross-attention makes the two halves differ. The cost is extra duplicate writes and more complex control flow, and it only activates when the caller passes shared_pair and the _CFG_SHARE flag is on.

After: 9.889 char_images/s, median of 6. 2.3% higher.

```diff
diff --git a/include/theatergen_hip.h b/include/theatergen_hip.h
--- a/include/theatergen_hip.h
+++ b/include/theatergen_hip.h
@@ -72,6 +72,7 @@
 int tg_gemm_plan(const tg_gemm_desc* d, int32_t* tile_m, int32_t* tile_n, int32_t* splits, int32_t* kernel_kind);
 int tg_gemm_gn_partial_blocks(const tg_gemm_desc* d);
 
+
 int tg_conv_up2_eligible(const tg_gemm_desc* d);
 int tg_conv_up2(const tg_gemm_desc* d, void* stream);
 
@@ -142,6 +143,7 @@
 int tg_geglu(int32_t dtype, const void* x, int64_t rows, int64_t inner, void* out, void* stream);
 int tg_act(int32_t dtype, const void* x, int64_t n, int32_t act, void* out, void* stream);
 int tg_add(int32_t dtype, const void* a, const void* b, int64_t n, void* out, void* stream);
+int tg_dup_rows(const void* src, void* dst, int64_t rows, int64_t cols, int64_t ld, int32_t dtype, void* stream);
 
 int tg_transpose(int32_t dtype, const void* src, int32_t batch, int32_t rows, int32_t cols, void* dst, void* stream);
 
@@ -152,6 +154,9 @@
 
 int tg_conv_in(int32_t dtype, const void* sample, int32_t src_dtype, int32_t batch, int32_t cin, int32_t h, int32_t w,
                const void* weight, const void* bias, int32_t cout, void* out, void* stream);
+int tg_conv_in_dup(int32_t dtype, const void* sample, int32_t src_dtype, int32_t batch, int32_t cin, int32_t h, int32_t w,
+                   const void* weight, const void* bias, int32_t cout, void* out, int64_t dup_offset, void* stream);
+int tg_conv_in_takes_dup(int32_t cin, int32_t cout);
 int tg_conv_out(int32_t dtype, const void* x, int32_t batch, int32_t cin, int32_t h, int32_t w, const void* weight,
                 const void* bias, int32_t cout, void* out, int32_t out_f32, void* stream);
 int tg_conv_out_gn(int32_t dtype, const void* x, const float* coef, int32_t a_silu, int32_t batch, int32_t cin, int32_t h, int32_t w,
@@ -242,6 +247,7 @@
   const float* u640;
 } tg_rc_linear_desc;
 int tg_rc_linear(const tg_rc_linear_desc* d, void* stream);
+int tg_rc_linear_dup(const tg_rc_linear_desc* d, int64_t c_dup_offset, void* stream);
 
 typedef struct {
   int32_t dtype;
diff --git a/theatergen_amd/_lib.py b/theatergen_amd/_lib.py
--- a/theatergen_amd/_lib.py
+++ b/theatergen_amd/_lib.py
@@ -140,6 +140,7 @@
     "tg_groupnorm_coef": (i32, [i32, vp, vp, i32, i32, i32, i64, i32, f32, vp, vp, vp, vp, vp]),
     "tg_groupnorm_from_partials": (i32, [i32, vp, i32, i32, i64, i32, f32, vp, vp, i32, vp, vp, vp, i32, vp]),
     "tg_gemm_gn_partial_blocks": (i32, [C.POINTER(GemmDesc)]),
+    "tg_dup_rows": (i32, [vp, vp, i64, i64, i64, i32, vp]),
     "tg_conv_up2_eligible": (i32, [C.POINTER(GemmDesc)]),
     "tg_conv_up2": (i32, [C.POINTER(GemmDesc), vp]),
     "tg_geglu": (i32, [i32, vp, i64, i64, vp, vp]),
@@ -149,6 +150,8 @@
     "tg_conv1x1_nchw": (i32, [vp, i32, i32, i32, i64, vp, vp, f32, vp, vp]),
     "tg_softmax_rows": (i32, [i32, vp, i64, i32, i64, f32, vp, i64, vp]),
     "tg_conv_in": (i32, [i32, vp, i32, i32, i32, i32, i32, vp, vp, i32, vp, vp]),
+    "tg_conv_in_dup": (i32, [i32, vp, i32, i32, i32, i32, i32, vp, vp, i32, vp, i64, vp]),
+    "tg_conv_in_takes_dup": (i32, [i32, i32]),
     "tg_conv_out": (i32, [i32, vp, i32, i32, i32, i32, vp, vp, i32, vp, i32, vp]),
     "tg_conv_out_gn": (i32, [i32, vp, vp, i32, i32, i32, i32, i32, vp, vp, i32, vp, i32, vp]),
     "tg_conv_out_takes_coef": (i32, [i32, i32, i32, i32]),
@@ -176,6 +179,7 @@
     "tg_softmax_bwd_rows": (i32, [i32, vp, i32, i64, vp, i64, vp, i64, i64, i32, f32, vp, vp, i64, vp]),
     "tg_sumpool2x2": (i32, [i32, vp, i32, i32, i32, i32, vp, vp]),
     "tg_rc_linear": (i32, [C.POINTER(RcLinearDesc), vp]),
+    "tg_rc_linear_dup": (i32, [C.POINTER(RcLinearDesc), i64, vp]),
     "tg_rc_xattn": (i32, [C.POINTER(RcXattnDesc), vp]),
     "tg_rc_kv_pack": (i32, [i32, i32, vp, vp, i64, i32, vp, vp, i64, i32, vp, vp]),
     "tg_rc_ff": (i32, [C.POINTER(RcFfDesc), vp]),
@@ -205,7 +209,11 @@
         for name, (res, args) in SIGNATURES.items():
             if compat and not hasattr(h, name):
                 continue
-            fn = getattr(h, name)
+            try:
+                fn = getattr(h, name)
+            except AttributeError:
+                raise RuntimeError(f"theatergen_amd: {LIB_PATH} (ABI version {got}) does not export {name}: "
+                                   "rebuild with `python -m theatergen_amd.build`") from None
             fn.restype = res
             fn.argtypes = args
         if got != ABI_VERSION and not compat:
diff --git a/theatergen_amd/attention_processor.py b/theatergen_amd/attention_processor.py
--- a/theatergen_amd/attention_processor.py
+++ b/theatergen_amd/attention_processor.py
@@ -284,15 +284,35 @@
     return hidden_states.contiguous().reshape(b * n, c), b, n, c, None
 
 
+_pair = None
+
+
+class pair_output:
+
+    def __enter__(self):
+        global _pair
+        self._prev, _pair = _pair, {"full": None}
+        return _pair
+
+    def __exit__(self, *exc):
+        global _pair
+        _pair = self._prev
+        return False
+
+
 def _finish(attn, o2d, B, N, C, shape4, x_tokens, fused_residual):
     res = fused_residual
     if res is None and attn.residual_connection:
         res = x_tokens
     out = None
+    kw = {}
+    if _pair is not None and _pair["full"] is None and shape4 is None:
+        _pair["full"] = torch.empty((2 * o2d.shape[0], attn.to_out[0].weight.shape[0]), dtype=o2d.dtype, device=o2d.device)
+        kw = dict(pair_out=_pair["full"])
     if attn.rescale_output_factor == 1.0:
-        out = rowchain.linear320(o2d, attn.to_out[0].weight, attn.to_out[0].bias, res, attn, "to_out", _cached)
+        out = rowchain.linear320(o2d, attn.to_out[0].weight, attn.to_out[0].bias, res, attn, "to_out", _cached, **kw)
     if out is None:
-        out = ops.linear(o2d, attn.to_out[0].weight, attn.to_out[0].bias, res=res, out_scale=1.0 / attn.rescale_output_factor)
+        out = ops.linear(o2d, attn.to_out[0].weight, attn.to_out[0].bias, res=res, out_scale=1.0 / attn.rescale_output_factor, **kw)
     if shape4 is not None:
         b, c, h, w = shape4
         return ops.transpose(out, b, h * w, c).reshape(b, c, h, w)
diff --git a/theatergen_amd/csrc/tg_elementwise.hip b/theatergen_amd/csrc/tg_elementwise.hip
--- a/theatergen_amd/csrc/tg_elementwise.hip
+++ b/theatergen_amd/csrc/tg_elementwise.hip
@@ -381,7 +381,7 @@
 
 template <typename T>
 __global__ __launch_bounds__(256) void conv_in_mfma_kernel(const void* sample, int src_dtype, int batch, int h, int w, const T* weight, const T* bias,
-                                                           int cout, T* out) {
+                                                           int cout, T* out, long dup) {
   typedef typename Vec<T>::v8 V8;
   typedef typename Vec<T>::v4 V4;
   constexpr int CIN = 4, K = 36, KP = 48, WP = 56, OP = 168;
@@ -449,7 +449,10 @@
       for (int it = 0; it < 10; ++it) {
         const int q = it * 64 + lane, px = q / 20, cn = q - px * 20;
         const V8 v = *reinterpret_cast<const V8*>(so + px * OP + cn * 8);
-        if (base + px < npix) *reinterpret_cast<V8*>(out + (base + px) * cout + half * 160 + cn * 8) = v;
+        if (base + px < npix) {
+          *reinterpret_cast<V8*>(out + (base + px) * cout + half * 160 + cn * 8) = v;
+          if (dup != 0) *reinterpret_cast<V8*>(out + (base + px) * cout + half * 160 + cn * 8 + dup) = v;
+        }
       }
       __builtin_amdgcn_wave_barrier();
       asm volatile("s_waitcnt lgkmcnt(0)" ::: "memory");
@@ -718,15 +721,62 @@
   return TG_OK;
 }
 
+namespace {
+bool conv_in_mfma_ok(int cin, int cout) {
+  static const bool mfma_on = [] { const char* e = getenv("TG_CONV_IN_MFMA"); return !(e && e[0] == '0'); }();
+  return mfma_on && cin == 4 && cout > 0 && cout % 160 == 0 && cout <= 640;
+}
+
+template <typename T>
+__global__ __launch_bounds__(256) void dup_rows_kernel(const T* src, T* dst, long rows, int cols8, long ld) {
+  typedef typename Vec<T>::v8 V8;
+  const long n = rows * cols8;
+  for (long i = (long)blockIdx.x * 256 + threadIdx.x; i < n; i += (long)gridDim.x * 256) {
+    const long r = i / cols8;
+    const int c = (int)(i - r * cols8);
+    *reinterpret_cast<V8*>(dst + (r * cols8 + c) * 8) = *reinterpret_cast<const V8*>(src + r * ld + c * 8);
+  }
+}
+}
+
+extern "C" int tg_dup_rows(const void* src, void* dst, int64_t rows, int64_t cols, int64_t ld, int32_t dtype, void* stream) {
+  TG_CHECK((dtype == TG_BF16 || dtype == TG_F16) && src && dst && rows > 0 && cols > 0, TG_ERR_ARG, "tg_dup_rows: bad args");
+  TG_CHECK(cols % 8 == 0 && ld % 8 == 0 && ld >= cols && cols < (1LL << 31), TG_ERR_ARG, "tg_dup_rows: cols = %lld and ld = %lld must be multiples of 8 with ld >= cols",
+           (long long)cols, (long long)ld);
+  TG_CHECK((reinterpret_cast<uintptr_t>(src) & 15) == 0 && (reinterpret_cast<uintptr_t>(dst) & 15) == 0, TG_ERR_ARG, "tg_dup_rows: src / dst must be 16-byte aligned");
+  {
+    const char* s0 = reinterpret_cast<const char*>(src);
+    const char* d0 = reinterpret_cast<const char*>(dst);
+    const long sb = ((rows - 1) * ld + cols) * 2, db = rows * cols * 2;
+    TG_CHECK(s0 + sb <= d0 || d0 + db <= s0, TG_ERR_ARG, "tg_dup_rows: src and dst overlap");
+  }
+  hipStream_t st = reinterpret_cast<hipStream_t>(stream);
+  const int grid = grid_for(rows * cols, 8);
+  if (dtype == TG_BF16) hipLaunchKernelGGL(dup_rows_kernel<bf16_t>, dim3(grid), dim3(256), 0, st, (const bf16_t*)src, (bf16_t*)dst, (long)rows, (int)(cols / 8), (long)ld);
+  else hipLaunchKernelGGL(dup_rows_kernel<f16_t>, dim3(grid), dim3(256), 0, st, (const f16_t*)src, (f16_t*)dst, (long)rows, (int)(cols / 8), (long)ld);
+  TG_LAUNCH_CHECK();
+  return TG_OK;
+}
+
+extern "C" int tg_conv_in_takes_dup(int32_t cin, int32_t cout) { return conv_in_mfma_ok(cin, cout) ? 1 : 0; }
+
 extern "C" int tg_conv_in(int32_t dtype, const void* sample, int32_t src_dtype, int32_t batch, int32_t cin, int32_t h,
                           int32_t w, const void* weight, const void* bias, int32_t cout, void* out, void* stream) {
+  return tg_conv_in_dup(dtype, sample, src_dtype, batch, cin, h, w, weight, bias, cout, out, 0, stream);
+}
+
+extern "C" int tg_conv_in_dup(int32_t dtype, const void* sample, int32_t src_dtype, int32_t batch, int32_t cin, int32_t h,
+                              int32_t w, const void* weight, const void* bias, int32_t cout, void* out, int64_t dup_offset, void* stream) {
   TG_CHECK((dtype == TG_BF16 || dtype == TG_F16) && sample && weight && out, TG_ERR_ARG, "tg_conv_in: bad args");
   TG_CHECK(src_dtype >= 0 && src_dtype <= 2 && batch > 0 && cin > 0 && cin <= 16 && cout > 0, TG_ERR_ARG, "tg_conv_in: bad shape");
   hipStream_t st = reinterpret_cast<hipStream_t>(stream);
   const long npix = (long)batch * h * w;
   {
-    static const bool mfma_on = [] { const char* e = getenv("TG_CONV_IN_MFMA"); return !(e && e[0] == '0'); }();
-    if (mfma_on && cin == 4 && cout % 160 == 0 && cout <= 640 && (reinterpret_cast<uintptr_t>(out) & 15) == 0 && (reinterpret_cast<uintptr_t>(weight) & 7) == 0) {
+    const bool mfma = conv_in_mfma_ok(cin, cout) && (reinterpret_cast<uintptr_t>(out) & 15) == 0 && (reinterpret_cast<uintptr_t>(weight) & 7) == 0;
+    TG_CHECK(dup_offset == 0 || (mfma && dup_offset % 8 == 0 && dup_offset >= npix * cout), TG_ERR_ARG,
+             "tg_conv_in_dup: dup_offset = %lld needs the matrix-core kernel (tg_conv_in_takes_dup, aligned out / weight) and a multiple of 8 past the first destination",
+             (long long)dup_offset);
+    if (mfma) {
       const size_t lds = ((size_t)cout * 56 + 4 * 32 * 168) * 2;
       long nb = (npix + 127) / 128;
       if (nb > 1024) nb = 1024;
@@ -734,12 +784,12 @@
         auto k = conv_in_mfma_kernel<bf16_t>;
         static const hipError_t attr = hipFuncSetAttribute(reinterpret_cast<const void*>(k), hipFuncAttributeMaxDynamicSharedMemorySize, 160 * 1024);
         (void)attr;
-        hipLaunchKernelGGL(k, dim3((unsigned)nb), dim3(256), lds, st, sample, src_dtype, batch, h, w, (const bf16_t*)weight, (const bf16_t*)bias, cout, (bf16_t*)out);
+        hipLaunchKernelGGL(k, dim3((unsigned)nb), dim3(256), lds, st, sample, src_dtype, batch, h, w, (const bf16_t*)weight, (const bf16_t*)bias, cout, (bf16_t*)out, (long)dup_offset);
       } else {
         auto k = conv_in_mfma_kernel<f16_t>;
         static const hipError_t attr = hipFuncSetAttribute(reinterpret_cast<const void*>(k), hipFuncAttributeMaxDynamicSharedMemorySize, 160 * 1024);
         (void)attr;
-        hipLaunchKernelGGL(k, dim3((unsigned)nb), dim3(256), lds, st, sample, src_dtype, batch, h, w, (const f16_t*)weight, (const f16_t*)bias, cout, (f16_t*)out);
+        hipLaunchKernelGGL(k, dim3((unsigned)nb), dim3(256), lds, st, sample, src_dtype, batch, h, w, (const f16_t*)weight, (const f16_t*)bias, cout, (f16_t*)out, (long)dup_offset);
       }
       TG_LAUNCH_CHECK();
       return TG_OK;
diff --git a/theatergen_amd/csrc/tg_rowchain.hip b/theatergen_amd/csrc/tg_rowchain.hip
--- a/theatergen_amd/csrc/tg_rowchain.hip
+++ b/theatergen_amd/csrc/tg_rowchain.hip
@@ -26,6 +26,7 @@
   int N, K;
   float ln_eps;
   int dbg;
+  long c_dup;
 };
 
 template <typename V>
@@ -166,6 +167,11 @@
 #pragma unroll
       for (int i = 0; i < 4; ++i)
         if (mok[i]) *reinterpret_cast<V8*>(outp + mrow[i] * p.ldc + pend_ch + 8 * qb) = pend[i];
+      if (p.c_dup != 0) {
+#pragma unroll
+        for (int i = 0; i < 4; ++i)
+          if (mok[i]) *reinterpret_cast<V8*>(outp + mrow[i] * p.ldc + pend_ch + 8 * qb + p.c_dup) = pend[i];
+      }
     }
     const long ch0 = 64 * (long)c + 32 * hi;
     V8 r8[4];
@@ -242,6 +248,11 @@
 #pragma unroll
     for (int i = 0; i < 4; ++i)
       if (mok[i]) *reinterpret_cast<V8*>(outp + mrow[i] * p.ldc + pend_ch + 8 * qb) = pend[i];
+    if (p.c_dup != 0) {
+#pragma unroll
+      for (int i = 0; i < 4; ++i)
+        if (mok[i]) *reinterpret_cast<V8*>(outp + mrow[i] * p.ldc + pend_ch + 8 * qb + p.c_dup) = pend[i];
+    }
   }
 }
 
@@ -1318,7 +1329,9 @@
 
 }
 
-extern "C" int tg_rc_linear(const tg_rc_linear_desc* d, void* stream) {
+extern "C" int tg_rc_linear(const tg_rc_linear_desc* d, void* stream) { return tg_rc_linear_dup(d, 0, stream); }
+
+extern "C" int tg_rc_linear_dup(const tg_rc_linear_desc* d, int64_t c_dup_offset, void* stream) {
   TG_CHECK(d != nullptr, TG_ERR_ARG, "tg_rc_linear: null descriptor");
   TG_CHECK(d->dtype == TG_BF16 || d->dtype == TG_F16, TG_ERR_ARG, "tg_rc_linear: dtype %d", d->dtype);
   TG_CHECK(d->K == 320, TG_ERR_ARG, "tg_rc_linear: K = %d (320: the token row lives in registers; the K = 640 variant of round 4 was removed)", d->K);
@@ -1327,7 +1340,10 @@
   TG_CHECK(d->M > 0 && d->x && d->wpk && d->out, TG_ERR_ARG, "tg_rc_linear: null operand or M <= 0");
   TG_CHECK(d->ldx >= d->K && d->ldx % 8 == 0 && d->ldc >= d->N && d->ldc % 8 == 0, TG_ERR_ARG, "tg_rc_linear: row pitches must be multiples of 8 elements");
   TG_CHECK(!d->res || (d->ldres >= d->N && d->ldres % 8 == 0), TG_ERR_ARG, "tg_rc_linear: residual pitch");
+  TG_CHECK(c_dup_offset == 0 || (c_dup_offset % 8 == 0 && c_dup_offset >= (d->M - 1) * d->ldc + d->N), TG_ERR_ARG,
+           "tg_rc_linear_dup: c_dup_offset = %lld must be a multiple of 8 elements past the first destination", (long long)c_dup_offset);
     RcLinearParams p;
+  p.c_dup = (long)c_dup_offset;
   p.x = d->x; p.ldx = d->ldx; p.wpk = d->wpk; p.res = d->res; p.ldres = d->ldres;
   p.out = d->out; p.ldc = d->ldc; p.M = d->M; p.N = d->N; p.K = d->K; p.ln_eps = d->ln_eps; p.dbg = d->variant >> 8;
   hipStream_t st = reinterpret_cast<hipStream_t>(stream);
diff --git a/theatergen_amd/ops.py b/theatergen_amd/ops.py
--- a/theatergen_amd/ops.py
+++ b/theatergen_amd/ops.py
@@ -60,8 +60,12 @@
 def gemm(a0, w, M, N, K, *, mode=0, a1=None, c0=None, c1=0, conv=None, bias=None, bvec=None, rows_per_batch=0,
          res=None, act=ACT_NONE, out_scale=1.0, out=None, n_split=0, out_t=None, ldt=0, force_split_k=0, force_tile=0,
          a_rows_per_batch=0, a_batch_stride=0, geglu=False, pad_mode=0, a_coef=None, a_silu=False, plan_only=False, ln=None, lda=0, ldw=0,
-         gn_out=None):
+         gn_out=None, pair_out=None):
     _need_cuda(a0)
+    if pair_out is not None:
+        if out is not None or n_split > 0 or geglu or pair_out.shape != (2 * M, N) or not pair_out.is_contiguous() or pair_out.dtype != a0.dtype:
+            raise RuntimeError("gemm: pair_out must be the only output, a dense [2 M, N] tensor of the activation dtype")
+        out = pair_out[:M]
     L = _lib.lib()
     d = GemmDesc()
     d.dtype = _dt(a0)
@@ -123,14 +127,18 @@
         ws = workspace(need, a0.device)
         d.workspace = ws.data_ptr()
         d.workspace_bytes = ws.numel() * 4
+    def launch():
+        _lib.check(L.tg_gemm(C.byref(d), _stream()))
+        if pair_out is not None:
+            dup_rows(out, pair_out[M:])
     if _gemm_profile is None:
-        _lib.check(L.tg_gemm(C.byref(d), _stream()))
+        launch()
         return out
     tm, tn, sp, kk = C.c_int32(), C.c_int32(), C.c_int32(), C.c_int32()
     _lib.check(L.tg_gemm_plan(C.byref(d), C.byref(tm), C.byref(tn), C.byref(sp), C.byref(kk)))
     e0, e1 = torch.cuda.Event(enable_timing=True), torch.cuda.Event(enable_timing=True)
     e0.record()
-    _lib.check(L.tg_gemm(C.byref(d), _stream()))
+    launch()
     e1.record()
     if kk.value == 2:
         kname = "conv_halo_kernel<128x128>"
@@ -192,10 +200,24 @@
     return gemm(x, w, M, N, K, bias=bias, **kw)
 
 
-def rc_linear(x, wpk, N, *, res=None, ln_eps=None, out=None, variant=0):
+def dup_rows(src, dst):
+    _need_cuda(src)
+    rows, cols = src.shape
+    if src.stride(1) != 1 or dst.shape != src.shape or not dst.is_contiguous() or dst.dtype != src.dtype:
+        raise RuntimeError("dup_rows: src [rows, cols] with unit column stride, dst a dense tensor of the same shape and dtype")
+    _lib.check(_lib.lib().tg_dup_rows(_ptr(src), _ptr(dst), int(rows), int(cols), int(src.stride(0)), _dt(src), _stream()))
+    return dst
+
+
+def rc_linear(x, wpk, N, *, res=None, ln_eps=None, out=None, variant=0, pair_out=None):
     from ._lib import RcLinearDesc
     _need_cuda(x)
     M, K = x.shape
+    if pair_out is not None:
+        if out is not None or pair_out.shape != (2 * M, N) or not pair_out.is_contiguous() or pair_out.dtype != x.dtype:
+            raise RuntimeError("rc_linear: pair_out must be the only output, a dense [2 M, N] tensor of the activation dtype")
+        out = pair_out[:M]
+    dup = int(M) * int(N) if pair_out is not None else 0
     assert x.stride(1) == 1 and wpk.dtype == torch.uint8
     if K != 320:
         raise RuntimeError(f"rc_linear: K = {K} (the row-chain projection keeps a 320-channel token row in registers)")
@@ -210,7 +232,8 @@
     d.M, d.N, d.K = int(M), int(N), int(K)
     d.ln, d.ln_eps = (1, float(ln_eps)) if ln_eps is not None else (0, 0.0)
     d.variant = int(variant)
-    _profiled(lambda: _lib.check(_lib.lib().tg_rc_linear(C.byref(d), _stream())), "rc_linear_kernel<320>" + ("+ln" if ln_eps is not None else ""),
+    _profiled(lambda: _lib.check(_lib.lib().tg_rc_linear_dup(C.byref(d), dup, _stream()) if dup else _lib.lib().tg_rc_linear(C.byref(d), _stream())),
+              "rc_linear_kernel<320>" + ("+ln" if ln_eps is not None else ""),
               M, N, K, 2.0 * M * N * K, res is not None)
     return out
 
@@ -664,10 +687,20 @@
 _SRC = {torch.bfloat16: 0, torch.float16: 1, torch.float32: 2}
 
 
-def conv_in(sample, weight_packed, bias, cout, dtype):
+def conv_in(sample, weight_packed, bias, cout, dtype, pair=False):
     _need_cuda(sample)
     B, cin, h, w = sample.shape
     out = torch.empty((B * h * w, cout), dtype=dtype, device=sample.device)
+    if pair:
+        L = _lib.lib()
+        hb, rows = B // 2, (B // 2) * h * w
+        if L.tg_conv_in_takes_dup(cin, cout) and out.data_ptr() % 16 == 0 and weight_packed.data_ptr() % 8 == 0:
+            _lib.check(L.tg_conv_in_dup(_dt(out), _ptr(sample), _SRC[sample.dtype], hb, cin, h, w, _ptr(weight_packed), _ptr(bias), cout, _ptr(out),
+                                        rows * cout, _stream()))
+        else:
+            _lib.check(L.tg_conv_in(_dt(out), _ptr(sample), _SRC[sample.dtype], hb, cin, h, w, _ptr(weight_packed), _ptr(bias), cout, _ptr(out), _stream()))
+            dup_rows(out[:rows], out[rows:])
+        return out
     _lib.check(_lib.lib().tg_conv_in(_dt(out), _ptr(sample), _SRC[sample.dtype], B, cin, h, w, _ptr(weight_packed), _ptr(bias),
                                      cout, _ptr(out), _stream()))
     return out
diff --git a/theatergen_amd/pipelines.py b/theatergen_amd/pipelines.py
--- a/theatergen_amd/pipelines.py
+++ b/theatergen_amd/pipelines.py
@@ -195,7 +195,7 @@
             down = self.adapter_feats
         noise_pred = self.unet(self.model_in, self.sched, self.enc, added_cond_kwargs=self.added, return_dict=False,
                                out_dtype=torch.float32, down_block_additional_residuals=down,
-                               mid_block_additional_residual=mid, time_proj=tp)[0]
+                               mid_block_additional_residual=mid, time_proj=tp, shared_pair=self.added is None)[0]
         if self.kind != "ddim":
             ops.step_epilogue_sigma(noise_pred, self.latents, self.g, self.coef, self.step_idx, advance=True, noise=self.step_noise,
                                     frozen=self.frozen, frozen_mask=self.frozen_mask, frozen_steps=self.frozen_steps, history=self.history,
diff --git a/theatergen_amd/rowchain.py b/theatergen_amd/rowchain.py
--- a/theatergen_amd/rowchain.py
+++ b/theatergen_amd/rowchain.py
@@ -87,7 +87,7 @@
     return rc_pack_tiles(w2, bo.detach().float() if bo is not None else None)
 
 
-def linear320(x2d, lin_weight, bias, res, owner, name, cached):
+def linear320(x2d, lin_weight, bias, res, owner, name, cached, pair_out=None):
     M, K = x2d.shape
     N = lin_weight.shape[0]
     if not ENABLED or x2d.stride(1) != 1 or lin_weight.shape[1] != K:
@@ -96,7 +96,7 @@
     if K == 320 and (MODE & 1) and N % 64 == 0 and M >= MIN_ROWS_CHAIN:
         trace("linear320 yes", name, M, N)
         wpk = cached(owner, "rc_" + name, ts, lambda: rc_pack(lin_weight.detach(), bias.detach().float() if bias is not None else None))
-        return ops.rc_linear(x2d, wpk, N, res=res)
+        return ops.rc_linear(x2d, wpk, N, res=res, pair_out=pair_out)
     trace("linear_rc no", name, M, K, N)
     return None
 
diff --git a/theatergen_amd/unet.py b/theatergen_amd/unet.py
--- a/theatergen_amd/unet.py
+++ b/theatergen_amd/unet.py
@@ -8,7 +8,7 @@
 from . import ops
 from . import rowchain
 from .attention_processor import (tensor_version, Attention, AttnProcessor, CNAttnProcessor, IPAttnProcessor, _cached, front_eligible, fused_cross_block,
-                                  ln_weight, self_attention_from_qkv)
+                                  ln_weight, pair_output, self_attention_from_qkv)
 from .config import UNetConfig
 from .weights_pack import pack_conv1x1, pack_conv3x3, pack_conv3x3_up2, pack_geglu, pack_ln_linear, rc_pack_tiles
 
@@ -90,7 +90,7 @@
         self._p = _Packed()
         self.temb_slot = None
 
-    def run(self, x: _Act, skip: _Act, tproj):
+    def run(self, x: _Act, skip: _Act, tproj, pair=False, pair_src=None):
         c1 = skip.c if skip is not None else 0
         assert x.c + c1 == self.in_channels
         w1 = self._p.get("c1", [self.conv1.weight], lambda: pack_conv3x3(self.conv1.weight.detach()))
@@ -106,8 +106,12 @@
             kw1.update(gn_out=gn1)
         if _FUSE_GN and ops.conv3x3_takes_gn(x.t.dtype, x.b, x.h, x.w, x.c, c1, self.out_channels):
             g0 = _gn_of(x.gn, self.groups) if skip is None else None
-            coef = (ops.groupnorm_from_partials(g0, x.b, x.hw, x.c, self.eps, self.norm1.weight, self.norm1.bias) if g0 is not None else
-                    ops.groupnorm_coef(x.t, x.b, x.hw, self.groups, self.eps, self.norm1.weight, self.norm1.bias, x1=x1))
+            if g0 is not None:
+                coef = ops.groupnorm_from_partials(g0, x.b, x.hw, x.c, self.eps, self.norm1.weight, self.norm1.bias)
+            elif pair_src is not None and skip is None:
+                coef = ops.groupnorm_coef(pair_src.t, pair_src.b, x.hw, self.groups, self.eps, self.norm1.weight, self.norm1.bias)[:x.b]
+            else:
+                coef = ops.groupnorm_coef(x.t, x.b, x.hw, self.groups, self.eps, self.norm1.weight, self.norm1.bias, x1=x1)
             h = ops.conv3x3(x.t, w1, x.b, x.h, x.w, x.c, x1=x1, c1=c1, a_coef=coef, a_silu=True, **kw1)
         else:
             h = ops.groupnorm(x.t, x.b, x.hw, self.groups, self.eps, self.norm1.weight, self.norm1.bias, silu=True, x1=x1)
@@ -119,6 +123,9 @@
         else:
             res = x.t
         kw2 = dict(bias=self.conv2.bias, res=res, out_scale=1.0 / self.output_scale_factor)
+        full = torch.empty((2 * x.b * x.hw, self.out_channels), dtype=x.t.dtype, device=x.t.device) if pair else None
+        if pair:
+            kw2.update(pair_out=full)
         gn2 = {"groups": self.groups} if _GN_EPI else None
         if gn2 is not None:
             kw2.update(gn_out=gn2)
@@ -130,7 +137,10 @@
         else:
             h = ops.groupnorm(h, x.b, x.hw, self.groups, self.eps, self.norm2.weight, self.norm2.bias, silu=True)
             out = ops.conv3x3(h, w2, x.b, x.h, x.w, self.out_channels, **kw2)
-        return _Act(out, x.b, x.h, x.w, self.out_channels, gn=_gn_of(gn2, self.groups))
+        half = _Act(out, x.b, x.h, x.w, self.out_channels, gn=_gn_of(gn2, self.groups))
+        if pair:
+            return half, _Act(full, 2 * x.b, x.h, x.w, self.out_channels)
+        return half
 
 
 class Downsample2D(nn.Module):
@@ -145,6 +155,9 @@
         kw = {} if res is None else dict(res=res)
         out = ops.conv3x3(x.t, w, x.b, x.h, x.w, x.c, stride=2, bias=self.conv.bias, **kw)
         return _Act(out, x.b, (x.h - 1) // 2 + 1, (x.w - 1) // 2 + 1, x.c)
+
+
+_CFG_SHARE = os.environ.get("TG_CFG_SHARE", "1") != "0"
 
 
 _UP_FOLD = os.environ.get("TG_UP_FOLD", "1") != "0"
@@ -265,23 +278,36 @@
             out = out[0]
         return ops.add(out.reshape(b * n, -1).contiguous(), residual)
 
-    def run(self, x2d, b, n, enc, ca_kwargs, tail=None, pre_qkv=None):
+    def _attn1_pair(self, fn, x2d):
+        with pair_output() as got:
+            h = fn()
+        if got["full"] is not None:
+            return got["full"]
+        full = torch.empty((2 * h.shape[0], h.shape[1]), dtype=h.dtype, device=h.device)
+        ops.dup_rows(h, full[:h.shape[0]])
+        ops.dup_rows(h, full[h.shape[0]:])
+        return full
+
+    def run(self, x2d, b, n, enc, ca_kwargs, tail=None, pre_qkv=None, pair=False):
         M, C = x2d.shape
+        one = (lambda fn, t: self._attn1_pair(fn, t)) if pair else (lambda fn, t: fn())
+        bf = 2 * b if pair else b
+        M = 2 * M if pair else M
         if _LN_MODE and M >= _FUSE_LN_MIN_ROWS and C % 64 == 0 and x2d.stride(0) == C:
             def folded(norm, t, n_out=0):
                 return (norm, ops.layernorm_stats(t, norm.eps) if (_LN_MODE & 4 or _pp_takes_ln(t.shape[0], n_out, t.shape[1])) else None)
             if _LN_MODE & 1:
                 if pre_qkv is not None:
-                    x2d = self_attention_from_qkv(self.attn1, pre_qkv[0], pre_qkv[1], pre_qkv[2], b, n, x2d)
+                    x2d = one(lambda: self_attention_from_qkv(self.attn1, pre_qkv[0], pre_qkv[1], pre_qkv[2], b, n, x2d), x2d)
                 else:
-                    x2d = self._call(self.attn1, x2d, b, n, None, x2d, ca_kwargs, ln=folded(self.norm1, x2d, 3 * self.attn1.to_q.weight.shape[0]))
-                h2 = fused_cross_block(self.attn2, self.norm2, x2d, b, n, enc, ca_kwargs)
-                x2d = h2 if h2 is not None else self._call(self.attn2, x2d, b, n, enc, x2d, ca_kwargs, ln=folded(self.norm2, x2d))
+                    x2d = one(lambda: self._call(self.attn1, x2d, b, n, None, x2d, ca_kwargs, ln=folded(self.norm1, x2d, 3 * self.attn1.to_q.weight.shape[0])), x2d)
+                h2 = fused_cross_block(self.attn2, self.norm2, x2d, bf, n, enc, ca_kwargs)
+                x2d = h2 if h2 is not None else self._call(self.attn2, x2d, bf, n, enc, x2d, ca_kwargs, ln=folded(self.norm2, x2d))
             else:
                 h = ops.layernorm(x2d, self.norm1.weight, self.norm1.bias, self.norm1.eps)
-                x2d = self._call(self.attn1, h, b, n, None, x2d, ca_kwargs)
+                x2d = one(lambda: self._call(self.attn1, h, b, n, None, x2d, ca_kwargs), x2d)
                 h = ops.layernorm(x2d, self.norm2.weight, self.norm2.bias, self.norm2.eps)
-                x2d = self._call(self.attn2, h, b, n, enc, x2d, ca_kwargs)
+                x2d = self._call(self.attn2, h, bf, n, enc, x2d, ca_kwargs)
             fused = self.ff.run_fused(x2d, self.norm3, tail)
             if fused is not None:
                 return (fused, True) if tail is not None else fused
@@ -290,9 +316,9 @@
             h = ops.layernorm(x2d, self.norm3.weight, self.norm3.bias, self.norm3.eps)
             return self.ff.run(h, x2d)
         h = ops.layernorm(x2d, self.norm1.weight, self.norm1.bias, self.norm1.eps)
-        x2d = self._call(self.attn1, h, b, n, None, x2d, ca_kwargs)
+        x2d = one(lambda: self._call(self.attn1, h, b, n, None, x2d, ca_kwargs), x2d)
         h = ops.layernorm(x2d, self.norm2.weight, self.norm2.bias, self.norm2.eps)
-        x2d = self._call(self.attn2, h, b, n, enc, x2d, ca_kwargs)
+        x2d = self._call(self.attn2, h, bf, n, enc, x2d, ca_kwargs)
         h = ops.layernorm(x2d, self.norm3.weight, self.norm3.bias, self.norm3.eps)
         return self.ff.run(h, x2d)
 
@@ -337,7 +363,9 @@
         wqkv = self._p.get("rc_front_qkv", [wl, ul, vl], lambda: rc_pack_tiles(wl, vl, ul))
         return ops.rc_front(x.t, coef, win, wqkv, x.hw, blk.norm1.eps)
 
-    def run(self, x: _Act, enc, ca_kwargs):
+    def run(self, x: _Act, enc, ca_kwargs, pair_full=None):
+        pair = pair_full is not None
+        xr = pair_full if pair else x
         w_in = self._w("in", self.proj_in)
         pre = self._front(x, w_in, ca_kwargs)
         if pre is not None:
@@ -354,14 +382,14 @@
         for i, blk in enumerate(self.transformer_blocks):
             if base_key is not None:
                 ca_kwargs["attn_key"] = base_key + [i]
-            y = blk.run(y, x.b, x.hw, enc, ca_kwargs, tail=(w_out, self.proj_out.bias, x.t) if i == last else None,
-                        pre_qkv=pre if i == 0 else None)
+            y = blk.run(y, x.b if (pair and i == 0) else xr.b, x.hw, enc, ca_kwargs, tail=(w_out, self.proj_out.bias, xr.t) if i == last else None,
+                        pre_qkv=pre if i == 0 else None, pair=pair and i == 0)
             if isinstance(y, tuple):
-                return _Act(y[0], x.b, x.h, x.w, x.c)
-        out = rowchain.linear320(y, w_out, self.proj_out.bias, x.t, self, "proj_out", _cached)
+                return _Act(y[0], xr.b, x.h, x.w, x.c)
+        out = rowchain.linear320(y, w_out, self.proj_out.bias, xr.t, self, "proj_out", _cached)
         if out is None:
-            out = ops.linear(y, w_out, self.proj_out.bias, res=x.t)
-        return _Act(out, x.b, x.h, x.w, x.c)
+            out = ops.linear(y, w_out, self.proj_out.bias, res=xr.t)
+        return _Act(out, xr.b, x.h, x.w, x.c)
 
 
 class _Block(nn.Module):
@@ -555,6 +583,21 @@
         tproj = ops.linear(ops.act(emb, ops.ACT_SILU), w, b)
         return emb, tproj
 
+    def _pair_prefix_ok(self, ca_kwargs, rows):
+        blk = self.down_blocks[0]
+        if ca_kwargs or not blk.has_cross_attention or len(blk.resnets) == 0:
+            return False
+        tfm0 = blk.attentions[0]
+        if len(tfm0.transformer_blocks) == 0:
+            return False
+        a1 = tfm0.transformer_blocks[0].attn1
+        if type(a1.processor) is not AttnProcessor or a1.rescale_output_factor != 1.0 or a1.residual_connection:
+            return False
+        if getattr(a1, "group_norm", None) is not None or getattr(a1, "spatial_norm", None) is not None:
+            return False
+        chain = rowchain.ENABLED and self.config.block_out_channels[0] == 320
+        return not (chain and rows >= rowchain.MIN_ROWS_CHAIN > rows // 2)
+
     def _residual(self, act: _Act, extra):
         if isinstance(extra, _Act):
             if (extra.b, extra.h, extra.w, extra.c) != (act.b, act.h, act.w, act.c):
@@ -584,7 +627,7 @@
 
     def forward(self, sample, timestep, encoder_hidden_states, class_labels=None, timestep_cond=None, attention_mask=None,
                 cross_attention_kwargs=None, added_cond_kwargs=None, down_block_additional_residuals=None,
-                mid_block_additional_residual=None, encoder_attention_mask=None, return_dict=True, out_dtype=None, time_proj=None):
+                mid_block_additional_residual=None, encoder_attention_mask=None, return_dict=True, out_dtype=None, time_proj=None, shared_pair=False):
         cfg = self.config
         if attention_mask is not None or encoder_attention_mask is not None or class_labels is not None or timestep_cond is not None:
             raise NotImplementedError("attention masks / class labels / timestep_cond are not on the TheaterGen hot path")
@@ -606,8 +649,11 @@
         else:
             _, tproj = self.time_embed(timestep, B, added_cond_kwargs)
 
+        if shared_pair and B % 2:
+            raise ValueError(f"shared_pair needs an even batch (two equal halves), got {B}")
+        share = shared_pair and _CFG_SHARE and self._pair_prefix_ok(ca_kwargs, B * H * W)
         w_in = self._p.get("conv_in", [self.conv_in.weight], lambda: pack_conv3x3(self.conv_in.weight.detach()))
-        x = _Act(ops.conv_in(sample.contiguous(), w_in, self.conv_in.bias, cfg.block_out_channels[0], dt), B, H, W,
+        x = _Act(ops.conv_in(sample.contiguous(), w_in, self.conv_in.bias, cfg.block_out_channels[0], dt, pair=share), B, H, W,
                  cfg.block_out_channels[0])
 
         is_controlnet = mid_block_additional_residual is not None and down_block_additional_residuals is not None
@@ -618,11 +664,16 @@
             cross_feat = feats.pop(0) if blk.has_cross_attention and feats else None
             last = len(blk.resnets) - 1
             for j, resnet in enumerate(blk.resnets):
-                x = resnet.run(x, None, tproj)
+                xh = None
+                if share and i == 0 and j == 0:
+                    hb = B // 2
+                    xh, x = resnet.run(_Act(x.t[:hb * x.hw], hb, x.h, x.w, x.c), None, tproj[:hb], pair=True, pair_src=x)
+                else:
+                    x = resnet.run(x, None, tproj)
                 if blk.has_cross_attention:
                     if track_keys:
                         ca_kwargs["attn_key"] = ["down", i, j]
-                    x = blk.attentions[j].run(x, enc, ca_kwargs)
+                    x = blk.attentions[j].run(x, enc, ca_kwargs) if xh is None else blk.attentions[j].run(xh, enc, ca_kwargs, pair_full=x)
                     if j == last and cross_feat is not None:
                         x = self._adapter_add(x, cross_feat)
                 res.append(x)
```
